# populationgenomics/cuKING

Measured on AMD Instinct MI355X. Metric: sample-pairs/s (all-pairs KING), higher is better.
Workload: dtype fp4 products, f32 accumulate (exact integers)

## Files before the change

### cuking_amd/csrc/king_abi.hip

```cpp
#include <hip/hip_runtime.h>

#include <algorithm>
#include <cstdio>
#include <cstdlib>
#include <cstring>
#include <vector>

#include "king_common.h"
#include "king_host.h"

using namespace cuking;

namespace {

#define HIP_TRY(expr)                                                      \
  do {                                                                     \
    const hipError_t _e = (expr);                                          \
    if (_e != hipSuccess) {                                                \
      (void)hipGetLastError();  \
      return cuking_fail(_e == hipErrorOutOfMemory ? CUKING_ERR_OUT_OF_MEMORY     \
                                            : CUKING_ERR_DEVICE,           \
                  "%s failed: %s", #expr, hipGetErrorString(_e));          \
    }                                                                      \
  } while (0)

uint32_t ceil_div(uint32_t a, uint32_t b) {
  return (uint32_t)(((uint64_t)a + b - 1) / b);
}
uint32_t round_up(uint32_t a, uint32_t b) { return ceil_div(a, b) * b; }

struct EventPair {
  hipEvent_t start = nullptr, stop = nullptr;
};

struct Timer {
  std::vector<EventPair> pool;
  size_t used = 0;

  hipError_t begin(hipStream_t s, EventPair **out) {
    if (used == pool.size()) {
      EventPair p;
      hipError_t e = hipEventCreate(&p.start);
      if (e != hipSuccess) return e;
      e = hipEventCreate(&p.stop);
      if (e != hipSuccess) return e;
      pool.push_back(p);
    }
    *out = &pool[used++];
    return hipEventRecord((*out)->start, s);
  }
  hipError_t collect(double *ms, uint64_t *n) {
    *ms = 0;
    *n = used;
    for (size_t k = 0; k < used; ++k) {
      hipError_t e = hipEventSynchronize(pool[k].stop);
      if (e != hipSuccess) return e;
      float t = 0;
      e = hipEventElapsedTime(&t, pool[k].start, pool[k].stop);
      if (e != hipSuccess) return e;
      *ms += t;
    }
    return hipSuccess;
  }
  void destroy() {
    for (auto &p : pool) {
      if (p.start) (void)hipEventDestroy(p.start);
      if (p.stop) (void)hipEventDestroy(p.stop);
    }
    pool.clear();
    used = 0;
  }
};

}

struct cuking_ctx {
  int device = 0;
  cuking_kernel kernel = CUKING_KERNEL_TILED;
  int variant = 0;
  uint32_t band_rows = 0;
  int counts_mode = -1;
  int xcd_swizzle = 2;
  uint32_t dyn_tail_tiles = 16384;

  uint4 *planes = nullptr;
  size_t planes_bytes = 0;
  uint64_t *band_prefix = nullptr;
  size_t band_prefix_bytes = 0;
  TileSpace prefix_for = {0, 0, 0, 0};

  uint32_t split_wgs = 0;
  struct StreamScratch {
    hipStream_t stream;
    uint32_t *split = nullptr;
    uint8_t *filter = nullptr;
    uint64_t filter_tiles = 0;
  };
  std::vector<StreamScratch> scratch;
  unsigned long long filter_totals_retired[kNumTotals] = {};
  uint32_t filter_quadrant_cap = kFilterQuadrantCap;
  uint32_t filter_cand_cap = kFilterCandCap;
  uint32_t filter_split_min_steps = 8;
  int filter_check0 = 1, filter_check1 = 1, filter_check_emit = (int)kCheckEmitCap;
  int filter_rotate = 1;
  uint32_t filter_rotate_min_steps = 128;
  uint32_t filter_rotate_min_tiles = 2048;
  int filter_sort = 1;
  bool filter_lazy_codes = true;
  void *sort_temp = nullptr;
  size_t sort_temp_bytes = 0;

  struct Prepared {
    bool valid = false;
    cuking_submatrix sm = {0, 0, 0, 0};
    uint32_t words_per_sample = 0;
    int variant = -1;
    uint32_t tile = 0;
    const uint64_t *bits = nullptr;
    bool codes = true;
    std::vector<uint8_t> tiles;
    hipStream_t ordered_on = nullptr;
    bool ordered_valid = false;
  } prepared;
  std::vector<std::pair<hipStream_t, hipEvent_t>> readers;

  bool reuse_prepared = false;
  uint64_t workspace_allocations = 0, host_syncs = 0, conversions_skipped = 0;

  bool timing = false;
  Timer king_timer, prepare_timer;
};

namespace {

int default_variant() {
  if (const char *v = getenv("CUKING_AMD_VARIANT")) {
    const int k = atoi(v);
    if (k >= 0 && k < kNumTiledVariants) return k;
  }
  return kMfmaFilterVariant;
}

int effective_variant(const cuking_ctx *ctx, uint32_t words_per_sample) {
  const uint64_t sites = (uint64_t)round_up(words_per_sample, 8) * 32;
  int v = ctx->variant;
  if ((v == kMfmaN4Variant || v == kMfmaFilterVariant) && sites > kMfmaN4MaxSites) v = kMfmaVariant;
  if (v == kMfmaVariant && sites > kMfmaMaxSites) v = 2;
  return v;
}

TiledVariant plan_variant(const cuking_ctx *ctx, uint32_t words_per_sample) {
  TiledVariant v = tiled_variant(effective_variant(ctx, words_per_sample));
  v.tile = tiled_variant(ctx->variant).tile;
  return v;
}

bool use_full_counts(const cuking_ctx *ctx, float kin_threshold, bool dense,
                     uint32_t words_per_sample) {
  if (dense || ctx->counts_mode == 1) return true;
  if (ctx->counts_mode == 0) return false;
  if (!(kin_threshold > 0.0f)) return true;
  const double sites = 32.0 * words_per_sample;
  const double c = is_mfma_variant(effective_variant(ctx, words_per_sample)) ? 2.05 : 1.6;
  return (double)kin_threshold * kin_threshold * sites < c * c;
}

cuking_status bind(cuking_ctx *ctx) {
  if (ctx == nullptr) return cuking_fail(CUKING_ERR_INVALID_ARGUMENT, "null context");
  HIP_TRY(hipSetDevice(ctx->device));
  return CUKING_OK;
}

PlaneGeometry make_geometry(const cuking_submatrix &sm,
                            uint32_t words_per_sample,
                            const TiledVariant &v) {
  PlaneGeometry g;
  g.num_rows = sm_num_rows(sm);
  g.num_cols = sm_num_cols(sm);
  g.diag = sm_is_diag(sm) ? 1u : 0u;
  g.rows_padded = round_up(g.num_rows, v.tile);
  g.cols_padded = round_up(g.num_cols, v.tile);
  g.col_base = g.diag ? 0u : g.rows_padded;
  g.s_stride = g.diag ? g.rows_padded : g.rows_padded + g.cols_padded;
  g.k_words = round_up(words_per_sample, v.k_chunk);
  return g;
}

uint32_t band_rows_for(uint32_t pinned, const PlaneGeometry &g, const TiledVariant &v) {
  if (pinned != 0) return pinned;
  if (v.layout == kLayoutWord) return 17;
  if (v.tile == kFilterTile) return 8;
  return g.rows_padded / v.tile >= 128 ? 5 : 17;
}

TileSpace make_tiles(const PlaneGeometry &g, const TiledVariant &v,
                     uint32_t band_rows) {
  band_rows = band_rows_for(band_rows, g, v);
  TileSpace t;
  t.tiles_r = g.rows_padded / v.tile;
  t.tiles_c = g.cols_padded / v.tile;
  t.band_rows = band_rows;
  t.diag = g.diag;
  return t;
}

uint64_t total_tiles(const TileSpace &t) {
  uint64_t n = 0;
  for (uint32_t b = 0; b < t.num_bands(); ++b) n += t.band_tiles(b);
  return n;
}

constexpr size_t kMaxStreams = 8;

void free_filter_scratch(cuking_ctx *ctx, cuking_ctx::StreamScratch &e) {
  if (e.filter == nullptr) return;
  unsigned long long v[kNumTotals] = {};
  if (hipMemcpy(v, e.filter + filter_scratch_layout(e.filter_tiles).totals, sizeof v,
                hipMemcpyDeviceToHost) == hipSuccess) {
    for (uint32_t k = 0; k < kNumTotals; ++k) ctx->filter_totals_retired[k] += v[k];
  }
  (void)hipGetLastError();
  (void)hipFree(e.filter);
  e.filter = nullptr;
}

void evict_scratch(cuking_ctx *ctx, size_t k) {
  cuking_ctx::StreamScratch &e = ctx->scratch[k];
  ++ctx->host_syncs;
  if (hipStreamSynchronize(e.stream) != hipSuccess) {
    (void)hipGetLastError();
    (void)hipDeviceSynchronize();
    (void)hipGetLastError();
  }
  free_filter_scratch(ctx, e);
  if (e.split != nullptr) (void)hipFree(e.split);
  ctx->scratch.erase(ctx->scratch.begin() + (ptrdiff_t)k);
}

bool uses_split_slab(const cuking_ctx *ctx) {
  return ctx->split_wgs != 0 && is_mfma_variant(ctx->variant);
}
bool uses_filter_scratch(const cuking_ctx *ctx) { return ctx->variant == kMfmaFilterVariant; }

cuking_status alloc_scratch(cuking_ctx *ctx, void **p, size_t bytes, size_t zero_at,
                            size_t zero_bytes, hipStream_t stream) {
  HIP_TRY(hipMalloc(p, bytes));
  ++ctx->workspace_allocations;
  const hipError_t e = hipMemsetAsync(static_cast<uint8_t *>(*p) + zero_at, 0, zero_bytes, stream);
  if (e != hipSuccess) {
    (void)hipFree(*p);
    *p = nullptr;
    HIP_TRY(e);
  }
  return CUKING_OK;
}

cuking_status scratch_for(cuking_ctx *ctx, hipStream_t stream, uint64_t tiles,
                          cuking_ctx::StreamScratch **out) {
  *out = nullptr;
  const bool split = uses_split_slab(ctx), filter = uses_filter_scratch(ctx);
  if (!split && !filter) return CUKING_OK;
  cuking_ctx::StreamScratch *e = nullptr;
  for (auto &x : ctx->scratch)
    if (x.stream == stream) e = &x;
  if (e == nullptr) {
    if (ctx->scratch.size() >= kMaxStreams) evict_scratch(ctx, 0);
    ctx->scratch.push_back({stream});
    e = &ctx->scratch.back();
  }
  cuking_status st;
  if (split && e->split == nullptr) {
    st = alloc_scratch(ctx, reinterpret_cast<void **>(&e->split),
                       mfma_split_scratch_bytes(ctx->split_wgs), 0,
                       mfma_split_counter_bytes(ctx->split_wgs), stream);
    if (st != CUKING_OK) return st;
  }
  const FilterScratchLayout want = filter_scratch_layout(tiles);
  if (filter && e->filter != nullptr && filter_scratch_layout(e->filter_tiles).bytes < want.bytes) {
    ++ctx->host_syncs;
    HIP_TRY(hipStreamSynchronize(stream));
    free_filter_scratch(ctx, *e);
  }
  if (filter && e->filter == nullptr) {
    st = alloc_scratch(ctx, reinterpret_cast<void **>(&e->filter), want.bytes, want.totals,
                       kFilterCtrlBytes + kFilterTicketBytes, stream);
    if (st != CUKING_OK) return st;
    e->filter_tiles = tiles;
  }
  *out = e;
  return CUKING_OK;
}

struct Outputs {
  uint32_t max_results;
  cuking_result *results;
  uint32_t *result_index, *result_overflow;
  cuking_counts *counts;
};
cuking_status launch_args(cuking_ctx *ctx, hipStream_t stream, const cuking_submatrix &sm,
                          uint32_t words_per_sample, const uint64_t *d_bit_sets,
                          const PlaneGeometry &geo, const TileSpace &tiles,
                          uint64_t block_tiles, float kin_threshold, const Outputs &out,
                          TiledArgs *args) {
  TiledArgs &a = *args;
  a = {};
  a.planes = ctx->planes;
  a.geo = geo;
  a.tiles = tiles;
  a.band_prefix = ctx->band_prefix;
  a.i_begin = sm.i_begin;
  a.j_begin = sm.j_begin;
  a.kin_threshold = kin_threshold;
  a.max_results = out.max_results;
  a.results = out.results;
  a.result_index = out.result_index;
  a.result_overflow = out.result_overflow;
  a.dense_counts = out.counts;
  a.rect_row_stride = 1;
  a.bits = d_bit_sets;
  a.words_per_sample = words_per_sample;
  a.split_wgs = ctx->split_wgs;
  a.xcd_chunk = (uint32_t)ctx->xcd_swizzle;
  a.dyn_tiles = ctx->dyn_tail_tiles;
  if (plan_variant(ctx, words_per_sample).layout == kLayoutNibbleStats) {
    a.perm = plane_perm(ctx->planes, geo);
    if (!ctx->prepared.codes) a.codes_ready = plane_flags(ctx->planes, geo);
  }
  cuking_ctx::StreamScratch *e;
  const cuking_status st = scratch_for(ctx, stream, block_tiles, &e);
  if (st != CUKING_OK || e == nullptr) return st;
  if (uses_split_slab(ctx)) {
    a.split_counters = e->split;
    a.split_scratch = e->split + mfma_split_counter_bytes(ctx->split_wgs) / sizeof(uint32_t);
  }
  if (!uses_filter_scratch(ctx)) return CUKING_OK;
  uint8_t *base = e->filter;
  const FilterScratchLayout l = filter_scratch_layout(e->filter_tiles);
  a.sample_stats = plane_stats(ctx->planes, geo);
  a.t2 = plane_t2(ctx->planes, geo);
  a.prefix_u = plane_prefix_u(ctx->planes, geo);
  a.cohort_sums = plane_cohort_sums(ctx->planes, geo);
  a.filter_ctrl = reinterpret_cast<uint32_t *>(base);
  a.filter_totals = reinterpret_cast<unsigned long long *>(base + l.totals);
  a.fsplit_tickets = reinterpret_cast<uint32_t *>(base + l.tickets);
  a.tile_done = base + l.tile_done;
  a.cand_list = reinterpret_cast<uint2 *>(base + l.cand);
  a.cand_cap = ctx->filter_cand_cap < l.cand_entries ? ctx->filter_cand_cap : l.cand_entries;
  a.quadrant_cap = ctx->filter_quadrant_cap;
  a.dense_list = reinterpret_cast<uint2 *>(base + l.dense);
  a.dense_cap = l.chunk_tiles * 4;
  a.fsplit_first = ctx->filter_split_min_steps;
  a.fsplit_slabs = ctx->split_wgs != 0 ? reinterpret_cast<float4 *>(base + l.slabs) : nullptr;
  a.check0 = (uint32_t)ctx->filter_check0;
  a.check1 = (uint32_t)ctx->filter_check1 | ((uint32_t)ctx->filter_check_emit << 8) |
             (ctx->filter_check0 != 0 ? 1u << 16 : 0u);
  a.rotate = (uint32_t)ctx->filter_rotate;
  a.rotate_min_steps = ctx->filter_rotate_min_steps;
  a.rotate_min_tiles = ctx->filter_rotate_min_tiles;
  a.check_steps = plane_check_steps(ctx->planes, geo);
  return CUKING_OK;
}

bool filter_runs(const cuking_ctx *ctx, uint32_t words_per_sample, bool full, float kin_threshold) {
  return effective_variant(ctx, words_per_sample) == kMfmaFilterVariant && !full &&
         kin_threshold > 0.f && kin_threshold < 0.5f;
}

hipError_t launch_planned(const cuking_ctx *ctx, uint32_t words_per_sample, bool full,
                          TiledArgs a, uint64_t num_tiles, hipStream_t stream) {
  const int kv = effective_variant(ctx, words_per_sample);
  a.quad = 0;
  a.tile_list = nullptr;
  a.tile_list_count = nullptr;
  a.tile_list_cap = 0;
  if (tiled_variant(kv).tile != tiled_variant(ctx->variant).tile) {
    if (tiled_variant(kv).tile * 2 != tiled_variant(ctx->variant).tile) return hipErrorInvalidValue;
    a.quad = 1;
    a.tile_begin *= 4;
    num_tiles *= 4;
  }
  return launch_tiled(kv, full, a, num_tiles, stream);
}

void note_reader(cuking_ctx *ctx, hipStream_t stream) {
  for (auto &r : ctx->readers)
    if (r.first == stream) return;
  ctx->readers.emplace_back(stream, nullptr);
}

cuking_status wait_for_readers(cuking_ctx *ctx, hipStream_t stream) {
  bool failed = false;
  for (auto &r : ctx->readers) {
    if (r.first == stream) continue;
    if (r.second == nullptr &&
        hipEventCreateWithFlags(&r.second, hipEventDisableTiming) != hipSuccess) {
      failed = true;
      break;
    }
    if (hipEventRecord(r.second, r.first) != hipSuccess ||
        hipStreamWaitEvent(stream, r.second, 0) != hipSuccess) {
      failed = true;
      break;
    }
  }
  if (failed) {
    (void)hipGetLastError();
    ++ctx->host_syncs;
    HIP_TRY(hipDeviceSynchronize());
  }
  for (auto &r : ctx->readers)
    if (r.second) (void)hipEventDestroy(r.second);
  ctx->readers.clear();
  ctx->readers.emplace_back(stream, nullptr);
  ctx->prepared.ordered_on = stream;
  ctx->prepared.ordered_valid = true;
  for (auto &t : ctx->prepared.tiles)
    if (t == 2) t = 1;
  return CUKING_OK;
}

void mark_read(cuking_ctx *ctx, uint32_t begin, uint32_t end) {
  std::vector<uint8_t> &t = ctx->prepared.tiles;
  if (end > t.size()) end = (uint32_t)t.size();
  for (uint32_t k = begin; k < end; ++k) t[k] = 2;
}

bool same_block(const cuking_ctx::Prepared &p, const cuking_submatrix &sm,
                uint32_t words_per_sample, int variant, uint32_t tile, const uint64_t *bits) {
  return p.valid && p.sm.i_begin == sm.i_begin && p.sm.i_end == sm.i_end &&
         p.sm.j_begin == sm.j_begin && p.sm.j_end == sm.j_end &&
         p.words_per_sample == words_per_sample && p.variant == variant &&
         p.tile == tile && p.bits == bits;
}

cuking_status grow(cuking_ctx *ctx, void **buf, size_t *bytes, size_t need) {
  if (need <= *bytes) return CUKING_OK;
  ++ctx->host_syncs;
  HIP_TRY(hipDeviceSynchronize());
  if (*buf) HIP_TRY(hipFree(*buf));
  *buf = nullptr;
  *bytes = 0;
  HIP_TRY(hipMalloc(buf, need));
  ++ctx->workspace_allocations;
  *bytes = need;
  return CUKING_OK;
}

cuking_status ensure_workspace(cuking_ctx *ctx, const PlaneGeometry &geo, const TiledVariant &v,
                               const TileSpace &tiles) {
  const size_t planes = plane_bytes(geo, v.layout);
  if (planes > ctx->planes_bytes) ctx->prepared.valid = false;
  cuking_status st = grow(ctx, reinterpret_cast<void **>(&ctx->planes), &ctx->planes_bytes, planes);
  if (st != CUKING_OK) return st;
  const size_t prefix = ((size_t)tiles.num_bands() + 1) * sizeof(uint64_t);
  if (prefix > ctx->band_prefix_bytes) ctx->prefix_for = TileSpace{0, 0, 0, 0};
  st = grow(ctx, reinterpret_cast<void **>(&ctx->band_prefix), &ctx->band_prefix_bytes, prefix);
  if (st != CUKING_OK || v.layout != kLayoutNibbleStats || ctx->filter_sort == 0) return st;
  return grow(ctx, &ctx->sort_temp, &ctx->sort_temp_bytes, sort_temp_bytes_for(geo.s_stride));
}

bool same_tile_space(const TileSpace &a, const TileSpace &b) {
  return a.tiles_r == b.tiles_r && a.tiles_c == b.tiles_c && a.band_rows == b.band_rows &&
         a.diag == b.diag;
}

cuking_status upload_prefix(cuking_ctx *ctx, const TileSpace &tiles, hipStream_t stream) {
  const uint32_t nb = tiles.num_bands();
  std::vector<uint64_t> prefix((size_t)nb + 1, 0);
  for (uint32_t b = 0; b < nb; ++b) prefix[b + 1] = prefix[b] + tiles.band_tiles(b);
  HIP_TRY(hipMemcpyAsync(ctx->band_prefix, prefix.data(), prefix.size() * sizeof(uint64_t),
                         hipMemcpyHostToDevice, stream));
  ++ctx->host_syncs;
  HIP_TRY(hipStreamSynchronize(stream));
  ctx->prefix_for = tiles;
  return CUKING_OK;
}

cuking_status convert_codes_now(cuking_ctx *ctx, const PlaneGeometry &geo,
                                uint32_t words_per_sample, const uint64_t *d_bit_sets,
                                hipStream_t stream) {
  cuking_ctx::Prepared &pr = ctx->prepared;
  const uint32_t all = (uint32_t)pr.tiles.size();
  for (uint32_t t = 0; t < all;) {
    if (pr.tiles[t] == 0) {
      ++t;
      continue;
    }
    uint32_t e = t;
    while (e < all && pr.tiles[e] != 0) ++e;
    HIP_TRY(launch_prepare_nibbles(true, false, d_bit_sets, words_per_sample, geo, ctx->planes,
                                   plane_perm(ctx->planes, geo), t, e, nullptr, nullptr, stream));
    t = e;
  }
  HIP_TRY(hipMemsetAsync(plane_flags(ctx->planes, geo), 1, sizeof(uint32_t), stream));
  pr.codes = true;
  return CUKING_OK;
}

cuking_status prepare(cuking_ctx *ctx, const cuking_submatrix &sm,
                      uint32_t words_per_sample, const uint64_t *d_bit_sets,
                      hipStream_t stream, PlaneGeometry *geo_out,
                      TileSpace *tiles_out, bool need_codes, uint32_t s_tile_begin = 0,
                      uint32_t s_tile_end = 0xFFFFFFFFu) {
  const int variant = effective_variant(ctx, words_per_sample);
  const TiledVariant v = plan_variant(ctx, words_per_sample);
  const PlaneGeometry geo = make_geometry(sm, words_per_sample, v);
  const TileSpace tiles = make_tiles(geo, v, ctx->band_rows);
  *geo_out = geo;
  *tiles_out = tiles;

  cuking_status st = ensure_workspace(ctx, geo, v, tiles);
  if (st != CUKING_OK) return st;
  const uint32_t all_tiles = (geo.s_stride + 63) / 64;
  const uint32_t t_end = s_tile_end < all_tiles ? s_tile_end : all_tiles;
  cuking_ctx::Prepared &pr = ctx->prepared;
  const bool new_prefix = !same_tile_space(ctx->prefix_for, tiles);
  const bool same = same_block(pr, sm, words_per_sample, variant, v.tile, d_bit_sets);
  if (ctx->reuse_prepared && same && !new_prefix) {
    bool all_there = true;
    for (uint32_t t = s_tile_begin; t < t_end && all_there; ++t) all_there = pr.tiles[t] != 0;
    if (all_there) {
      ++ctx->conversions_skipped;
      if (v.layout == kLayoutNibbleStats && need_codes && !pr.codes)
        return convert_codes_now(ctx, geo, words_per_sample, d_bit_sets, stream);
      return CUKING_OK;
    }
  }
  const bool other_stream = pr.ordered_valid && pr.ordered_on != stream;
  bool must_wait = new_prefix && !ctx->readers.empty();
  if (!same) {
    must_wait = must_wait || !ctx->readers.empty();
    pr.valid = true;
    pr.sm = sm;
    pr.words_per_sample = words_per_sample;
    pr.variant = variant;
    pr.tile = v.tile;
    pr.bits = d_bit_sets;
    pr.tiles.assign(all_tiles, 0);
    pr.codes = true;
  }
  for (uint32_t t = s_tile_begin; t < t_end; ++t)
    must_wait = must_wait || pr.tiles[t] == 2 || (pr.tiles[t] == 1 && other_stream);
  if (must_wait) {
    st = wait_for_readers(ctx, stream);
    if (st != CUKING_OK) return st;
  }
  for (uint32_t t = s_tile_begin; t < t_end; ++t) pr.tiles[t] = 1;
  if (new_prefix) {
    st = upload_prefix(ctx, tiles, stream);
    if (st != CUKING_OK) return st;
  }

  if (plane_bytes(geo, v.layout) == 0) return CUKING_OK;
  EventPair *ev = nullptr;
  if (ctx->timing) HIP_TRY(ctx->prepare_timer.begin(stream, &ev));
  if (v.layout == kLayoutNibbleStats) {
    const bool whole = s_tile_begin == 0 && t_end == all_tiles;
    const bool codes = need_codes || !ctx->filter_lazy_codes || !whole;
    const uint32_t sb = s_tile_begin * 64, se = t_end * 64;
    if (s_tile_begin == 0)
      HIP_TRY(hipMemsetAsync(const_cast<unsigned long long *>(plane_cohort_sums(ctx->planes, geo)),
                             0, 64, stream));
    HIP_TRY(hipMemsetAsync(plane_flags(ctx->planes, geo), 0, sizeof(uint32_t), stream));
    HIP_TRY(launch_sample_stats(d_bit_sets, words_per_sample, geo, ctx->planes, sb, se, stream));
    HIP_TRY(launch_sample_order(geo, words_per_sample, ctx->planes, sb, se,
                                ctx->filter_sort == 2 || (ctx->filter_sort == 1 && whole),
                                ctx->sort_temp, ctx->sort_temp_bytes, stream));
    HIP_TRY(launch_prepare_nibbles(codes, true, d_bit_sets, words_per_sample, geo, ctx->planes,
                                   plane_perm(ctx->planes, geo), s_tile_begin, t_end, nullptr,
                                   nullptr, stream));
    if (!codes) {
      pr.codes = false;
    } else if (!pr.codes) {
      st = convert_codes_now(ctx, geo, words_per_sample, d_bit_sets, stream);
      if (st != CUKING_OK) return st;
    } else {
      HIP_TRY(hipMemsetAsync(plane_flags(ctx->planes, geo), 1, sizeof(uint32_t), stream));
    }
  } else {
    HIP_TRY(launch_prepare_planes(v.layout, d_bit_sets, words_per_sample, geo, ctx->planes,
                                  s_tile_begin, s_tile_end, stream));
  }
  if (ev) HIP_TRY(hipEventRecord(ev->stop, stream));
  return CUKING_OK;
}

cuking_status run_tiled(cuking_ctx *ctx, const cuking_submatrix &sm,
                        uint32_t words_per_sample, const uint64_t *d_bit_sets,
                        uint64_t tile_begin, uint64_t tile_end, bool whole,
                        float kin_threshold, const Outputs &out, hipStream_t stream) {
  PlaneGeometry geo;
  TileSpace tiles;
  const bool full = use_full_counts(ctx, kin_threshold, out.counts != nullptr, words_per_sample);
  cuking_status st = prepare(ctx, sm, words_per_sample, d_bit_sets, stream, &geo, &tiles,
                             !filter_runs(ctx, words_per_sample, full, kin_threshold));
  if (st != CUKING_OK) return st;
  const uint64_t n_tiles = total_tiles(tiles);
  if (whole) {
    tile_begin = 0;
    tile_end = n_tiles;
  }
  if (tile_begin > tile_end || tile_end > n_tiles)
    return cuking_fail(CUKING_ERR_INVALID_ARGUMENT,
                "tile range [%llu, %llu) outside [0, %llu)",
                (unsigned long long)tile_begin, (unsigned long long)tile_end,
                (unsigned long long)n_tiles);
  if (tile_begin == tile_end) return CUKING_OK;

  TiledArgs a;
  st = launch_args(ctx, stream, sm, words_per_sample, d_bit_sets, geo, tiles, n_tiles,
                   kin_threshold, out, &a);
  if (st != CUKING_OK) return st;
  a.tile_begin = tile_begin;

  EventPair *ev = nullptr;
  if (ctx->timing) HIP_TRY(ctx->king_timer.begin(stream, &ev));
  HIP_TRY(launch_planned(ctx, words_per_sample, full, a, tile_end - tile_begin, stream));
  note_reader(ctx, stream);
  mark_read(ctx, 0, 0xFFFFFFFFu);
  if (ev) HIP_TRY(hipEventRecord(ev->stop, stream));
  return CUKING_OK;
}

cuking_status run_stream(cuking_ctx *ctx, const cuking_submatrix &sm,
                         uint32_t words_per_sample, const uint64_t *d_bit_sets,
                         float kin_threshold, uint32_t max_results,
                         cuking_result *d_results, uint32_t *d_result_index,
                         uint32_t *d_result_overflow, cuking_counts *d_counts,
                         hipStream_t stream) {
  EventPair *ev = nullptr;
  if (ctx->timing) HIP_TRY(ctx->king_timer.begin(stream, &ev));
  HIP_TRY(launch_stream(sm, words_per_sample, d_bit_sets, kin_threshold,
                        max_results, d_results, d_result_index,
                        d_result_overflow, d_counts, stream));
  if (ev) HIP_TRY(hipEventRecord(ev->stop, stream));
  return CUKING_OK;
}


enum : uint8_t {
  kInvalidatesLayout = 1,
  kResizesSlabs = 2,
};

struct Option {
  const char *key;
  int64_t lo, hi;
  const char *error;
  uint32_t error_arg;
  uint8_t effects;
  int64_t (*get)(const cuking_ctx *);
  void (*set)(cuking_ctx *, int64_t);
  int64_t hole = INT64_MIN;
};

#define CTX_FIELD(f)                                                     \
  [](const cuking_ctx *c) -> int64_t { return (int64_t)c->f; },          \
  [](cuking_ctx *c, int64_t v) { c->f = (decltype(c->f))v; }

const Option kOptions[] = {
    {"variant", 0, kNumTiledVariants - 1, "variant outside [0, %u)", kNumTiledVariants, 0,
     CTX_FIELD(variant)},
    {"band_rows", 0, 64, "band_rows outside [0, 64]", 0, 0, CTX_FIELD(band_rows)},
    {"counts_mode", -1, 1, "counts_mode outside [-1, 1]", 0, 0, CTX_FIELD(counts_mode)},
    {"split_wgs", 0, 4096, "split_wgs outside [0, 4096]", 0, kResizesSlabs, CTX_FIELD(split_wgs)},
    {"xcd_swizzle", 0, 2, "xcd_swizzle outside [0, 2]", 0, 0, CTX_FIELD(xcd_swizzle)},
    {"dyn_tail_tiles", 0, 0x7FFFFFFF, "dyn_tail_tiles outside [0, 2^31)", 0, 0,
     CTX_FIELD(dyn_tail_tiles)},
    {"reuse_prepared", 0, 1, "reuse_prepared outside [0, 1]", 0, 0, CTX_FIELD(reuse_prepared)},
    {"filter_sort", 0, 2, "filter_sort outside [0, 2]", 0, kInvalidatesLayout,
     CTX_FIELD(filter_sort)},
    {"filter_lazy_codes", 0, 1, "filter_lazy_codes outside [0, 1]", 0, kInvalidatesLayout,
     CTX_FIELD(filter_lazy_codes)},
    {"filter_check0", 0, 2, "filter_check0 outside [0, 2]", 0, 0, CTX_FIELD(filter_check0)},
    {"filter_check1", 0, 1 + kNumCheckShares, "filter_check1 outside {0, 1, 3 .. %u}",
     1 + kNumCheckShares, 0, CTX_FIELD(filter_check1), 2},
    {"filter_check_emit", 0, 255, "filter_check_emit outside [0, 255]", 0, 0,
     CTX_FIELD(filter_check_emit)},
    {"filter_rotate", 0, 2 + kNumPhases, "filter_rotate outside [0, %u]", 2 + kNumPhases, 0,
     CTX_FIELD(filter_rotate)},
    {"filter_rotate_min_steps", 1, 1 << 20, "filter_rotate_min_steps outside [1, 2^20]", 0, 0,
     CTX_FIELD(filter_rotate_min_steps)},
    {"filter_rotate_min_tiles", 0, 1 << 30, "filter_rotate_min_tiles outside [0, 2^30]", 0, 0,
     CTX_FIELD(filter_rotate_min_tiles)},
    {"filter_quadrant_cap", 0, 16384, "filter_quadrant_cap outside [0, 16384]", 0, 0,
     CTX_FIELD(filter_quadrant_cap)},
    {"filter_cand_cap", 0, kFilterCandCap, "filter_cand_cap outside [0, %u]", kFilterCandCap, 0,
     CTX_FIELD(filter_cand_cap)},
    {"filter_split_min_steps", 1, 4096, "filter_split_min_steps outside [1, 4096]", 0, 0,
     CTX_FIELD(filter_split_min_steps)},
    {"max_launch_blocks", 0, INT64_MAX, "negative block cap", 0, 0,
     [](const cuking_ctx *) -> int64_t { return (int64_t)max_blocks_override(); },
     [](cuking_ctx *, int64_t v) { set_max_blocks_per_launch((uint64_t)v); }},
    {"filter_check_min_steps", 4, 1 << 20, "filter_check_min_steps outside [4, 2^20]", 0,
     kInvalidatesLayout,
     [](const cuking_ctx *) -> int64_t { return filter_check_min_steps(); },
     [](cuking_ctx *, int64_t v) { set_filter_check_min_steps((uint32_t)v); }},
};
#undef CTX_FIELD

const Option *find_option(const char *key) {
  for (const Option &o : kOptions)
    if (strcmp(o.key, key) == 0) return &o;
  return nullptr;
}

cuking_status read_diagnostic(const cuking_ctx *ctx, const char *key, int64_t *value) {
  const std::pair<const char *, uint64_t> counters[] = {
      {"workspace_allocations", ctx->workspace_allocations},
      {"host_syncs", ctx->host_syncs},
      {"conversions_skipped", ctx->conversions_skipped}};
  for (const auto &c : counters)
    if (strcmp(c.first, key) == 0) {
      *value = (int64_t)c.second;
      return CUKING_OK;
    }
  const char *const totals[kNumTotals] = {"filter_candidates", "filter_dense_quadrants",
                                          "filter_early_exits", "filter_rotated_tiles"};
  static_assert(kTotalCand == 0 && kTotalDense == 1 && kTotalEarly == 2 && kTotalRotated == 3,
                "totals[] in the order of the running totals");
  uint32_t word = 0;
  while (word < kNumTotals && strcmp(totals[word], key) != 0) ++word;
  const bool ticks = strcmp(key, "filter_step_ticks16") == 0;
  if (word == kNumTotals && !ticks)
    return cuking_fail(CUKING_ERR_INVALID_ARGUMENT, "unknown option %s", key);
  if (hipSetDevice(ctx->device) != hipSuccess || hipDeviceSynchronize() != hipSuccess)
    return cuking_fail(CUKING_ERR_DEVICE, "device wait failed");
  unsigned long long sum = 0;
  uint64_t count = 0;
  for (const auto &e : ctx->scratch) {
    if (e.filter == nullptr) continue;
    if (ticks) {
      uint32_t w[8];
      if (hipMemcpy(w, e.filter + kCtrlStepTicks * 4, sizeof w, hipMemcpyDeviceToHost) != hipSuccess)
        return cuking_fail(CUKING_ERR_DEVICE, "reading the filter counters failed");
      for (uint32_t v : w)
        if (v != 0) {
          sum += v;
          ++count;
        }
    } else {
      unsigned long long v = 0;
      if (hipMemcpy(&v, e.filter + filter_scratch_layout(e.filter_tiles).totals + word * 8, 8,
                    hipMemcpyDeviceToHost) != hipSuccess)
        return cuking_fail(CUKING_ERR_DEVICE, "reading the filter counters failed");
      sum += v;
    }
  }
  if (ticks) *value = count != 0 ? (int64_t)(sum / count) : 0;
  else *value = (int64_t)(sum + ctx->filter_totals_retired[word]);
  return CUKING_OK;
}

}

extern "C" {


int cuking_device_count(void) {
  int n = 0;
  if (hipGetDeviceCount(&n) != hipSuccess) return 0;
  return n;
}

cuking_status cuking_ctx_create(int device, cuking_ctx **out) {
  if (out == nullptr) return cuking_fail(CUKING_ERR_INVALID_ARGUMENT, "null out pointer");
  *out = nullptr;
  int n = 0;
  hipError_t e = hipGetDeviceCount(&n);
  if (e != hipSuccess || n == 0)
    return cuking_fail(CUKING_ERR_DEVICE,
                "no HIP device available (%s); this library has no CPU path",
                e == hipSuccess ? "0 devices" : hipGetErrorString(e));
  if (device < 0 || device >= n)
    return cuking_fail(CUKING_ERR_INVALID_ARGUMENT, "device %d outside [0, %d)", device, n);
  hipDeviceProp_t prop;
  HIP_TRY(hipGetDeviceProperties(&prop, device));
  if (strncmp(prop.gcnArchName, "gfx950", 6) != 0)
    return cuking_fail(CUKING_ERR_DEVICE,
                "device %d is %s; this library only carries gfx950 code",
                device, prop.gcnArchName);
  HIP_TRY(hipSetDevice(device));
  cuking_ctx *ctx = new cuking_ctx();
  ctx->device = device;
  ctx->variant = default_variant();
  ctx->split_wgs = (uint32_t)prop.multiProcessorCount;
  *out = ctx;
  return CUKING_OK;
}

void cuking_ctx_destroy(cuking_ctx *ctx) {
  if (ctx == nullptr) return;
  (void)hipSetDevice(ctx->device);
  if (ctx->planes) (void)hipFree(ctx->planes);
  if (ctx->band_prefix) (void)hipFree(ctx->band_prefix);
  if (ctx->sort_temp) (void)hipFree(ctx->sort_temp);
  for (auto &e : ctx->scratch) {
    if (e.split) (void)hipFree(e.split);
    if (e.filter) (void)hipFree(e.filter);
  }
  for (auto &r : ctx->readers)
    if (r.second) (void)hipEventDestroy(r.second);
  ctx->king_timer.destroy();
  ctx->prepare_timer.destroy();
  delete ctx;
}

cuking_status cuking_ctx_set_kernel(cuking_ctx *ctx, cuking_kernel kernel) {
  if (ctx == nullptr) return cuking_fail(CUKING_ERR_INVALID_ARGUMENT, "null context");
  if (kernel != CUKING_KERNEL_TILED && kernel != CUKING_KERNEL_STREAM)
    return cuking_fail(CUKING_ERR_INVALID_ARGUMENT, "unknown kernel %d", (int)kernel);
  ctx->kernel = kernel;
  return CUKING_OK;
}

cuking_status cuking_ctx_set_option(cuking_ctx *ctx, const char *key,
                                    int64_t value) {
  if (ctx == nullptr || key == nullptr)
    return cuking_fail(CUKING_ERR_INVALID_ARGUMENT, "null argument");
  const Option *o = find_option(key);
  if (o == nullptr) return cuking_fail(CUKING_ERR_INVALID_ARGUMENT, "unknown option %s", key);
  if (value < o->lo || value > o->hi || value == o->hole)
    return cuking_fail(CUKING_ERR_INVALID_ARGUMENT, o->error, o->error_arg);
  if ((o->effects & kResizesSlabs) && value != o->get(ctx)) {
    HIP_TRY(hipDeviceSynchronize());
    for (auto &e : ctx->scratch) {
      if (e.split) (void)hipFree(e.split);
      e.split = nullptr;
    }
  }
  o->set(ctx, value);
  if (o->effects & kInvalidatesLayout) ctx->prepared.valid = false;
  return CUKING_OK;
}

cuking_status cuking_device_alloc(cuking_ctx *ctx, size_t bytes, void **d_ptr) {
  cuking_status st = bind(ctx);
  if (st != CUKING_OK) return st;
  if (d_ptr == nullptr) return cuking_fail(CUKING_ERR_INVALID_ARGUMENT, "null out pointer");
  *d_ptr = nullptr;
  if (bytes == 0) return CUKING_OK;
  HIP_TRY(hipMalloc(d_ptr, bytes));
  return CUKING_OK;
}

cuking_status cuking_device_free(cuking_ctx *ctx, void *d_ptr) {
  cuking_status st = bind(ctx);
  if (st != CUKING_OK) return st;
  if (d_ptr) HIP_TRY(hipFree(d_ptr));
  return CUKING_OK;
}

cuking_status cuking_memset_async(cuking_ctx *ctx, void *d_ptr, int byte_value,
                                  size_t bytes, void *stream) {
  cuking_status st = bind(ctx);
  if (st != CUKING_OK) return st;
  if (bytes) HIP_TRY(hipMemsetAsync(d_ptr, byte_value, bytes, (hipStream_t)stream));
  return CUKING_OK;
}

cuking_status cuking_copy_to_device(cuking_ctx *ctx, void *d_dst,
                                    const void *src, size_t bytes,
                                    void *stream) {
  cuking_status st = bind(ctx);
  if (st != CUKING_OK) return st;
  if (bytes)
    HIP_TRY(hipMemcpyAsync(d_dst, src, bytes, hipMemcpyHostToDevice,
                           (hipStream_t)stream));
  return CUKING_OK;
}

cuking_status cuking_copy_to_host(cuking_ctx *ctx, void *dst, const void *d_src,
                                  size_t bytes, void *stream) {
  cuking_status st = bind(ctx);
  if (st != CUKING_OK) return st;
  if (bytes)
    HIP_TRY(hipMemcpyAsync(dst, d_src, bytes, hipMemcpyDeviceToHost,
                           (hipStream_t)stream));
  return CUKING_OK;
}

cuking_status cuking_stream_synchronize(cuking_ctx *ctx, void *stream) {
  cuking_status st = bind(ctx);
  if (st != CUKING_OK) return st;
  HIP_TRY(hipStreamSynchronize((hipStream_t)stream));
  return CUKING_OK;
}

cuking_status cuking_stream_create(cuking_ctx *ctx, void **stream) {
  cuking_status st = bind(ctx);
  if (st != CUKING_OK) return st;
  if (stream == nullptr) return cuking_fail(CUKING_ERR_INVALID_ARGUMENT, "null out pointer");
  hipStream_t s = nullptr;
  HIP_TRY(hipStreamCreateWithFlags(&s, hipStreamNonBlocking));
  *stream = s;
  return CUKING_OK;
}

cuking_status cuking_stream_destroy(cuking_ctx *ctx, void *stream) {
  cuking_status st = bind(ctx);
  if (st != CUKING_OK) return st;
  if (stream) {
    auto &rs = ctx->readers;
    for (size_t k = 0; k < rs.size(); ++k)
      if (rs[k].first == (hipStream_t)stream) {
        HIP_TRY(hipStreamSynchronize((hipStream_t)stream));
        if (rs[k].second) (void)hipEventDestroy(rs[k].second);
        rs.erase(rs.begin() + k);
        break;
      }
    HIP_TRY(hipStreamDestroy((hipStream_t)stream));
  }
  return CUKING_OK;
}

cuking_status cuking_host_alloc(cuking_ctx *ctx, size_t bytes, void **ptr) {
  cuking_status st = bind(ctx);
  if (st != CUKING_OK) return st;
  if (ptr == nullptr) return cuking_fail(CUKING_ERR_INVALID_ARGUMENT, "null out pointer");
  *ptr = nullptr;
  if (bytes == 0) return CUKING_OK;
  HIP_TRY(hipHostMalloc(ptr, bytes, hipHostMallocDefault));
  return CUKING_OK;
}

cuking_status cuking_host_free(cuking_ctx *ctx, void *ptr) {
  cuking_status st = bind(ctx);
  if (st != CUKING_OK) return st;
  if (ptr) HIP_TRY(hipHostFree(ptr));
  return CUKING_OK;
}


cuking_status cuking_pack_device(cuking_ctx *ctx, const cuking_submatrix *sm,
                                 uint32_t words_per_sample, uint64_t *d_bit_set,
                                 const int64_t *d_row_idx,
                                 const int64_t *d_col_idx,
                                 const int32_t *d_n_alt_alleles,
                                 size_t num_triples, uint32_t *d_status,
                                 void *stream) {
  cuking_status st = bind(ctx);
  if (st != CUKING_OK) return st;
  st = cuking_check_block(sm, words_per_sample);
  if (st != CUKING_OK) return st;
  if (num_triples &&
      (!d_bit_set || !d_row_idx || !d_col_idx || !d_n_alt_alleles || !d_status))
    return cuking_fail(CUKING_ERR_INVALID_ARGUMENT, "null device pointer");
  HIP_TRY(launch_pack(*sm, words_per_sample, d_bit_set, d_row_idx, d_col_idx,
                      d_n_alt_alleles, num_triples, d_status,
                      (hipStream_t)stream));
  return CUKING_OK;
}

cuking_status cuking_pack_device_compact(cuking_ctx *ctx, const cuking_submatrix *sm,
                                         uint32_t words_per_sample, uint64_t *d_bit_set,
                                         const uint32_t *d_site,
                                         const uint32_t *d_sample_alt, size_t num_triples,
                                         uint32_t *d_status, void *stream) {
  cuking_status st = bind(ctx);
  if (st != CUKING_OK) return st;
  st = cuking_check_block(sm, words_per_sample);
  if (st != CUKING_OK) return st;
  if (num_triples && (!d_bit_set || !d_site || !d_sample_alt || !d_status))
    return cuking_fail(CUKING_ERR_INVALID_ARGUMENT, "null device pointer");
  HIP_TRY(launch_pack_compact(words_per_sample, sm_num_samples(*sm), d_bit_set, d_site,
                              d_sample_alt, num_triples, d_status, (hipStream_t)stream));
  return CUKING_OK;
}

cuking_status cuking_event_create(cuking_ctx *ctx, void **event) {
  cuking_status st = bind(ctx);
  if (st != CUKING_OK) return st;
  if (event == nullptr) return cuking_fail(CUKING_ERR_INVALID_ARGUMENT, "null out pointer");
  hipEvent_t e = nullptr;
  HIP_TRY(hipEventCreateWithFlags(&e, hipEventDisableTiming));
  *event = e;
  return CUKING_OK;
}

cuking_status cuking_event_record(cuking_ctx *ctx, void *event, void *stream) {
  cuking_status st = bind(ctx);
  if (st != CUKING_OK) return st;
  HIP_TRY(hipEventRecord((hipEvent_t)event, (hipStream_t)stream));
  return CUKING_OK;
}

cuking_status cuking_event_synchronize(cuking_ctx *ctx, void *event) {
  cuking_status st = bind(ctx);
  if (st != CUKING_OK) return st;
  HIP_TRY(hipEventSynchronize((hipEvent_t)event));
  return CUKING_OK;
}

cuking_status cuking_event_destroy(cuking_ctx *ctx, void *event) {
  cuking_status st = bind(ctx);
  if (st != CUKING_OK) return st;
  if (event) HIP_TRY(hipEventDestroy((hipEvent_t)event));
  return CUKING_OK;
}

uint32_t cuking_tile_samples(const cuking_ctx *ctx) {
  return tiled_variant(ctx ? ctx->variant : default_variant()).tile;
}

uint64_t cuking_num_tiles(const cuking_ctx *ctx, const cuking_submatrix *sm) {
  if (sm == nullptr) return 0;
  const TiledVariant &v = tiled_variant(ctx ? ctx->variant : default_variant());
  const PlaneGeometry g = make_geometry(*sm, 2, v);
  if (g.num_rows == 0 || g.num_cols == 0) return 0;
  return total_tiles(make_tiles(g, v, ctx ? ctx->band_rows : 0));
}

cuking_status cuking_tile_bounds(const cuking_ctx *ctx,
                                 const cuking_submatrix *sm, uint64_t tile,
                                 uint32_t *row_begin, uint32_t *row_end,
                                 uint32_t *col_begin, uint32_t *col_end) {
  cuking_status st = cuking_check_block(sm, 2);
  if (st != CUKING_OK) return st;
  const TiledVariant &v = tiled_variant(ctx ? ctx->variant : default_variant());
  const PlaneGeometry g = make_geometry(*sm, 2, v);
  const TileSpace ts = make_tiles(g, v, ctx ? ctx->band_rows : 0);
  if (g.num_rows == 0 || g.num_cols == 0 || tile >= total_tiles(ts))
    return cuking_fail(CUKING_ERR_INVALID_ARGUMENT, "tile index out of range");
  uint32_t b = 0;
  uint64_t first = 0;
  while (first + ts.band_tiles(b) <= tile) first += ts.band_tiles(b++);
  uint32_t tr, tc;
  ts.decode(b, tile - first, &tr, &tc);
  auto clampr = [&](uint64_t x) { return (uint32_t)std::min<uint64_t>(x, g.num_rows); };
  auto clampc = [&](uint64_t x) { return (uint32_t)std::min<uint64_t>(x, g.num_cols); };
  if (row_begin) *row_begin = sm->i_begin + clampr((uint64_t)tr * v.tile);
  if (row_end) *row_end = sm->i_begin + clampr((uint64_t)(tr + 1) * v.tile);
  if (col_begin) *col_begin = sm->j_begin + clampc((uint64_t)tc * v.tile);
  if (col_end) *col_end = sm->j_begin + clampc((uint64_t)(tc + 1) * v.tile);
  return CUKING_OK;
}

cuking_status cuking_ctx_get_option(const cuking_ctx *ctx, const char *key,
                                    int64_t *value) {
  if (ctx == nullptr || key == nullptr || value == nullptr)
    return cuking_fail(CUKING_ERR_INVALID_ARGUMENT, "null argument");
  if (const Option *o = find_option(key)) {
    *value = o->get(ctx);
    return CUKING_OK;
  }
  return read_diagnostic(ctx, key, value);
}

int cuking_num_variants(void) { return kNumTiledVariants; }
const char *cuking_variant_name(int variant) {
  if (variant < 0 || variant >= kNumTiledVariants) return "";
  return tiled_variant(variant).name;
}

static cuking_status check_compute_args(const cuking_submatrix *sm,
                                        uint32_t words_per_sample,
                                        const uint64_t *d_bit_sets) {
  cuking_status st = cuking_check_block(sm, words_per_sample);
  if (st != CUKING_OK) return st;
  if (sm_num_samples(*sm) != 0 && d_bit_sets == nullptr)
    return cuking_fail(CUKING_ERR_INVALID_ARGUMENT, "null bitset pointer");
  return CUKING_OK;
}

cuking_status cuking_compute_king(cuking_ctx *ctx, const cuking_submatrix *sm,
                                  uint32_t words_per_sample,
                                  const uint64_t *d_bit_sets,
                                  float kin_threshold, uint32_t max_results,
                                  cuking_result *d_results,
                                  uint32_t *d_result_index,
                                  uint32_t *d_result_overflow, void *stream) {
  cuking_status st = bind(ctx);
  if (st != CUKING_OK) return st;
  st = check_compute_args(sm, words_per_sample, d_bit_sets);
  if (st != CUKING_OK) return st;
  if (!d_result_index || !d_result_overflow || (max_results && !d_results))
    return cuking_fail(CUKING_ERR_INVALID_ARGUMENT, "null result pointer");
  if (sm_num_rows(*sm) == 0 || sm_num_cols(*sm) == 0) return CUKING_OK;
  if (ctx->kernel == CUKING_KERNEL_STREAM)
    return run_stream(ctx, *sm, words_per_sample, d_bit_sets, kin_threshold,
                      max_results, d_results, d_result_index, d_result_overflow,
                      nullptr, (hipStream_t)stream);
  return run_tiled(ctx, *sm, words_per_sample, d_bit_sets, 0, 0, true, kin_threshold,
                   {max_results, d_results, d_result_index, d_result_overflow, nullptr},
                   (hipStream_t)stream);
}

cuking_status cuking_compute_king_tiles(
    cuking_ctx *ctx, const cuking_submatrix *sm, uint32_t words_per_sample,
    const uint64_t *d_bit_sets, uint64_t tile_begin, uint64_t tile_end,
    float kin_threshold, uint32_t max_results, cuking_result *d_results,
    uint32_t *d_result_index, uint32_t *d_result_overflow, void *stream) {
  cuking_status st = bind(ctx);
  if (st != CUKING_OK) return st;
  st = check_compute_args(sm, words_per_sample, d_bit_sets);
  if (st != CUKING_OK) return st;
  if (!d_result_index || !d_result_overflow || (max_results && !d_results))
    return cuking_fail(CUKING_ERR_INVALID_ARGUMENT, "null result pointer");
  if (sm_num_rows(*sm) == 0 || sm_num_cols(*sm) == 0) {
    if (tile_begin != 0 || tile_end != 0)
      return cuking_fail(CUKING_ERR_INVALID_ARGUMENT, "empty block has no tiles");
    return CUKING_OK;
  }
  return run_tiled(ctx, *sm, words_per_sample, d_bit_sets, tile_begin, tile_end, false,
                   kin_threshold,
                   {max_results, d_results, d_result_index, d_result_overflow, nullptr},
                   (hipStream_t)stream);
}

static cuking_status tile_span(const cuking_submatrix &sm, uint32_t tile,
                               uint32_t begin, uint32_t end, const char *what,
                               uint32_t *t0, uint32_t *t1) {
  if (begin < sm.i_begin || end > sm.i_end || begin > end)
    return cuking_fail(CUKING_ERR_INVALID_ARGUMENT, "%s range [%u, %u) outside the block",
                what, begin, end);
  const uint32_t b = begin - sm.i_begin, e = end - sm.i_begin;
  if (b % tile != 0 || (e % tile != 0 && end != sm.i_end))
    return cuking_fail(CUKING_ERR_INVALID_ARGUMENT,
                "%s range [%u, %u) is not aligned to the %u-sample tile edge", what,
                begin, end, tile);
  *t0 = b / tile;
  *t1 = (e + tile - 1) / tile;
  return CUKING_OK;
}

cuking_status cuking_prepare_samples(cuking_ctx *ctx, const cuking_submatrix *sm,
                                     uint32_t words_per_sample,
                                     const uint64_t *d_bit_sets,
                                     uint32_t sample_begin, uint32_t sample_end,
                                     void *stream) {
  cuking_status st = bind(ctx);
  if (st != CUKING_OK) return st;
  st = check_compute_args(sm, words_per_sample, d_bit_sets);
  if (st != CUKING_OK) return st;
  if (!sm_is_diag(*sm))
    return cuking_fail(CUKING_ERR_INVALID_ARGUMENT,
                "staged preparation needs a diagonal block (rows == columns)");
  const uint32_t tile = plan_variant(ctx, words_per_sample).tile;
  uint32_t t0, t1;
  st = tile_span(*sm, tile, sample_begin, sample_end, "sample", &t0, &t1);
  if (st != CUKING_OK) return st;
  if (t0 == t1) return CUKING_OK;
  PlaneGeometry geo;
  TileSpace tiles;
  return prepare(ctx, *sm, words_per_sample, d_bit_sets, (hipStream_t)stream, &geo,
                 &tiles, true, t0 * (tile / 64), t1 * (tile / 64));
}

cuking_status cuking_compute_king_rect(
    cuking_ctx *ctx, const cuking_submatrix *sm, uint32_t words_per_sample,
    const uint64_t *d_bit_sets, uint32_t row_begin, uint32_t row_end,
    uint32_t row_step, uint32_t col_begin, uint32_t col_end, float kin_threshold,
    uint32_t max_results, cuking_result *d_results, uint32_t *d_result_index,
    uint32_t *d_result_overflow, void *stream) {
  cuking_status st = bind(ctx);
  if (st != CUKING_OK) return st;
  st = check_compute_args(sm, words_per_sample, d_bit_sets);
  if (st != CUKING_OK) return st;
  if (!sm_is_diag(*sm))
    return cuking_fail(CUKING_ERR_INVALID_ARGUMENT,
                "rectangle launches need a diagonal block (rows == columns)");
  if (!d_result_index || !d_result_overflow || (max_results && !d_results))
    return cuking_fail(CUKING_ERR_INVALID_ARGUMENT, "null result pointer");
  const TiledVariant v = plan_variant(ctx, words_per_sample);
  const PlaneGeometry geo = make_geometry(*sm, words_per_sample, v);
  const TileSpace tiles = make_tiles(geo, v, ctx->band_rows ? ctx->band_rows : 17);
  const size_t need = plane_bytes(geo, v.layout);
  const int variant = effective_variant(ctx, words_per_sample);
  if (ctx->planes == nullptr || ctx->planes_bytes < need ||
      !same_block(ctx->prepared, *sm, words_per_sample, variant, v.tile, d_bit_sets))
    return cuking_fail(CUKING_ERR_FAILED_PRECONDITION,
                "cuking_prepare_samples() has not been called for this block "
                "(or the workspace has been converted for another one since)");
  uint32_t r0, r1, c0, c1;
  st = tile_span(*sm, v.tile, row_begin, row_end, "row", &r0, &r1);
  if (st != CUKING_OK) return st;
  st = tile_span(*sm, v.tile, col_begin, col_end, "column", &c0, &c1);
  if (st != CUKING_OK) return st;
  if (r0 == r1 || c0 == c1) return CUKING_OK;
  if (row_step == 0) row_step = v.tile;
  if (row_step % v.tile != 0)
    return cuking_fail(CUKING_ERR_INVALID_ARGUMENT,
                "row_step %u is not a multiple of the %u-sample tile edge", row_step,
                v.tile);
  const uint32_t stride = row_step / v.tile;
  const uint32_t n_rows = (r1 - r0 + stride - 1) / stride;
  {
    const uint32_t per = v.tile / 64;
    const std::vector<uint8_t> &done = ctx->prepared.tiles;
    auto converted = [&](uint32_t tile) {
      for (uint32_t t = tile * per; t < (tile + 1) * per; ++t)
        if (t >= done.size() || !done[t]) return false;
      return true;
    };
    for (uint32_t r = r0; r < r1; r += stride)
      if (!converted(r))
        return cuking_fail(CUKING_ERR_FAILED_PRECONDITION,
                    "row samples from %u on have not been prepared",
                    sm->i_begin + r * v.tile);
    for (uint32_t c = c0; c < c1; ++c)
      if (!converted(c))
        return cuking_fail(CUKING_ERR_FAILED_PRECONDITION,
                    "column samples from %u on have not been prepared",
                    sm->i_begin + c * v.tile);
  }

  TiledArgs a;
  st = launch_args(ctx, (hipStream_t)stream, *sm, words_per_sample, d_bit_sets, geo, tiles,
                   total_tiles(make_tiles(geo, v, ctx->band_rows)), kin_threshold,
                   {max_results, d_results, d_result_index, d_result_overflow, nullptr}, &a);
  if (st != CUKING_OK) return st;
  a.rect_rows = n_rows;
  a.rect_cols = c1 - c0;
  a.rect_row0 = r0;
  a.rect_col0 = c0;
  a.rect_row_stride = stride;
  a.xcd_chunk = ctx->xcd_swizzle == 2 ? 2u : 0u;
  const bool full = use_full_counts(ctx, kin_threshold, false, words_per_sample);
  if (v.layout == kLayoutNibbleStats && !ctx->prepared.codes &&
      !filter_runs(ctx, words_per_sample, full, kin_threshold)) {
    st = convert_codes_now(ctx, geo, words_per_sample, d_bit_sets, (hipStream_t)stream);
    if (st != CUKING_OK) return st;
    a.codes_ready = nullptr;
  }
  EventPair *ev = nullptr;
  if (ctx->timing) HIP_TRY(ctx->king_timer.begin((hipStream_t)stream, &ev));
  HIP_TRY(launch_planned(ctx, words_per_sample, full, a, (uint64_t)n_rows * (c1 - c0),
                         (hipStream_t)stream));
  note_reader(ctx, (hipStream_t)stream);
  {
    const uint32_t per = v.tile / 64;
    for (uint32_t r = r0; r < r1; r += stride) mark_read(ctx, r * per, (r + 1) * per);
    mark_read(ctx, c0 * per, c1 * per);
  }
  if (ev) HIP_TRY(hipEventRecord(ev->stop, (hipStream_t)stream));
  return CUKING_OK;
}

cuking_status cuking_ctx_reserve(cuking_ctx *ctx, const cuking_submatrix *sm,
                                 uint32_t words_per_sample, void *const *streams,
                                 size_t num_streams) {
  cuking_status st = bind(ctx);
  if (st != CUKING_OK) return st;
  st = cuking_check_block(sm, words_per_sample);
  if (st != CUKING_OK) return st;
  if (num_streams != 0 && streams == nullptr)
    return cuking_fail(CUKING_ERR_INVALID_ARGUMENT, "null stream list");
  if (sm_num_rows(*sm) == 0 || sm_num_cols(*sm) == 0) return CUKING_OK;
  const TiledVariant v = plan_variant(ctx, words_per_sample);
  const PlaneGeometry geo = make_geometry(*sm, words_per_sample, v);
  const TileSpace tiles = make_tiles(geo, v, ctx->band_rows);
  st = ensure_workspace(ctx, geo, v, tiles);
  if (st != CUKING_OK) return st;
  if (!same_tile_space(ctx->prefix_for, tiles)) {
    if (!ctx->readers.empty()) {
      ++ctx->host_syncs;
      HIP_TRY(hipDeviceSynchronize());
    }
    st = upload_prefix(ctx, tiles, nullptr);
    if (st != CUKING_OK) return st;
  }
  if (num_streams > kMaxStreams)
    return cuking_fail(CUKING_ERR_INVALID_ARGUMENT,
                       "at most %zu streams per context can be reserved", kMaxStreams);
  auto named = [&](hipStream_t s) {
    for (size_t k = 0; k < num_streams; ++k)
      if ((hipStream_t)streams[k] == s) return true;
    return false;
  };
  if (uses_split_slab(ctx) || uses_filter_scratch(ctx)) {
    size_t missing = num_streams;
    for (const auto &e : ctx->scratch) missing -= named(e.stream) ? 1 : 0;
    for (size_t k = 0; ctx->scratch.size() + missing > kMaxStreams;) {
      if (named(ctx->scratch[k].stream))
        ++k;
      else
        evict_scratch(ctx, k);
    }
  }
  for (size_t k = 0; k < num_streams; ++k) {
    cuking_ctx::StreamScratch *e;
    st = scratch_for(ctx, (hipStream_t)streams[k], total_tiles(tiles), &e);
    if (st != CUKING_OK) return st;
  }
  return CUKING_OK;
}

cuking_status cuking_invalidate(cuking_ctx *ctx) {
  if (ctx == nullptr) return cuking_fail(CUKING_ERR_INVALID_ARGUMENT, "null context");
  ctx->prepared.valid = false;
  return CUKING_OK;
}

cuking_status cuking_compute_counts(cuking_ctx *ctx, const cuking_submatrix *sm,
                                    uint32_t words_per_sample,
                                    const uint64_t *d_bit_sets,
                                    cuking_counts *d_counts, void *stream) {
  cuking_status st = bind(ctx);
  if (st != CUKING_OK) return st;
  st = check_compute_args(sm, words_per_sample, d_bit_sets);
  if (st != CUKING_OK) return st;
  if (sm_num_rows(*sm) == 0 || sm_num_cols(*sm) == 0) return CUKING_OK;
  if (d_counts == nullptr)
    return cuking_fail(CUKING_ERR_INVALID_ARGUMENT, "null counts pointer");
  if (ctx->kernel == CUKING_KERNEL_STREAM)
    return run_stream(ctx, *sm, words_per_sample, d_bit_sets, 0.f, 0, nullptr,
                      nullptr, nullptr, d_counts, (hipStream_t)stream);
  return run_tiled(ctx, *sm, words_per_sample, d_bit_sets, 0, 0, true, 0.f,
                   {0, nullptr, nullptr, nullptr, d_counts}, (hipStream_t)stream);
}


cuking_status cuking_timing_enable(cuking_ctx *ctx, int enabled) {
  if (ctx == nullptr) return cuking_fail(CUKING_ERR_INVALID_ARGUMENT, "null context");
  ctx->timing = enabled != 0;
  return CUKING_OK;
}

cuking_status cuking_timing_reset(cuking_ctx *ctx) {
  if (ctx == nullptr) return cuking_fail(CUKING_ERR_INVALID_ARGUMENT, "null context");
  ctx->king_timer.used = 0;
  ctx->prepare_timer.used = 0;
  return CUKING_OK;
}

cuking_status cuking_timing_collect(cuking_ctx *ctx, double *king_ms,
                                    uint64_t *king_launches, double *prepare_ms,
                                    uint64_t *prepare_launches) {
  cuking_status st = bind(ctx);
  if (st != CUKING_OK) return st;
  double a = 0, b = 0;
  uint64_t na = 0, nb = 0;
  HIP_TRY(ctx->king_timer.collect(&a, &na));
  HIP_TRY(ctx->prepare_timer.collect(&b, &nb));
  if (king_ms) *king_ms = a;
  if (king_launches) *king_launches = na;
  if (prepare_ms) *prepare_ms = b;
  if (prepare_launches) *prepare_launches = nb;
  return CUKING_OK;
}

cuking_status cuking_clock_probe(cuking_ctx *ctx, uint64_t microseconds,
                                 uint64_t *d_ticks, void *stream) {
  cuking_status st = bind(ctx);
  if (st != CUKING_OK) return st;
  if (d_ticks == nullptr) return cuking_fail(CUKING_ERR_INVALID_ARGUMENT, "null out pointer");
  if (microseconds == 0 || microseconds > 60ull * 1000 * 1000)
    return cuking_fail(CUKING_ERR_INVALID_ARGUMENT, "probe time outside (0, 60 s]");
  HIP_TRY(launch_clock_probe(microseconds, d_ticks, (hipStream_t)stream));
  return CUKING_OK;
}


cuking_status cuking_synth_bitset(cuking_ctx *ctx, uint64_t seed,
                                  const uint32_t *d_kind, const uint32_t *d_pa,
                                  const uint32_t *d_pb, uint32_t sample_begin,
                                  uint32_t sample_end, uint32_t num_sites,
                                  uint32_t words_per_sample,
                                  uint64_t *d_bit_set, void *stream) {
  cuking_status st = bind(ctx);
  if (st != CUKING_OK) return st;
  if (sample_end < sample_begin)
    return cuking_fail(CUKING_ERR_INVALID_ARGUMENT, "sample range reversed");
  if (words_per_sample != cuking_words_per_sample(num_sites))
    return cuking_fail(CUKING_ERR_INVALID_ARGUMENT,
                "words_per_sample %u does not match %u sites", words_per_sample,
                num_sites);
  if (sample_end > sample_begin && (!d_kind || !d_pa || !d_pb || !d_bit_set))
    return cuking_fail(CUKING_ERR_INVALID_ARGUMENT, "null device pointer");
  HIP_TRY(launch_synth(seed, d_kind, d_pa, d_pb, sample_begin, sample_end,
                       num_sites, words_per_sample, d_bit_set,
                       (hipStream_t)stream));
  return CUKING_OK;
}

}
```

### cuking_amd/csrc/king_common.h

```cpp
#ifndef CUKING_AMD_KING_COMMON_H_
#define CUKING_AMD_KING_COMMON_H_

#include <hip/hip_runtime.h>
#include <stdint.h>

#include "cuking_amd.h"
#include "king_submatrix.h"

namespace cuking {

constexpr uint32_t kLayoutWord = 0;
constexpr uint32_t kLayoutQuad = 1;
constexpr uint32_t kLayoutNibble = 2;
constexpr uint32_t kLayoutNibbleStats = 3;

struct PlaneGeometry {
  uint32_t num_rows, num_cols;
  uint32_t rows_padded, cols_padded;
  uint32_t col_base;
  uint32_t s_stride;
  uint32_t k_words;
  uint32_t diag;
};

struct TileSpace {
  uint32_t tiles_r, tiles_c;
  uint32_t band_rows;
  uint32_t diag;

  __host__ __device__ uint32_t num_bands() const {
    return (tiles_r + band_rows - 1) / band_rows;
  }
  __host__ __device__ uint64_t band_tiles(uint32_t b) const {
    const uint32_t r0 = b * band_rows;
    const uint32_t h = (tiles_r - r0 < band_rows) ? tiles_r - r0 : band_rows;
    if (!diag) return (uint64_t)h * tiles_c;
    const uint32_t ncols = tiles_c - r0;
    return (uint64_t)h * (h + 1) / 2 + (uint64_t)(ncols - h) * h;
  }
  __host__ __device__ void decode(uint32_t b, uint64_t u, uint32_t *tr,
                                  uint32_t *tc) const {
    const uint32_t r0 = b * band_rows;
    const uint32_t h = (tiles_r - r0 < band_rows) ? tiles_r - r0 : band_rows;
    if (!diag) {
      *tc = (uint32_t)(u / h);
      *tr = r0 + (uint32_t)(u % h);
      return;
    }
    const uint64_t tri = (uint64_t)h * (h + 1) / 2;
    if (u < tri) {
      uint32_t c = 0;
      uint64_t before = 0;
      while (before + c + 1 <= u) {
        before += c + 1;
        ++c;
      }
      *tc = r0 + c;
      *tr = r0 + (uint32_t)(u - before);
    } else {
      const uint64_t v = u - tri;
      *tc = r0 + h + (uint32_t)(v / h);
      *tr = r0 + (uint32_t)(v % h);
    }
  }
};

struct TiledArgs {
  const uint4 *planes;
  PlaneGeometry geo;
  TileSpace tiles;
  const uint64_t *band_prefix;
  uint64_t tile_begin;
  uint32_t rect_rows, rect_cols, rect_row0, rect_col0, rect_row_stride;
  uint32_t i_begin, j_begin;
  float kin_threshold;
  uint32_t max_results;
  cuking_result *results;
  uint32_t *result_index;
  uint32_t *result_overflow;
  cuking_counts *dense_counts;
  const uint64_t *bits;
  uint32_t words_per_sample;
  uint32_t split_tiles, split_wgs;
  uint32_t split_whole;
  uint32_t *split_scratch, *split_counters;
  uint32_t xcd_chunk, launch_tiles;
  uint32_t dyn_tiles, dyn_wgs;
  uint32_t quad;
  const uint2 *tile_list;
  const uint32_t *tile_list_count;
  uint32_t tile_list_cap;
  const float2 *sample_stats;
  const uint4 *t2;
  uint32_t *filter_ctrl;
  unsigned long long *filter_totals;
  uint2 *cand_list;
  uint32_t cand_cap;
  uint32_t quadrant_cap;
  uint2 *dense_list;
  uint32_t dense_cap;
  uint32_t fsplit_parts, fsplit_first, fsplit_tile0;
  float4 *fsplit_slabs;
  uint32_t *fsplit_tickets;
  const uint32_t *check_steps;
  const float *prefix_u;
  const unsigned long long *cohort_sums;
  uint32_t check0, check1;
  uint32_t rotate, rotate_min_steps;
  uint32_t rotate_min_tiles;
  uint8_t *tile_done;
  const uint32_t *gate;
  uint32_t gate_count;
  const uint8_t *skip_tiles;
  uint64_t skip_base;
  const uint32_t *perm;
  uint32_t *codes_ready;
};

constexpr uint32_t kCheckEmitCap = 64;
constexpr uint32_t kNumCheckShares = 8;
constexpr uint32_t kCheckShares64[kNumCheckShares] = {8, 50, 53, 56, 58, 60, 61, 62};
constexpr uint32_t kNumPhases = 128;
constexpr uint32_t kPhasesPerShare = kNumPhases / 64;
constexpr uint32_t kNumCum = kNumPhases - 1;
__host__ __device__ inline uint32_t phase_step(uint32_t all_steps, uint32_t x) {
  return (uint32_t)((uint64_t)all_steps * x / kNumPhases);
}
__host__ __device__ inline uint32_t check_step_of(uint32_t all_steps, uint32_t k,
                                                  uint32_t min_steps = 64) {
  if (all_steps < min_steps) return 0;
  return phase_step(all_steps, kCheckShares64[k] * kPhasesPerShare);
}
constexpr uint32_t kFilterSplitSlabs = 256;
constexpr size_t kFilterSlabBytes = 256 * 256 * sizeof(float);
constexpr size_t kFilterTicketBytes = kFilterSplitSlabs * sizeof(uint32_t);
__host__ __device__ inline size_t plane_bytes(const PlaneGeometry &g,
                                              uint32_t layout) {
  const size_t base = (size_t)g.k_words * g.s_stride * (layout == kLayoutQuad ? 8 : 16);
  if (layout == kLayoutNibble) return base + base / 4;
  if (layout == kLayoutNibbleStats)
    return base + base / 4 + base / 2 + (size_t)g.s_stride * sizeof(float2) +
           (size_t)g.s_stride * kNumCum * sizeof(float) + 64 + 64 +
           64 + (size_t)g.s_stride * (4 + 8 + 4 * kNumCum + 16);
  return base;
}
__host__ __device__ inline const uint4 *plane_t2(const uint4 *planes, const PlaneGeometry &g) {
  return planes + (size_t)g.k_words * g.s_stride * 5 / 4;
}
__host__ __device__ inline const float2 *plane_stats(const uint4 *planes, const PlaneGeometry &g) {
  return reinterpret_cast<const float2 *>(planes + (size_t)g.k_words * g.s_stride * 7 / 4);
}
__host__ __device__ inline const float *plane_prefix_u(const uint4 *planes, const PlaneGeometry &g) {
  return reinterpret_cast<const float *>(plane_stats(planes, g) + g.s_stride);
}
__host__ __device__ inline const unsigned long long *plane_cohort_sums(const uint4 *planes,
                                                                       const PlaneGeometry &g) {
  return reinterpret_cast<const unsigned long long *>(plane_prefix_u(planes, g) +
                                                      (size_t)g.s_stride * kNumCum);
}

struct TiledVariant {
  const char *name;
  uint32_t tile;
  uint32_t k_chunk;
  uint32_t threads;
  uint32_t lds_bytes;
  uint32_t layout;
};

constexpr uint32_t kMfmaMaxSites = 1u << 24;

constexpr int kNumTiledVariants = 8;
constexpr int kMfmaVariant = 5;
constexpr int kMfmaN4Variant = 6;
constexpr uint32_t kMfmaN4MaxSites = 1u << 22;
constexpr int kMfmaN4Stages = 5;
constexpr uint32_t kMfmaN4LdsBytes = kMfmaN4Stages * 2 * 2 * 4 * 128 * 16;
static_assert(kMfmaN4LdsBytes <= 160 * 1024, "LDS of one CU");
constexpr int kMfmaFilterVariant = 7;
constexpr uint32_t kFilterTile = 256;
constexpr uint32_t kFilterLdsBytes = 5 * 2 * 2 * 2 * 256 * 16;
static_assert(kFilterLdsBytes <= 160 * 1024, "LDS of one CU");
constexpr uint32_t kFilterChunkTiles = 1u << 17;
constexpr uint32_t kFilterCandCap = 1u << 25;
constexpr uint32_t kFilterQuadrantCap = 384;
constexpr size_t kFilterCtrlBytes = 256;
constexpr uint32_t kCtrlCand = 0, kCtrlDense = 1, kCtrlDyn = 2, kCtrlFinished = 3,
                   kCtrlLeft = 4, kCtrlAllLeave = 5, kCtrlGate = 6;
constexpr uint32_t kCtrlStepTicks = 8, kCtrlPos = 16, kPosSlots = 16;
constexpr size_t kCtrlChunkBytes = (kCtrlPos + 8 * kPosSlots * 2) * 4;
constexpr uint32_t kTotalCand = 0, kTotalDense = 1, kTotalEarly = 2, kTotalRotated = 3;
constexpr uint32_t kNumTotals = 4;
__host__ __device__ inline const uint32_t *plane_check_steps(const uint4 *planes,
                                                             const PlaneGeometry &g) {
  return reinterpret_cast<const uint32_t *>(plane_cohort_sums(planes, g) + 8);
}
__host__ __device__ inline uint32_t *plane_flags(const uint4 *planes, const PlaneGeometry &g) {
  return const_cast<uint32_t *>(plane_check_steps(planes, g)) + 16;
}
__host__ __device__ inline uint32_t *plane_perm(const uint4 *planes, const PlaneGeometry &g) {
  return plane_flags(planes, g) + 16;
}
__host__ __device__ inline float2 *plane_tmp_stats(const uint4 *planes, const PlaneGeometry &g) {
  return reinterpret_cast<float2 *>(plane_perm(planes, g) + g.s_stride);
}
__host__ __device__ inline float *plane_tmp_prefix(const uint4 *planes, const PlaneGeometry &g) {
  return reinterpret_cast<float *>(plane_tmp_stats(planes, g) + g.s_stride);
}
__host__ __device__ inline uint32_t *plane_sort_words(const uint4 *planes, const PlaneGeometry &g) {
  return reinterpret_cast<uint32_t *>(plane_tmp_prefix(planes, g) +
                                      (size_t)g.s_stride * kNumCum);
}
constexpr uint32_t kNoSample = 0xFFFFFFFFu;

struct FilterScratchLayout {
  size_t tile_done, totals, tickets, cand, dense, slabs, bytes;
  uint32_t chunk_tiles, cand_entries;
};
inline FilterScratchLayout filter_scratch_layout(uint64_t tiles) {
  FilterScratchLayout l;
  l.chunk_tiles = (uint32_t)(tiles < kFilterChunkTiles ? (tiles ? tiles : 1) : kFilterChunkTiles);
  const uint64_t cand = (uint64_t)l.chunk_tiles * 4 * 64;
  l.cand_entries = (uint32_t)(cand < kFilterCandCap ? cand : kFilterCandCap);
  auto up = [](size_t x) { return (x + 255) / 256 * 256; };
  l.tile_done = kCtrlChunkBytes;
  l.totals = up(l.tile_done + l.chunk_tiles);
  l.tickets = l.totals + kFilterCtrlBytes;
  l.cand = l.tickets + kFilterTicketBytes;
  l.dense = l.cand + up((size_t)l.cand_entries * sizeof(uint2));
  l.slabs = l.dense + up((size_t)l.chunk_tiles * 4 * sizeof(uint2));
  l.bytes = l.slabs + kFilterSplitSlabs * kFilterSlabBytes;
  return l;
}
inline bool is_mfma_variant(int v) {
  return v == kMfmaVariant || v == kMfmaN4Variant || v == kMfmaFilterVariant;
}
constexpr int kMfmaStages = 6;
constexpr uint32_t kMfmaLdsBytes = kMfmaStages * 2 * 2 * 2 * 128 * 16;
constexpr uint32_t kMfmaParkBytes = 4 * 64 * 64 * 4;
static_assert(kMfmaLdsBytes + kMfmaParkBytes <= 160 * 1024, "LDS of one CU");
const TiledVariant &tiled_variant(int v);
hipError_t launch_tiled(int variant, bool full, const TiledArgs &args,
                        uint64_t num_tiles, hipStream_t stream);
hipError_t launch_mfma(bool full, bool nibble, const TiledArgs &args, uint64_t num_tiles,
                       uint32_t lds_bytes, hipStream_t stream);
hipError_t launch_mfma_list(const TiledArgs &args, uint32_t grid, hipStream_t stream);
hipError_t launch_mfma_gated(const TiledArgs &args, uint64_t num_units, uint32_t grid,
                             hipStream_t stream);
hipError_t launch_filter(const TiledArgs &args, uint64_t num_tiles, hipStream_t stream);
hipError_t launch_sample_stats(const uint64_t *d_bit_sets, uint32_t words_per_sample,
                               const PlaneGeometry &geo, uint4 *d_planes, uint32_t s_begin,
                               uint32_t s_end, hipStream_t stream);
void set_filter_check_min_steps(uint32_t steps);
uint32_t filter_check_min_steps();
size_t sort_temp_bytes_for(uint32_t n);
hipError_t launch_sample_order(const PlaneGeometry &geo, uint32_t words_per_sample,
                               uint4 *d_planes, uint32_t s_begin, uint32_t s_end, bool sort,
                               void *sort_temp, size_t sort_temp_bytes, hipStream_t stream);
hipError_t launch_prepare_nibbles(bool codes, bool t2, const uint64_t *d_bit_sets,
                                  uint32_t words_per_sample, const PlaneGeometry &geo,
                                  uint4 *d_planes, const uint32_t *perm, uint32_t s_tile_begin,
                                  uint32_t s_tile_end, const uint32_t *gate,
                                  const uint32_t *ready, hipStream_t stream);
hipError_t launch_mark_codes_ready(const uint32_t *gate, uint32_t *ready, hipStream_t stream);
size_t mfma_split_scratch_bytes(uint32_t wgs);
size_t mfma_split_counter_bytes(uint32_t wgs);

void set_max_blocks_per_launch(uint64_t blocks);
uint64_t max_blocks_override();

hipError_t launch_prepare_planes(uint32_t layout, const uint64_t *d_bit_sets,
                                 uint32_t words_per_sample,
                                 const PlaneGeometry &geo, uint4 *d_planes,
                                 uint32_t s_tile_begin, uint32_t s_tile_end,
                                 hipStream_t stream);

hipError_t launch_stream(const cuking_submatrix &sm, uint32_t words_per_sample,
                         const uint64_t *d_bit_sets, float kin_threshold,
                         uint32_t max_results, cuking_result *d_results,
                         uint32_t *d_result_index, uint32_t *d_result_overflow,
                         cuking_counts *d_dense_counts, hipStream_t stream);

hipError_t launch_pack(const cuking_submatrix &sm, uint32_t words_per_sample,
                       uint64_t *d_bit_set, const int64_t *d_row_idx,
                       const int64_t *d_col_idx, const int32_t *d_n_alt,
                       size_t num_triples, uint32_t *d_status,
                       hipStream_t stream);

hipError_t launch_pack_compact(uint32_t words_per_sample, uint32_t num_samples,
                               uint64_t *d_bit_set, const uint32_t *d_site,
                               const uint32_t *d_sample_alt, size_t num_triples,
                               uint32_t *d_status, hipStream_t stream);

hipError_t launch_synth(uint64_t seed, const uint32_t *d_kind,
                        const uint32_t *d_pa, const uint32_t *d_pb,
                        uint32_t sample_begin, uint32_t sample_end,
                        uint32_t num_sites, uint32_t words_per_sample,
                        uint64_t *d_bit_set, hipStream_t stream);

hipError_t launch_clock_probe(uint64_t microseconds, uint64_t *d_out,
                              hipStream_t stream);

}

#endif
```

### cuking_amd/csrc/king_filter.hip

```cpp
#include <hip/hip_runtime.h>
#include <stdio.h>

#include <atomic>
#include <stdlib.h>

#include "king_common.h"
#include "king_device.h"

#pragma clang diagnostic ignored "-Winline-asm"

namespace cuking {

namespace {

typedef int v8i __attribute__((ext_vector_type(8)));
typedef float v16f __attribute__((ext_vector_type(16)));

constexpr int kT = (int)kFilterTile;
constexpr int kUnits = 2;
constexpr int kStages = 5;
constexpr int kSliceU4 = kT;
constexpr int kStageU4 = 2 * 2 * kUnits * kSliceU4;
constexpr int kStageReqs = 4 * kUnits;
constexpr int kSyncVm = (kStages - 3) * kStageReqs + (kStageReqs - 2);
static_assert(kSyncVm < 64, "vmcnt is a 6-bit counter");
static_assert(kStages * kStageU4 * 16 == (int)kFilterLdsBytes, "LDS size");
constexpr int vmcnt_imm(int n) { return 0x0F70 | (n & 15) | ((n >> 4) << 14); }
constexpr uint32_t kNoPair = 0xFFFFFFFFu;

__device__ __forceinline__ uint32_t source_sample(const PlaneGeometry &geo, uint32_t ps) {
  if (geo.diag || ps < geo.rows_padded) return ps < geo.num_rows ? ps : kNoPair;
  const uint32_t c = ps - geo.col_base;
  return c < geo.num_cols ? geo.num_rows + c : kNoPair;
}

struct CheckWords {
  uint32_t w[kNumCheckShares];
};
constexpr uint32_t kStatsMaxSteps = kMfmaN4MaxSites / 256;
__global__ __launch_bounds__(256) void sample_stats_kernel(
    const uint64_t *__restrict__ bits, uint32_t words_per_sample, PlaneGeometry geo,
    float2 *__restrict__ stats, float *__restrict__ cum, unsigned long long *__restrict__ sums,
    uint32_t *__restrict__ steps_out, CheckWords cw, uint32_t s_begin, uint32_t s_end) {
  __shared__ uint8_t phase_of[kStatsMaxSteps];
  __shared__ int32_t phase_sum[4][kNumPhases];
  const uint32_t lane = threadIdx.x & 63, wave = threadIdx.x >> 6;
  if (blockIdx.x == 0 && threadIdx.x < kNumCheckShares) steps_out[threadIdx.x] = cw.w[threadIdx.x];
  const uint32_t all_steps = geo.k_words / 8;
  for (uint32_t st = threadIdx.x; st < all_steps; st += 256) {
    const uint32_t x = (kNumPhases * (st + 1) - 1) / all_steps;
    phase_of[st] = (uint8_t)(x < kNumPhases ? x : kNumPhases - 1);
  }
#pragma unroll
  for (uint32_t k = 0; k < kNumPhases / 64; ++k) phase_sum[wave][lane + 64 * k] = 0;
  __syncthreads();
  const uint32_t ps = s_begin + blockIdx.x * 4 + wave;
  if (ps >= s_end) return;
  const uint32_t src = source_sample(geo, ps);
  int32_t yc = 0, mc = 0, hc = 0;
  if (src != kNoPair) {
    const uint32_t n = words_per_sample / 2;
    const uint64_t *het = bits + (uint64_t)src * words_per_sample;
    const uint64_t *hom = het + n;
    constexpr uint32_t kAhead = 4;
    for (uint32_t w0 = 0; w0 < n; w0 += 64 * kAhead) {
      uint64_t h[kAhead], v[kAhead];
#pragma unroll
      for (uint32_t k = 0; k < kAhead; ++k) {
        const uint32_t w = w0 + 64 * k + lane;
        const bool in = w < n;
        h[k] = in ? het[w] : 0ull;
        v[k] = in ? hom[w] : 0ull;
      }
#pragma unroll
      for (uint32_t k = 0; k < kAhead; ++k) {
        const uint32_t w = w0 + 64 * k + lane;
        const bool in = w < n;
        const int32_t y = in ? __popcll(~h[k]) : 0;
        const int32_t m = __popcll(h[k] & v[k]);
        yc += y;
        mc += m;
        hc += __popcll(h[k] & ~v[k]);
        int32_t d = y - m;
        d += __shfl_xor(d, 1);
        d += __shfl_xor(d, 2);
        if ((lane & 3) == 0 && in) atomicAdd(&phase_sum[wave][phase_of[w >> 2]], d);
      }
    }
#pragma unroll
    for (int off = 32; off > 0; off >>= 1) {
      yc += __shfl_xor(yc, off);
      mc += __shfl_xor(mc, off);
      hc += __shfl_xor(hc, off);
    }
  }
  static_assert(kNumPhases == 128, "two phases per lane");
  const int32_t p0 = phase_sum[wave][2 * lane], p1 = phase_sum[wave][2 * lane + 1];
  int32_t run = p0 + p1;
#pragma unroll
  for (int off = 1; off < 64; off <<= 1) {
    const int32_t up = __shfl_up(run, off);
    if ((int)lane >= off) run += up;
  }
  cum[(size_t)(2 * lane) * geo.s_stride + ps] = (float)(run - p1);
  if (2 * lane + 1 < kNumCum) cum[(size_t)(2 * lane + 1) * geo.s_stride + ps] = (float)run;
  if (lane == 0) {
    stats[ps] = make_float2((float)(yc - mc), (float)hc);
    if (src != kNoPair && ((blockIdx.x & 15) == 0 || gridDim.x < 64)) {
      __hip_atomic_fetch_add(sums, 1ull, __ATOMIC_RELAXED, __HIP_MEMORY_SCOPE_AGENT);
      __hip_atomic_fetch_add(sums + 1, (unsigned long long)mc, __ATOMIC_RELAXED,
                             __HIP_MEMORY_SCOPE_AGENT);
      __hip_atomic_fetch_add(sums + 2, (unsigned long long)hc, __ATOMIC_RELAXED,
                             __HIP_MEMORY_SCOPE_AGENT);
    }
  }
}

__device__ __forceinline__ v16f mma(const v8i a, const v8i b, const v16f c) {
  return __builtin_amdgcn_mfma_scale_f32_32x32x64_f8f6f4(a, b, c, 4 , 4, 0, 0, 0, 0);
}

__device__ __forceinline__ v8i tfrag(const uint4 w, uint32_t mask) {
  v8i r = {0, 0, 0, 0, 0, 0, 0, 0};
  r[0] = (int)(w.x & mask);
  r[1] = (int)(w.y & mask);
  r[2] = (int)(w.z & mask);
  r[3] = (int)(w.w & mask);
  return r;
}

__device__ __forceinline__ uint4 shl2(const uint4 w) {
  return make_uint4(w.x << 2, w.y << 2, w.z << 2, w.w << 2);
}

#define F_ISSUE(SRC, DST, OFF)                                                 \
  asm volatile("s_mov_b32 m0, %0\n\t"                                          \
               "s_nop 0\n\t"                                                   \
               "global_load_lds_dwordx4 %1, %2 offset:" #OFF                   \
               :                                                               \
               : "s"(DST), "v"(lane16), "s"(SRC)                               \
               : "memory", "m0")

__device__ __forceinline__ int filter_tile(const TiledArgs &a, const uint32_t wg, uint4 *const lds) {
  uint32_t bid = wg;
  const bool split = a.fsplit_parts != 0 && wg >= a.fsplit_first;
  uint32_t part = 0, piece = 0;
  if (split) {
    piece = wg - a.fsplit_first;
    part = __builtin_amdgcn_readfirstlane(piece % a.fsplit_parts);
    bid = a.fsplit_tile0 + piece / a.fsplit_parts;
  } else
  if (a.dyn_tiles != 0 && wg >= a.launch_tiles) {
    uint32_t *slot = reinterpret_cast<uint32_t *>(lds);
    if (threadIdx.x == 0)
      *slot = __hip_atomic_fetch_add(a.filter_ctrl + kCtrlDyn, 1u, __ATOMIC_RELAXED,
                                     __HIP_MEMORY_SCOPE_AGENT);
    __syncthreads();
    const uint32_t t = __builtin_amdgcn_readfirstlane(*slot);
    __syncthreads();
    if (t >= a.dyn_tiles) return 1;
    bid = a.launch_tiles + t;
  } else if (a.xcd_chunk == 1) {
    const uint32_t x = bid & 7, j = bid >> 3;
    bid = (((j >> 5) * 8 + x) << 5) + (j & 31);
    if (bid >= a.launch_tiles) return 0;
  }
  bid = __builtin_amdgcn_readfirstlane(bid);
  uint32_t tr, tc;
  if (!decode_tile_space(a, a.tile_begin + bid, &tr, &tc)) return 0;
  tr = __builtin_amdgcn_readfirstlane(tr);
  tc = __builtin_amdgcn_readfirstlane(tc);

  const uint32_t lane = threadIdx.x & 63;
  const uint32_t wave = __builtin_amdgcn_readfirstlane(threadIdx.x >> 6);
  const uint32_t wy = wave >> 1, wx = wave & 1;
  uint32_t xcd_pos = 0;
  if (!split && a.tile_done != nullptr) {
    uint32_t *verdict = reinterpret_cast<uint32_t *>(lds);
    if (threadIdx.x == 0) {
      uint32_t leave = __hip_atomic_load(a.filter_ctrl + kCtrlAllLeave, __ATOMIC_RELAXED,
                                         __HIP_MEMORY_SCOPE_AGENT);
      if (leave == 0 && a.cohort_sums != nullptr && a.check_steps != nullptr) {
        const float ns = (float)a.cohort_sums[0], nm = (float)a.cohort_sums[1],
                    nh = (float)a.cohort_sums[2];
        if (ns > 0.f && nh > 0.f) {
          const float sites = 32.f * (float)a.geo.k_words;
          const float m = nm / (ns * sites), h = nh / (ns * sites);
          if (m * (1.f + m / (2.f * h * (1.f - m))) - 4.f * rsqrtf(sites) > a.kin_threshold &&
              (a.check1 >> 16) != 0) {
            leave = 1;
            __hip_atomic_store(a.filter_ctrl + kCtrlAllLeave, 1u, __ATOMIC_RELAXED,
                               __HIP_MEMORY_SCOPE_AGENT);
            __hip_atomic_store(a.filter_ctrl + kCtrlGate, 1u, __ATOMIC_RELAXED,
                               __HIP_MEMORY_SCOPE_AGENT);
          }
        }
      }
      if (leave == 0) {
        const uint32_t dense_so_far =
            __hip_atomic_load(a.filter_ctrl + kCtrlDense, __ATOMIC_RELAXED, __HIP_MEMORY_SCOPE_AGENT) +
            __hip_atomic_load(a.filter_ctrl + kCtrlLeft, __ATOMIC_RELAXED, __HIP_MEMORY_SCOPE_AGENT);
        const uint32_t finished = __hip_atomic_load(a.filter_ctrl + kCtrlFinished, __ATOMIC_RELAXED,
                                                    __HIP_MEMORY_SCOPE_AGENT);
        if (finished >= 512 && 2 * dense_so_far > finished) {
          leave = 1;
          __hip_atomic_store(a.filter_ctrl + kCtrlAllLeave, 1u, __ATOMIC_RELAXED,
                             __HIP_MEMORY_SCOPE_AGENT);
          __hip_atomic_store(a.filter_ctrl + kCtrlGate, 1u, __ATOMIC_RELAXED,
                             __HIP_MEMORY_SCOPE_AGENT);
        }
      }
      verdict[0] = leave;
    }
    if (a.rotate == 1 && threadIdx.x < kPosSlots) {
      const uint32_t x = wg & 7;
      const unsigned long long said = __hip_atomic_load(
          reinterpret_cast<const unsigned long long *>(a.filter_ctrl + kCtrlPos) + x * kPosSlots +
              threadIdx.x,
          __ATOMIC_RELAXED, __HIP_MEMORY_SCOPE_AGENT);
      const uint32_t ticks16 = __hip_atomic_load(a.filter_ctrl + kCtrlStepTicks + x,
                                                 __ATOMIC_RELAXED, __HIP_MEMORY_SCOPE_AGENT);
      uint32_t pos = (uint32_t)(said >> 32);
      const uint32_t ago = (uint32_t)__builtin_amdgcn_s_memrealtime() - (uint32_t)said;
      if (said != 0 && ticks16 != 0 && ago < 16384u)
        pos += ago * 16u / ticks16;
      verdict[1 + threadIdx.x] = pos;
    }
    __syncthreads();
    const bool give_up = verdict[0] != 0;
    if (a.rotate == 1) {
#pragma unroll
      for (uint32_t k = 0; k < kPosSlots; ++k) xcd_pos = max(xcd_pos, verdict[1 + k]);
    }
    __syncthreads();
    if (give_up) {
      if (threadIdx.x == 0)
        __hip_atomic_fetch_add(a.filter_totals + kTotalDense, 4ull, __ATOMIC_RELAXED,
                               __HIP_MEMORY_SCOPE_AGENT);
      return 0;
    }
  }
  xcd_pos = __builtin_amdgcn_readfirstlane(xcd_pos);
  const uint32_t g = lane >> 5;
  const uint32_t lr = lane & 31;
  uint32_t lane16 = lane * 16;
  const uint32_t s_stride = a.geo.s_stride;
  const uint32_t all_steps = a.geo.k_words / (4 * kUnits);
  const uint32_t k_first = __builtin_amdgcn_readfirstlane(
      split ? part * all_steps / a.fsplit_parts : 0u);
  const uint32_t num_steps = __builtin_amdgcn_readfirstlane(
      split ? (part + 1) * all_steps / a.fsplit_parts - k_first : all_steps);
  const uint4 *g_rows = a.t2 + (uint64_t)tr * kT;
  const uint4 *g_cols = a.t2 + a.geo.col_base + (uint64_t)tc * kT;

  uint32_t mT;
  asm volatile("s_mov_b32 %0, 0xcccccccc" : "=s"(mT));

  const uint32_t dma_side = wave >> 1, dma_h = wave & 1;
  const uint32_t row_bytes = s_stride * 16;
  const char *const g_wave = reinterpret_cast<const char *>(
      (dma_side ? g_cols : g_rows) + ((uint64_t)2 * kUnits * k_first + kUnits * dma_h) * s_stride);
  const uint32_t l_wave = (uint32_t)(uintptr_t)(lds_void_ptr)(
      lds + ((dma_side * 2 + dma_h) * kUnits) * kSliceU4);
  struct Addr { const char *src; uint32_t dst; };
  const uint32_t kstep_bytes = 2 * kUnits * row_bytes;
  const char *seg_src = g_wave;
  uint32_t seg_steps = num_steps;
  uint32_t seg_wrap = 0xFFFFFFFFu;
  auto addr_of = [&](uint32_t step, uint32_t buf) {
    Addr pa;
    if (step >= seg_steps) step = seg_steps - 1;
    const int32_t rel = (int32_t)step - (int32_t)(step >= seg_wrap ? all_steps : 0u);
    pa.src = seg_src + (int64_t)rel * (int64_t)kstep_bytes;
    pa.dst = l_wave + buf * (kStageU4 * 16);
    asm volatile("" : "+s"(pa.src), "+s"(pa.dst));
    return pa;
  };
  auto addr_next = [&](const Addr &cur, uint32_t step, uint32_t buf) {
    Addr pa;
    const int32_t adv = (int32_t)(step < seg_steps ? 1u : 0u) -
                        (int32_t)(step == seg_wrap ? all_steps : 0u);
    pa.src = cur.src + (int64_t)adv * (int64_t)kstep_bytes;
    pa.dst = l_wave + buf * (kStageU4 * 16);
    asm volatile("" : "+s"(pa.src), "+s"(pa.dst));
    return pa;
  };
#define F_ISSUE4(PA, C)                                                        \
  {                                                                            \
    const char *src_ = (PA).src + (C) * row_bytes;                             \
    const uint32_t dst_ = (PA).dst + (C) * (kSliceU4 * 16);                    \
    F_ISSUE(src_, dst_, 0);                                                    \
    F_ISSUE(src_, dst_, 1024);                                                 \
    F_ISSUE(src_, dst_, 2048);                                                 \
    F_ISSUE(src_, dst_, 3072);                                                 \
  }

  v16f acc[4][4];
#pragma unroll
  for (int bi = 0; bi < 4; ++bi)
#pragma unroll
    for (int bj = 0; bj < 4; ++bj)
#pragma unroll
      for (int r = 0; r < 16; ++r) acc[bi][bj][r] = 0.f;

  uint32_t row_off = ((0 * 2 + g) * kUnits) * kSliceU4 + wy * 128 + lr;
  uint32_t col_off = ((1 * 2 + g) * kUnits) * kSliceU4 + wx * 128 + lr;
  asm volatile("" : "+v"(row_off), "+v"(col_off), "+v"(lane16));
  v8i FA[2][4], FB[2][4];
  uint4 RAW[8];
#define F_READ(K, BUF, C)                                                      \
  RAW[K] = lds[(BUF) * kStageU4 + ((K) < 4 ? row_off : col_off) + (C) * kSliceU4 + ((K) & 3) * 32];
#define F_PIN4(W) asm volatile("" : "+v"((W).x), "+v"((W).y), "+v"((W).z), "+v"((W).w));
#define F_PINF(F) asm volatile("" : "+v"((F)[0]), "+v"((F)[1]), "+v"((F)[2]), "+v"((F)[3]));
#define F_BUILD_B(NXT, K)                                                      \
  F_PIN4(RAW[K])                                                               \
  if ((K) < 4) {                                                               \
    FA[NXT][(K) & 3] = tfrag(RAW[K], mT);                                      \
    F_PINF(FA[NXT][(K) & 3])                                                   \
  } else {                                                                     \
    FB[NXT][(K) & 3] = tfrag(RAW[K], mT);                                      \
    F_PINF(FB[NXT][(K) & 3])                                                   \
  }
#define F_BUILD_A(NXT, K)                                                      \
  F_PIN4(RAW[K])                                                               \
  if ((K) < 4) {                                                               \
    FA[NXT][(K) & 3] = tfrag(shl2(RAW[K]), mT);                                \
    F_PINF(FA[NXT][(K) & 3])                                                   \
  } else {                                                                     \
    FB[NXT][(K) & 3] = tfrag(shl2(RAW[K]), mT);                                \
    F_PINF(FB[NXT][(K) & 3])                                                   \
  }
#define F_MMA(CUR, BI, BJ) acc[BI][BJ] = mma(FA[CUR][BI], FB[CUR][BJ], acc[BI][BJ]);
#define F_BAR __builtin_amdgcn_sched_barrier(0);
#define F_SLICE_B(CUR, NXT, PA, DC, OFF0, OFF1)                                \
  {                                                                            \
    const char *src_ = (PA).src + (DC) * row_bytes;                            \
    const uint32_t dst_ = (PA).dst + (DC) * (kSliceU4 * 16);                   \
    F_ISSUE(src_, dst_, OFF0);                                                 \
    F_MMA(CUR, 0, 0) F_BAR                                                     \
    F_BUILD_A(NXT, 0) F_MMA(CUR, 0, 1) F_BAR                                   \
    F_MMA(CUR, 0, 2) F_BAR                                                     \
    F_BUILD_A(NXT, 1) F_MMA(CUR, 0, 3) F_BAR                                   \
    F_MMA(CUR, 1, 0) F_BAR                                                     \
    F_BUILD_A(NXT, 2) F_MMA(CUR, 1, 1) F_BAR                                   \
    F_MMA(CUR, 1, 2) F_BAR                                                     \
    F_BUILD_A(NXT, 3) F_MMA(CUR, 1, 3) F_BAR                                   \
    F_ISSUE(src_, dst_, OFF1);                                                 \
    F_MMA(CUR, 2, 0) F_BAR                                                     \
    F_BUILD_A(NXT, 4) F_MMA(CUR, 2, 1) F_BAR                                   \
    F_MMA(CUR, 2, 2) F_BAR                                                     \
    F_BUILD_A(NXT, 5) F_MMA(CUR, 2, 3) F_BAR                                   \
    F_MMA(CUR, 3, 0) F_BAR                                                     \
    F_BUILD_A(NXT, 6) F_MMA(CUR, 3, 1) F_BAR                                   \
    F_MMA(CUR, 3, 2) F_BAR                                                     \
    F_BUILD_A(NXT, 7) F_MMA(CUR, 3, 3) F_BAR                                   \
  }
#define F_SLICE_A(CUR, NXT, RBUF, RC, SYNC, PA, DC, OFF0, OFF1)                \
  {                                                                            \
    if (SYNC) {                                                                \
      __builtin_amdgcn_s_waitcnt(vmcnt_imm(kSyncVm));                          \
      __syncthreads();                                                         \
    }                                                                          \
    const char *src_ = (PA).src + (DC) * row_bytes;                            \
    const uint32_t dst_ = (PA).dst + (DC) * (kSliceU4 * 16);                   \
    F_READ(0, RBUF, RC) F_READ(1, RBUF, RC)                                    \
    F_ISSUE(src_, dst_, OFF0);                                                 \
    F_MMA(CUR, 0, 0) F_MMA(CUR, 0, 1) F_BAR                                    \
    F_READ(2, RBUF, RC) F_READ(3, RBUF, RC)                                    \
    F_MMA(CUR, 0, 2) F_MMA(CUR, 0, 3) F_BAR                                    \
    F_READ(4, RBUF, RC) F_READ(5, RBUF, RC)                                    \
    F_ISSUE(src_, dst_, OFF1);                                                 \
    F_MMA(CUR, 1, 0) F_MMA(CUR, 1, 1) F_BAR                                    \
    F_READ(6, RBUF, RC) F_READ(7, RBUF, RC)                                    \
    F_MMA(CUR, 1, 2) F_MMA(CUR, 1, 3) F_BAR                                    \
    F_BUILD_B(NXT, 0) F_MMA(CUR, 2, 0) F_BAR                                   \
    F_BUILD_B(NXT, 1) F_MMA(CUR, 2, 1) F_BAR                                   \
    F_BUILD_B(NXT, 2) F_MMA(CUR, 2, 2) F_BAR                                   \
    F_BUILD_B(NXT, 3) F_MMA(CUR, 2, 3) F_BAR                                   \
    F_BUILD_B(NXT, 4) F_MMA(CUR, 3, 0) F_BAR                                   \
    F_BUILD_B(NXT, 5) F_MMA(CUR, 3, 1) F_BAR                                   \
    F_BUILD_B(NXT, 6) F_MMA(CUR, 3, 2) F_BAR                                   \
    F_BUILD_B(NXT, 7) F_MMA(CUR, 3, 3) F_BAR                                   \
  }
#define F_KSTEP                                                                \
  {                                                                            \
    const uint32_t nbuf = buf == kStages - 1 ? 0 : buf + 1;                    \
    F_SLICE_B(0, 1, pa, 0, 0, 1024)                                            \
    F_SLICE_A(1, 0, buf, 1, false, pa, 0, 2048, 3072)                          \
    F_SLICE_B(0, 1, pa, 1, 0, 1024)                                            \
    F_SLICE_A(1, 0, nbuf, 0, true, pa, 1, 2048, 3072)                          \
    pa = addr_next(pa, step + kStages, buf);                                   \
    buf = nbuf;                                                                \
    ++step;                                                                    \
  }

  uint32_t chk0 = 0, chk1 = 0, entry1 = 0, share1 = 0;
  uint32_t phase = 0, k0 = 0, wrap = 0, start_abs = 0;
  if (!split && a.check_steps != nullptr && a.tile_done != nullptr) {
    if (a.rotate != 0 && all_steps >= a.rotate_min_steps) {
      uint32_t base = 0;
      if (a.rotate == 1) {
        const uint32_t r = xcd_pos % all_steps;
        base = xcd_pos - r;
        phase = (r * kNumPhases + all_steps / 2) / all_steps;
        if (phase >= kNumPhases) {
          phase = 0;
          base += all_steps;
        }
      } else if (a.rotate == 2) {
        phase = (bid * 37u + 11u) & (kNumPhases - 1);
      } else {
        phase = (a.rotate - 3u) & (kNumPhases - 1);
      }
      k0 = phase_step(all_steps, phase);
      start_abs = base + k0;
      wrap = k0 != 0 ? all_steps - k0 : 0u;
    }
    float kappa = -1.f;
    {
      const float ns = (float)a.cohort_sums[0], nm = (float)a.cohort_sums[1],
                  nh = (float)a.cohort_sums[2];
      if (ns > 0.f && nh > 0.f) {
        const float sites = 256.f * (float)all_steps;
        const float m = nm / (ns * sites), h = nh / (ns * sites);
        kappa = m * (1.f + m / (2.f * h * (1.f - m))) + 4.6f * rsqrtf(sites) + 0.003f;
      }
    }
    auto steps_of = [&](uint32_t share) {
      const uint32_t hi = phase + share * kPhasesPerShare;
      return hi <= kNumPhases ? phase_step(all_steps, hi) - k0
                              : (all_steps - k0) + phase_step(all_steps, hi - kNumPhases);
    };
    if ((a.check0 == 2 || (a.check0 == 1 && kappa > 0.7f * a.kin_threshold)) &&
        a.check_steps[0] != 0)
      chk0 = steps_of(kCheckShares64[0]);
    const uint32_t sw1 = a.check1 & 0xFFu;
    if (sw1 >= 2) {
      entry1 = sw1 - 2;
    } else if (sw1 == 1 && kappa >= 0.f) {
      const float f64 = 64.f * (1.f - 2.f * a.kin_threshold) / (1.f - 2.f * kappa);
      if (f64 <= 62.f) {
        share1 = (uint32_t)ceilf(f64);
        if (share1 < 32) share1 = 32;
        entry1 = 1;
      }
    }
#pragma unroll
    for (uint32_t k = 1; k < kNumCheckShares; ++k)
      if (sw1 >= 2 && k == entry1) share1 = kCheckShares64[k];
    if (share1 != 0 && a.check_steps[entry1] != 0) chk1 = steps_of(share1);
    if (chk0 >= num_steps) chk0 = 0;
    if (chk1 >= num_steps || chk1 <= chk0) chk1 = 0;
  }
  chk0 = __builtin_amdgcn_readfirstlane(chk0);
  chk1 = __builtin_amdgcn_readfirstlane(chk1);
  share1 = __builtin_amdgcn_readfirstlane(share1);
  phase = __builtin_amdgcn_readfirstlane(phase);
  k0 = __builtin_amdgcn_readfirstlane(k0);
  wrap = __builtin_amdgcn_readfirstlane(wrap);
  start_abs = __builtin_amdgcn_readfirstlane(start_abs);
  auto prefix_u_of = [&](uint32_t share, size_t idx, float total) {
    const uint32_t hi = phase + share * kPhasesPerShare;
    const uint32_t xb = hi > kNumPhases ? hi - kNumPhases : hi;
    float u = hi > kNumPhases ? total : 0.f;
    if (xb == kNumPhases)
      u += total;
    else if (xb != 0)
      u += a.prefix_u[(size_t)(xb - 1) * s_stride + idx];
    if (phase != 0) u -= a.prefix_u[(size_t)(phase - 1) * s_stride + idx];
    return u;
  };
  unsigned long long *const pos_word =
      reinterpret_cast<unsigned long long *>(a.filter_ctrl + kCtrlPos) +
      (wg & 7) * kPosSlots + ((wg >> 3) & (kPosSlots - 1));
  uint32_t *const ticks_word = a.filter_ctrl + kCtrlStepTicks + (wg & 7);
  const uint32_t t_start = a.rotate == 1 ? (uint32_t)__builtin_amdgcn_s_memrealtime() : 0u;
#define F_PUBLISH(STEPS)                                                       \
  if (a.rotate == 1 && wave == 0) {                                            \
    const uint32_t now_ = (uint32_t)__builtin_amdgcn_s_memrealtime();          \
    const unsigned long long val_ =                                            \
        ((unsigned long long)(start_abs + (STEPS)) << 32) | now_;              \
     \
    const uint32_t t16_ = (STEPS) >= 32 ? (now_ - t_start) * 16u / (STEPS) : 0u; \
    const uint32_t zero_ = 0;                                                  \
    unsigned long long save_;                                                  \
    asm volatile("s_mov_b64 %0, exec\n\t"                                      \
                 "s_mov_b64 exec, 1\n\t"                                       \
                 "global_store_dwordx2 %1, %2, %3\n\t"                         \
                 "s_mov_b64 exec, %0"                                          \
                 : "=&s"(save_)                                                \
                 : "v"(zero_), "v"(val_), "s"(pos_word)                        \
                 : "memory");                                                  \
    if (t16_ != 0)                                                             \
      asm volatile("s_mov_b64 %0, exec\n\t"                                    \
                   "s_mov_b64 exec, 1\n\t"                                     \
                   "global_store_dword %1, %2, %3\n\t"                         \
                   "s_mov_b64 exec, %0"                                        \
                   : "=&s"(save_)                                              \
                   : "v"(zero_), "v"(t16_), "s"(ticks_word)                    \
                   : "memory");                                                \
  }

  uint32_t seg_first = 0;
  bool left = false, left_forecast = false, left_emit = false;
#pragma nounroll
  while (true) {
    uint32_t seg_end = num_steps;
    if (chk1 > seg_first) seg_end = chk1;
    if (chk0 > seg_first) seg_end = chk0;
    seg_end = __builtin_amdgcn_readfirstlane(seg_end);
    seg_steps = seg_end - seg_first;
    const uint32_t seg_k = seg_first >= wrap && wrap != 0 ? seg_first - wrap : k0 + seg_first;
    seg_src = g_wave + (uint64_t)seg_k * kstep_bytes;
    seg_wrap = __builtin_amdgcn_readfirstlane(
        wrap > seg_first && wrap < seg_end ? wrap - seg_first : 0xFFFFFFFFu);
    asm volatile("" : "+s"(seg_src), "+s"(seg_steps), "+s"(seg_wrap));

#pragma unroll
    for (int st = 0; st < kStages - 1; ++st) {
      const Addr p0 = addr_of(st, st);
      F_ISSUE4(p0, 0)
      F_ISSUE4(p0, 1)
    }
    __builtin_amdgcn_s_waitcnt(vmcnt_imm((kStages - 2) * kStageReqs));
    __syncthreads();
#pragma unroll
    for (int k = 0; k < 8; ++k) {
      F_READ(k, 0, 0)
    }
#pragma unroll
    for (int k = 0; k < 8; ++k) {
      F_BUILD_B(0, k)
    }
    uint32_t buf = 0;
    Addr pa = addr_of(kStages - 1, kStages - 1);
    uint32_t step = 0;
    while (step + 1 < seg_steps) {
      F_KSTEP
      F_KSTEP
    }
    if (step < seg_steps) F_KSTEP
    __builtin_amdgcn_s_waitcnt(0x0F70);
    __syncthreads();
    F_PUBLISH(seg_end)
    if (seg_end == num_steps) break;

    const bool forecast = seg_end == chk0;
    const float scale = forecast ? (float)kCheckShares64[0] * (1.f / 64.f) : 1.f;
    float2 *const ck_rows = reinterpret_cast<float2 *>(lds);
    float2 *const ck_cols = ck_rows + kT;
    uint32_t *const ck_words = reinterpret_cast<uint32_t *>(ck_cols + kT);
    {
      const uint32_t share = forecast ? kCheckShares64[0] : share1;
      const float thr_f = forecast ? a.kin_threshold + 3.66f * rsqrtf(256.f * (float)all_steps)
                                   : a.kin_threshold;
      const float t = 2.f - 4.f * thr_f;
      const size_t ir = (size_t)tr * kT + threadIdx.x;
      const size_t ic = (size_t)a.geo.col_base + (size_t)tc * kT + threadIdx.x;
      const float2 sr = a.sample_stats[ir], sc = a.sample_stats[ic];
      ck_rows[threadIdx.x] = make_float2(prefix_u_of(share, ir, sr.x), scale * fmaf(t, sr.y, 8.f));
      ck_cols[threadIdx.x] = make_float2(prefix_u_of(share, ic, sc.x), scale * fmaf(t, sc.y, 8.f));
    }
    __syncthreads();
    const uint32_t emit_cap = (a.check1 >> 8) & 0xFFu;
    uint32_t cnt = 0;
    {
      float2 cc[4];
#pragma unroll
      for (int bj = 0; bj < 4; ++bj) cc[bj] = ck_cols[wx * 128 + bj * 32 + lr];
#pragma unroll
      for (int bi = 0; bi < 4; ++bi)
#pragma unroll
        for (int r = 0; r < 16; ++r) {
          const float2 cr = ck_rows[wy * 128 + bi * 32 + (r & 3) + 8 * (r >> 2) + 4 * g];
#pragma unroll
          for (int bj = 0; bj < 4; ++bj)
            cnt += fmaf(-0.5f, acc[bi][bj][r], cr.x + cc[bj].x) < fminf(cr.y, cc[bj].y) ? 1u : 0u;
        }
    }
#pragma unroll
    for (int off = 32; off > 0; off >>= 1) cnt += __shfl_xor(cnt, off);
    if (lane == 0)
      ck_words[wave] = forecast ? (cnt > 2 * a.quadrant_cap ? 1u : 0u)
                                : (cnt > emit_cap ? emit_cap + 1 : cnt);
    __syncthreads();
    uint32_t found = forecast ? ck_words[0] + ck_words[1] + ck_words[2] + ck_words[3]
                              : max(max(ck_words[0], ck_words[1]), max(ck_words[2], ck_words[3]));
    found = __builtin_amdgcn_readfirstlane(found);
    __syncthreads();
    if (forecast ? found >= 3 : found <= emit_cap) {
      left = true;
      left_forecast = forecast;
      left_emit = !forecast && found != 0;
      break;
    }
    seg_first = seg_end;
  }
#undef F_KSTEP
#undef F_SLICE_A
#undef F_SLICE_B
#undef F_BAR
#undef F_MMA
#undef F_BUILD_A
#undef F_BUILD_B
#undef F_PIN4
#undef F_PINF
#undef F_READ
#undef F_ISSUE4
#undef F_PUBLISH
  if (left && left_emit && threadIdx.x == 0)
    __hip_atomic_fetch_add(a.filter_totals + kTotalEarly, 1ull, __ATOMIC_RELAXED,
                           __HIP_MEMORY_SCOPE_AGENT);
  if (phase != 0 && threadIdx.x == 0)
    __hip_atomic_fetch_add(a.filter_totals + kTotalRotated, 1ull, __ATOMIC_RELAXED,
                           __HIP_MEMORY_SCOPE_AGENT);
  if (left && !left_emit) {
    if (threadIdx.x == 0) {
      __hip_atomic_fetch_add(a.filter_ctrl + kCtrlFinished, 4u, __ATOMIC_RELAXED,
                             __HIP_MEMORY_SCOPE_AGENT);
      if (left_forecast) {
        __hip_atomic_fetch_add(a.filter_ctrl + kCtrlLeft, 4u, __ATOMIC_RELAXED,
                               __HIP_MEMORY_SCOPE_AGENT);
        __hip_atomic_store(a.filter_ctrl + kCtrlGate, 1u, __ATOMIC_RELAXED,
                           __HIP_MEMORY_SCOPE_AGENT);
        __hip_atomic_fetch_add(
            a.filter_totals + kTotalDense, 4ull,
            __ATOMIC_RELAXED, __HIP_MEMORY_SCOPE_AGENT);
      } else {
        a.tile_done[bid] = 1;
        __hip_atomic_fetch_add(
            a.filter_totals + kTotalEarly, 1ull,
            __ATOMIC_RELAXED, __HIP_MEMORY_SCOPE_AGENT);
      }
    }
    return 0;
  }

  if (!split && a.tile_done != nullptr && threadIdx.x == 0) a.tile_done[bid] = 1;

  if (split) {
    typedef uint32_t v4u __attribute__((ext_vector_type(4)));
    constexpr uint32_t kSlabU4 = 64 * 256;
    {
      const __amdgpu_buffer_rsrc_t rsrc = __builtin_amdgcn_make_buffer_rsrc(
          a.fsplit_slabs + (size_t)piece * kSlabU4, 0, (int)(kSlabU4 * 16), 0x00020000);
#pragma unroll
      for (int bi = 0; bi < 4; ++bi)
#pragma unroll
        for (int bj = 0; bj < 4; ++bj)
#pragma unroll
          for (int r4 = 0; r4 < 4; ++r4) {
            v4u v;
            v[0] = __float_as_uint(acc[bi][bj][4 * r4]);
            v[1] = __float_as_uint(acc[bi][bj][4 * r4 + 1]);
            v[2] = __float_as_uint(acc[bi][bj][4 * r4 + 2]);
            v[3] = __float_as_uint(acc[bi][bj][4 * r4 + 3]);
            __builtin_amdgcn_raw_buffer_store_b128(
                v, rsrc, (int)((((bi * 4 + bj) * 4 + r4) * 256 + threadIdx.x) * 16), 0,
                16 );
          }
    }
    asm volatile("s_waitcnt vmcnt(0)" ::: "memory");
    __syncthreads();
    uint32_t *flag = reinterpret_cast<uint32_t *>(lds);
    if (threadIdx.x == 0) {
      uint32_t *counter = a.fsplit_tickets + piece / a.fsplit_parts;
      const uint32_t ticket = __hip_atomic_fetch_add(counter, 1u, __ATOMIC_RELAXED,
                                                     __HIP_MEMORY_SCOPE_AGENT);
      const bool last = ticket == a.fsplit_parts - 1;
      if (last) {
        __builtin_amdgcn_fence(__ATOMIC_ACQUIRE, "agent");
        asm volatile("s_waitcnt vmcnt(0)" ::: "memory");
        *counter = 0;
      }
      *flag = last ? 1u : 0u;
    }
    __syncthreads();
    const bool last = *flag != 0;
    __syncthreads();
    if (!last) return 0;
    const uint32_t first_piece = piece - part;
    for (uint32_t p = 0; p < a.fsplit_parts; ++p) {
      if (p == part) continue;
      const float4 *src = a.fsplit_slabs + (size_t)(first_piece + p) * kSlabU4 + threadIdx.x;
#pragma unroll
      for (int bi = 0; bi < 4; ++bi)
#pragma unroll
        for (int bj = 0; bj < 4; ++bj)
#pragma unroll
          for (int r4 = 0; r4 < 4; ++r4) {
            const float4 v = src[((bi * 4 + bj) * 4 + r4) * 256];
            acc[bi][bj][4 * r4] += v.x;
            acc[bi][bj][4 * r4 + 1] += v.y;
            acc[bi][bj][4 * r4 + 2] += v.z;
            acc[bi][bj][4 * r4 + 3] += v.w;
          }
    }
  }

  float2 *const st_rows = reinterpret_cast<float2 *>(lds);
  float2 *const st_cols = st_rows + kT;
  {
    const float t = 2.f - 4.f * a.kin_threshold;
    const size_t ir = (size_t)tr * kT + threadIdx.x;
    const size_t ic = (size_t)a.geo.col_base + (size_t)tc * kT + threadIdx.x;
    float2 r = a.sample_stats[ir];
    float2 c = a.sample_stats[ic];
    if (left_emit) {
      r.x = prefix_u_of(share1, ir, r.x);
      c.x = prefix_u_of(share1, ic, c.x);
    }
    r.y = fmaf(t, r.y, 8.f);
    c.y = fmaf(t, c.y, 8.f);
    st_rows[threadIdx.x] = r;
    st_cols[threadIdx.x] = c;
  }
  __syncthreads();
  float2 sc[4];
#pragma unroll
  for (int bj = 0; bj < 4; ++bj) sc[bj] = st_cols[wx * 128 + bj * 32 + lr];

  {
    float best = -1.f;
#pragma unroll
    for (int bi = 0; bi < 4; ++bi)
#pragma unroll
      for (int r = 0; r < 16; ++r) {
        const float2 sr = st_rows[wy * 128 + bi * 32 + (r & 3) + 8 * (r >> 2) + 4 * g];
#pragma unroll
        for (int bj = 0; bj < 4; ++bj)
          best = fmaxf(best, fminf(sr.y, sc[bj].y) -
                                 fmaf(-0.5f, acc[bi][bj][r], sr.x + sc[bj].x));
      }
    if (__ballot(best > 0.f) == 0) {
      if (lane == 0)
        __hip_atomic_fetch_add(a.filter_ctrl + kCtrlFinished, 1u, __ATOMIC_RELAXED, __HIP_MEMORY_SCOPE_AGENT);
      return 0;
    }
  }
  if (lane == 0)
    __hip_atomic_fetch_add(a.filter_ctrl + kCtrlFinished, 1u, __ATOMIC_RELAXED, __HIP_MEMORY_SCOPE_AGENT);

  uint32_t total = 0, base = 0, run = 0;
#pragma nounroll
  for (int pass = 0; pass < 2; ++pass) {
    uint32_t tr_p = tr, tc_p = tc;
    asm volatile("" : "+s"(tr_p), "+s"(tc_p));
#pragma unroll
    for (int bi = 0; bi < 4; ++bi) {
#pragma unroll
      for (int r = 0; r < 16; ++r) {
        const uint32_t row = wy * 128 + bi * 32 + (r & 3) + 8 * (r >> 2) + 4 * g;
        const float2 sr = st_rows[row];
        const uint32_t li = tr_p * kT + row;
#pragma unroll
        for (int bj = 0; bj < 4; ++bj) {
          const uint32_t lj = tc_p * kT + wx * 128 + bj * 32 + lr;
          const bool valid = li < a.geo.num_rows && lj < a.geo.num_cols &&
                             a.i_begin + li < a.j_begin + lj;
          const float x_lb = fmaf(-0.5f, acc[bi][bj][r], sr.x + sc[bj].x);
          const bool cand = valid && x_lb < fminf(sr.y, sc[bj].y);
          const unsigned long long b = __ballot(cand);
          if (b != 0) {
            if (pass == 0) {
              total += (uint32_t)__popcll(b);
            } else {
              const uint32_t before = __builtin_amdgcn_mbcnt_hi(
                  (uint32_t)(b >> 32), __builtin_amdgcn_mbcnt_lo((uint32_t)b, 0u));
              if (cand) a.cand_list[base + run + before] = make_uint2(li, lj);
              run += (uint32_t)__popcll(b);
            }
          }
        }
      }
    }
    if (pass == 0) {
      if (total == 0) break;
      bool dense = total > a.quadrant_cap;
      if (!dense) {
        uint32_t got = 0;
        if (lane == 0) {
          got = __hip_atomic_fetch_add(a.filter_ctrl, total, __ATOMIC_RELAXED,
                                       __HIP_MEMORY_SCOPE_AGENT);
          __hip_atomic_fetch_add(a.filter_totals + kTotalCand,
                                 (unsigned long long)total, __ATOMIC_RELAXED,
                                 __HIP_MEMORY_SCOPE_AGENT);
        }
        base = (uint32_t)__builtin_amdgcn_readfirstlane(got);
        if (base >= a.cand_cap || total > a.cand_cap - base) {
          for (uint32_t k = base + lane; k < a.cand_cap; k += 64)
            a.cand_list[k] = make_uint2(kNoPair, kNoPair);
          dense = true;
        }
      }
      if (dense) {
        if (lane == 0) {
          const uint32_t slot = __hip_atomic_fetch_add(a.filter_ctrl + kCtrlDense, 1u, __ATOMIC_RELAXED,
                                                       __HIP_MEMORY_SCOPE_AGENT);
          if (slot < a.dense_cap) a.dense_list[slot] = make_uint2(2 * tr + wy, 2 * tc + wx);
          __hip_atomic_fetch_add(a.filter_totals + kTotalDense, 1ull,
                                 __ATOMIC_RELAXED, __HIP_MEMORY_SCOPE_AGENT);
        }
        break;
      }
    }
  }
  return 0;
}

__global__ __launch_bounds__(256, 1) void king_filter_kernel(const TiledArgs a) {
  extern __shared__ uint4 lds[];
  (void)filter_tile(a, blockIdx.x, lds);
}

__global__ __launch_bounds__(256) void king_refine_kernel(const TiledArgs a) {
  const uint32_t lane = threadIdx.x & 63;
  uint32_t count = *a.filter_ctrl;
  if (count > a.cand_cap) count = a.cand_cap;
  const uint32_t n = a.words_per_sample / 2;
  const uint32_t stride = gridDim.x * 4;
  for (uint32_t p = blockIdx.x * 4 + (threadIdx.x >> 6); p < count; p += stride) {
    const uint2 e = a.cand_list[p];
    if (e.x == kNoPair) continue;
    const uint32_t off_i = a.perm != nullptr ? a.perm[e.x] : e.x;
    const uint32_t off_j = a.perm != nullptr ? a.perm[a.geo.col_base + e.y]
                                             : (a.geo.diag ? e.y : a.geo.num_rows + e.y);
    const uint64_t *het_i_w = a.bits + (uint64_t)off_i * a.words_per_sample;
    const uint64_t *alt_i_w = het_i_w + n;
    const uint64_t *het_j_w = a.bits + (uint64_t)off_j * a.words_per_sample;
    const uint64_t *alt_j_w = het_j_w + n;
    uint32_t s_het_i = 0, s_het_j = 0, s_both = 0, s_opp = 0, s_conc = 0, s_shared = 0;
    constexpr uint32_t kAhead = 8;
    for (uint32_t w0 = 0; w0 < n; w0 += 64 * kAhead) {
      uint64_t hi[kAhead], ai[kAhead], hj[kAhead], aj[kAhead];
#pragma unroll
      for (uint32_t k = 0; k < kAhead; ++k) {
        const uint32_t w = w0 + 64 * k + lane;
        const bool in = w < n;
        hi[k] = in ? het_i_w[w] : ~0ull;
        ai[k] = in ? alt_i_w[w] : ~0ull;
        hj[k] = in ? het_j_w[w] : ~0ull;
        aj[k] = in ? alt_j_w[w] : ~0ull;
      }
#pragma unroll
      for (uint32_t k = 0; k < kAhead; ++k) {
        const uint64_t ri = ~(hi[k] | ai[k]), rj = ~(hj[k] | aj[k]);
        const uint64_t defined = ~((hi[k] & ai[k]) | (hj[k] & aj[k]));
        s_het_i += __popcll(hi[k] & defined);
        s_het_j += __popcll(hj[k] & defined);
        s_both += __popcll(hi[k] & hj[k] & defined);
        s_opp += __popcll(((ri & aj[k]) | (ai[k] & rj)) & defined);
        s_conc += __popcll(((ri & rj) | (ai[k] & aj[k])) & defined);
        s_shared += __popcll(defined);
      }
    }
#pragma unroll
    for (int off = 32; off > 0; off >>= 1) {
      s_het_i += __shfl_xor(s_het_i, off);
      s_het_j += __shfl_xor(s_het_j, off);
      s_both += __shfl_xor(s_both, off);
      s_opp += __shfl_xor(s_opp, off);
      s_conc += __shfl_xor(s_conc, off);
      s_shared += __shfl_xor(s_shared, off);
    }
    if (lane == 0) {
      const float kin = king_kinship(s_het_i, s_het_j, s_both, s_opp);
      if (kin > a.kin_threshold) {
        const uint32_t ibs0 = s_opp, ibs2 = s_conc + s_both;
        const uint32_t gi = a.i_begin + off_i;
        const uint32_t gj = a.geo.diag ? a.j_begin + off_j : a.j_begin + (off_j - a.geo.num_rows);
        emit_result(gi < gj ? gi : gj, gi < gj ? gj : gi, kin, ibs0, s_shared - ibs0 - ibs2, ibs2,
                    a.max_results, a.results, a.result_index, a.result_overflow);
      }
    }
  }
}

}

static std::atomic<uint32_t> g_check_min_steps{64};
void set_filter_check_min_steps(uint32_t steps) { g_check_min_steps.store(steps); }
uint32_t filter_check_min_steps() { return g_check_min_steps.load(); }

hipError_t launch_sample_stats(const uint64_t *d_bit_sets, uint32_t words_per_sample,
                               const PlaneGeometry &geo, uint4 *d_planes, uint32_t s_begin,
                               uint32_t s_end, hipStream_t stream) {
  if (s_end > geo.s_stride) s_end = geo.s_stride;
  if (s_begin >= s_end) return hipSuccess;
  float2 *stats = plane_tmp_stats(d_planes, geo);
  float *prefix = plane_tmp_prefix(d_planes, geo);
  unsigned long long *sums = const_cast<unsigned long long *>(plane_cohort_sums(d_planes, geo));
  uint32_t *steps = const_cast<uint32_t *>(plane_check_steps(d_planes, geo));
  CheckWords cw;
  const uint32_t all_steps = geo.k_words / 8;
  if (all_steps > kStatsMaxSteps) return hipErrorInvalidValue;
  for (uint32_t k = 0; k < kNumCheckShares; ++k)
    cw.w[k] = check_step_of(all_steps, k, g_check_min_steps.load());
  sample_stats_kernel<<<dim3((s_end - s_begin + 3) / 4), dim3(256), 0, stream>>>(
      d_bit_sets, words_per_sample, geo, stats, prefix, sums, steps, cw, s_begin, s_end);
  return hipGetLastError();
}

hipError_t launch_filter(const TiledArgs &args, uint64_t num_tiles, hipStream_t stream) {
  if ((uint64_t)args.geo.k_words * 32 > kMfmaN4MaxSites || args.filter_ctrl == nullptr ||
      args.cand_list == nullptr || args.dense_list == nullptr || args.sample_stats == nullptr)
    return hipErrorInvalidValue;
  static DeviceOnce attr_set;
  if (!attr_set.done()) {
    hipError_t e = hipFuncSetAttribute(reinterpret_cast<const void *>(king_filter_kernel),
                                       hipFuncAttributeMaxDynamicSharedMemorySize,
                                       (int)kFilterLdsBytes);
    if (e != hipSuccess) return e;
    attr_set.mark();
  }
  uint64_t cap = max_blocks_per_launch(256);
  if (cap > kFilterChunkTiles) cap = kFilterChunkTiles;
  if (cap > args.dense_cap / 4) cap = args.dense_cap / 4;
  if (cap == 0) return hipErrorInvalidValue;
  const uint32_t wgs = args.split_wgs != 0 ? args.split_wgs : 256;
  uint64_t done = 0;
  while (done < num_tiles) {
    const uint64_t n = num_tiles - done < cap ? num_tiles - done : cap;
    const bool checks = args.tile_done != nullptr;
    hipError_t e = hipMemsetAsync(args.filter_ctrl, 0, kCtrlChunkBytes + (checks ? n : 0), stream);
    if (e != hipSuccess) return e;
    TiledArgs a = args;
    a.tile_begin = args.tile_begin + done;
    a.quad = 0;
    a.tile_list = nullptr;
    a.gate = nullptr;
    a.skip_tiles = nullptr;
    a.check0 = !checks ? 0u : args.check0 == 2 ? 2u : (args.check0 == 1 && n < 16ull * wgs) ? 1u : 0u;
    a.check1 = checks ? args.check1 : 0u;
    a.rotate = checks && (n >= args.rotate_min_tiles || args.rotate >= 2) ? args.rotate : 0u;
    uint32_t rest = 0, parts = 0;
    if (args.fsplit_slabs != nullptr && args.fsplit_tickets != nullptr && n < 16ull * wgs) {
      rest = (uint32_t)(n % wgs);
      if (rest != 0 && 2 * rest <= wgs && rest <= kFilterSplitSlabs / 2) {
        parts = wgs / rest;
        if (parts > 8) parts = 8;
        if (parts * rest > kFilterSplitSlabs) parts = kFilterSplitSlabs / rest;
        const uint32_t min_steps = args.fsplit_first != 0 ? args.fsplit_first : 8;
        while (parts > 1 && args.geo.k_words / 8 / parts < min_steps) --parts;
      }
      if (parts < 2) rest = parts = 0;
    }
    const uint64_t n_whole = n - rest;
    uint64_t grid = n_whole;
    a.dyn_tiles = a.dyn_wgs = 0;
    if (args.xcd_chunk == 2 && args.dyn_tiles != 0 && n_whole >= args.dyn_tiles / 4 &&
        n_whole >= 288) {
      const uint64_t fixed = (n_whole - n_whole / 16) / 256 * 256;
      a.launch_tiles = (uint32_t)fixed;
      a.xcd_chunk = 1;
      a.dyn_tiles = (uint32_t)(n_whole - fixed);
      a.dyn_wgs = a.dyn_tiles + a.dyn_tiles / 2;
      grid = fixed + a.dyn_wgs;
    } else if (args.xcd_chunk == 2 && n_whole >= 64) {
      a.launch_tiles = (uint32_t)n_whole;
      a.xcd_chunk = 1;
      grid = 8ull * 32 * ((((n_whole + 31) / 32) + 7) / 8);
    } else {
      a.xcd_chunk = 0;
      a.launch_tiles = (uint32_t)n_whole;
    }
    a.fsplit_parts = parts;
    a.fsplit_tile0 = (uint32_t)n_whole;
    a.fsplit_first = (uint32_t)grid;
    grid += (uint64_t)rest * parts;
    if (checks && rest != 0) {
      e = hipMemsetAsync(args.tile_done + n_whole, 1, rest, stream);
      if (e != hipSuccess) return e;
    }
    king_filter_kernel<<<dim3((uint32_t)grid), dim3(256), kFilterLdsBytes, stream>>>(a);
    e = hipGetLastError();
    if (e != hipSuccess) return e;
    king_refine_kernel<<<dim3(wgs * 4), dim3(256), 0, stream>>>(a);
    e = hipGetLastError();
    if (e != hipSuccess) return e;
    if (a.codes_ready != nullptr) {
      e = launch_prepare_nibbles(true, false, a.bits, a.words_per_sample, a.geo,
                                 const_cast<uint4 *>(a.planes), a.perm, 0, 0xFFFFFFFFu,
                                 a.filter_ctrl, a.codes_ready, stream);
      if (e != hipSuccess) return e;
      e = launch_mark_codes_ready(a.filter_ctrl, a.codes_ready, stream);
      if (e != hipSuccess) return e;
    }
    TiledArgs d = a;
    d.tile_list = a.dense_list;
    d.tile_list_count = a.filter_ctrl + kCtrlDense;
    d.tile_list_cap = a.dense_cap;
    e = launch_mfma_list(d, wgs, stream);
    if (e != hipSuccess) return e;
    if (checks) {
      TiledArgs f = a;
      f.quad = 1;
      f.tile_begin = a.tile_begin * 4;
      f.gate = a.filter_ctrl + kCtrlGate;
      f.skip_tiles = a.tile_done;
      f.skip_base = a.tile_begin;
      e = launch_mfma_gated(f, n * 4, wgs, stream);
      if (e != hipSuccess) return e;
    }
    done += n;
  }
  return hipSuccess;
}

}
```

### cuking_amd/csrc/king_kernels.hip

```cpp
#include <hip/hip_runtime.h>

#include "king_common.h"
#include "king_device.h"

#pragma clang diagnostic ignored "-Winline-asm"

namespace cuking {

namespace {

constexpr int kPrepSamples = 64;
constexpr int kPrepWords = 16;

__global__ __launch_bounds__(256) void prepare_planes_kernel(
    const uint64_t *__restrict__ bits, uint32_t words_per_sample,
    PlaneGeometry geo, uint4 *__restrict__ planes, uint32_t s_tile_begin) {
  __shared__ uint64_t het_lds[kPrepSamples][kPrepWords + 1];
  __shared__ uint64_t hom_lds[kPrepSamples][kPrepWords + 1];

  const uint32_t plane_words = words_per_sample / 2;
  const uint32_t s0 = (s_tile_begin + blockIdx.x) * kPrepSamples;
  const uint32_t w0 = blockIdx.y * kPrepWords;

#pragma unroll
  for (int it = 0; it < kPrepSamples * kPrepWords / 256; ++it) {
    const uint32_t idx = it * 256 + threadIdx.x;
    const uint32_t s = idx / kPrepWords, w = idx % kPrepWords;
    const uint32_t ps = s0 + s;
    uint32_t src = 0xFFFFFFFFu;
    if (geo.diag || ps < geo.rows_padded) {
      if (ps < geo.num_rows) src = ps;
    } else {
      const uint32_t c = ps - geo.col_base;
      if (c < geo.num_cols) src = geo.num_rows + c;
    }
    uint64_t het = ~0ull, hom = ~0ull;
    if (src != 0xFFFFFFFFu && w0 + w < plane_words) {
      const uint64_t *p = bits + (uint64_t)src * words_per_sample + (w0 + w);
      het = p[0];
      hom = p[plane_words];
    }
    het_lds[s][w] = het;
    hom_lds[s][w] = hom;
  }
  __syncthreads();

#pragma unroll
  for (int it = 0; it < kPrepSamples * kPrepWords * 2 / 256; ++it) {
    const uint32_t idx = it * 256 + threadIdx.x;
    const uint32_t krow = idx / kPrepSamples, s = idx % kPrepSamples;
    const uint32_t k = w0 * 2 + krow;
    if (k >= geo.k_words || s0 + s >= geo.s_stride) continue;
    const uint32_t shift = (krow & 1) * 32;
    const uint32_t het = (uint32_t)(het_lds[s][krow >> 1] >> shift);
    const uint32_t hom = (uint32_t)(hom_lds[s][krow >> 1] >> shift);
    uint4 v;
    v.x = het & ~hom;
    v.y = hom & ~het;
    v.z = ~het;
    v.w = ~(het & hom);
    planes[(uint64_t)k * geo.s_stride + s0 + s] = v;
  }
}

__global__ __launch_bounds__(256) void prepare_quads_kernel(
    const uint64_t *__restrict__ bits, uint32_t words_per_sample,
    PlaneGeometry geo, uint4 *__restrict__ planes, uint32_t s_tile_begin) {
  __shared__ uint64_t het_lds[kPrepSamples][kPrepWords + 1];
  __shared__ uint64_t hom_lds[kPrepSamples][kPrepWords + 1];

  const uint32_t plane_words = words_per_sample / 2;
  const uint32_t s0 = (s_tile_begin + blockIdx.x) * kPrepSamples;
  const uint32_t w0 = blockIdx.y * kPrepWords;

#pragma unroll
  for (int it = 0; it < kPrepSamples * kPrepWords / 256; ++it) {
    const uint32_t idx = it * 256 + threadIdx.x;
    const uint32_t s = idx / kPrepWords, w = idx % kPrepWords;
    const uint32_t ps = s0 + s;
    uint32_t src = 0xFFFFFFFFu;
    if (geo.diag || ps < geo.rows_padded) {
      if (ps < geo.num_rows) src = ps;
    } else {
      const uint32_t c = ps - geo.col_base;
      if (c < geo.num_cols) src = geo.num_rows + c;
    }
    uint64_t het = ~0ull, hom = ~0ull;
    if (src != 0xFFFFFFFFu && w0 + w < plane_words) {
      const uint64_t *p = bits + (uint64_t)src * words_per_sample + (w0 + w);
      het = p[0];
      hom = p[plane_words];
    }
    het_lds[s][w] = het;
    hom_lds[s][w] = hom;
  }
  __syncthreads();

  constexpr int kQuads = kPrepWords / 2;
#pragma unroll
  for (int it = 0; it < kQuads * 2 * kPrepSamples / 256; ++it) {
    const uint32_t idx = it * 256 + threadIdx.x;
    const uint32_t s = idx % kPrepSamples;
    const uint32_t p = (idx / kPrepSamples) % 2;
    const uint32_t ql = idx / (kPrepSamples * 2);
    const uint32_t q = w0 / 2 + ql;
    if (q * 4 >= geo.k_words || s0 + s >= geo.s_stride) continue;
    const uint64_t lo = p ? hom_lds[s][2 * ql] : het_lds[s][2 * ql];
    const uint64_t hi = p ? hom_lds[s][2 * ql + 1] : het_lds[s][2 * ql + 1];
    uint4 v;
    v.x = (uint32_t)lo;
    v.y = (uint32_t)(lo >> 32);
    v.z = (uint32_t)hi;
    v.w = (uint32_t)(hi >> 32);
    planes[((uint64_t)q * 2 + p) * geo.s_stride + s0 + s] = v;
  }
}

__device__ __forceinline__ uint32_t spread8(uint32_t b) {
  uint32_t x = b & 0xFFu;
  x = (x | (x << 12)) & 0x000F000Fu;
  x = (x | (x << 6)) & 0x03030303u;
  x = (x | (x << 3)) & 0x11111111u;
  return x;
}

constexpr int kNibWords = 32;

template <bool CODES, bool T2>
__global__ __launch_bounds__(256) void prepare_nibbles_kernel(
    const uint64_t *__restrict__ bits, uint32_t words_per_sample,
    PlaneGeometry geo, uint4 *__restrict__ planes, uint32_t s_tile_begin,
    const uint32_t *__restrict__ perm, const uint32_t *__restrict__ gate,
    const uint32_t *__restrict__ ready) {
  __shared__ uint64_t het_lds[kPrepSamples][kNibWords + 1];
  __shared__ uint64_t hom_lds[kPrepSamples][kNibWords + 1];
  if (gate != nullptr && ((gate[kCtrlGate] | gate[kCtrlDense]) == 0 || *ready != 0)) return;

  const uint32_t plane_words = words_per_sample / 2;
  const uint32_t s0 = (s_tile_begin + blockIdx.x) * kPrepSamples;
  const uint32_t w0 = blockIdx.y * kNibWords;
  const bool wide = (plane_words & 1) == 0 && (words_per_sample & 1) == 0 &&
                    (reinterpret_cast<uintptr_t>(bits) & 15) == 0;

#pragma unroll
  for (int it = 0; it < kPrepSamples * kNibWords / 2 / 256; ++it) {
    const uint32_t idx = it * 256 + threadIdx.x;
    const uint32_t s = idx / (kNibWords / 2), w = (idx % (kNibWords / 2)) * 2;
    const uint32_t ps = s0 + s;
    uint32_t src = 0xFFFFFFFFu;
    if (perm != nullptr) {
      if (ps < geo.s_stride) src = perm[ps];
    } else if (geo.diag || ps < geo.rows_padded) {
      if (ps < geo.num_rows) src = ps;
    } else {
      const uint32_t c = ps - geo.col_base;
      if (c < geo.num_cols) src = geo.num_rows + c;
    }
    uint64_t het[2] = {~0ull, ~0ull}, hom[2] = {~0ull, ~0ull};
    if (src != 0xFFFFFFFFu && w0 + w < plane_words) {
      const uint64_t *p = bits + (uint64_t)src * words_per_sample + (w0 + w);
      if (wide && w0 + w + 1 < plane_words) {
        const ulonglong2 a = *reinterpret_cast<const ulonglong2 *>(p);
        const ulonglong2 b = *reinterpret_cast<const ulonglong2 *>(p + plane_words);
        het[0] = a.x; het[1] = a.y;
        hom[0] = b.x; hom[1] = b.y;
      } else {
        het[0] = p[0];
        hom[0] = p[plane_words];
        if (w0 + w + 1 < plane_words) {
          het[1] = p[1];
          hom[1] = p[plane_words + 1];
        }
      }
    }
    het_lds[s][w] = het[0];
    het_lds[s][w + 1] = het[1];
    hom_lds[s][w] = hom[0];
    hom_lds[s][w + 1] = hom[1];
  }
  __syncthreads();

  if constexpr (CODES) {
#pragma unroll
  for (int it = 0; it < kPrepSamples * kNibWords * 2 / 256; ++it) {
    const uint32_t idx = it * 256 + threadIdx.x;
    const uint32_t krow = idx / kPrepSamples, s = idx % kPrepSamples;
    const uint32_t k = w0 * 2 + krow;
    if (k >= geo.k_words || s0 + s >= geo.s_stride) continue;
    const uint32_t shift = (krow & 1) * 32;
    const uint32_t het = (uint32_t)(het_lds[s][krow >> 1] >> shift);
    const uint32_t hom = (uint32_t)(hom_lds[s][krow >> 1] >> shift);
    uint32_t out[4];
#pragma unroll
    for (int d = 0; d < 4; ++d) {
      const uint32_t hs = spread8(het >> (8 * d)), ms = spread8(hom >> (8 * d));
      const uint32_t H = hs & ~ms;
      const uint32_t D = 0x11111111u ^ (hs & ms);
      const uint32_t Y = 0x11111111u ^ hs;
      const uint32_t A = ms & ~hs;
      out[d] = H | (D << 1) | (Y << 2) | (A << 3);
    }
    planes[(uint64_t)k * geo.s_stride + s0 + s] = make_uint4(out[0], out[1], out[2], out[3]);
  }
  uint4 *hetq = planes + (uint64_t)geo.k_words * geo.s_stride;
  constexpr int kQuads = kNibWords / 2;
#pragma unroll
  for (int it = 0; it < kQuads * kPrepSamples / 256; ++it) {
    const uint32_t idx = it * 256 + threadIdx.x;
    const uint32_t s = idx % kPrepSamples, ql = idx / kPrepSamples;
    const uint32_t q = w0 / 2 + ql;
    if (q * 4 >= geo.k_words || s0 + s >= geo.s_stride) continue;
    const uint64_t lo = het_lds[s][2 * ql], hi = het_lds[s][2 * ql + 1];
    hetq[(uint64_t)q * geo.s_stride + s0 + s] =
        make_uint4((uint32_t)lo, (uint32_t)(lo >> 32), (uint32_t)hi, (uint32_t)(hi >> 32));
  }
  }
  if constexpr (T2) {
    uint4 *t2 = const_cast<uint4 *>(plane_t2(planes, geo));
#pragma unroll
    for (int it = 0; it < kNibWords * kPrepSamples / 256; ++it) {
      const uint32_t idx = it * 256 + threadIdx.x;
      const uint32_t s = idx % kPrepSamples, ul = idx / kPrepSamples;
      const uint32_t u = w0 + ul;
      if (u * 2 >= geo.k_words || s0 + s >= geo.s_stride) continue;
      const uint64_t het = het_lds[s][ul], hom = hom_lds[s][ul];
      uint32_t out[4];
#pragma unroll
      for (int d = 0; d < 4; ++d) {
        const uint32_t h_lo = (uint32_t)(het >> (8 * d)), m_lo = (uint32_t)(hom >> (8 * d));
        const uint32_t h_hi = (uint32_t)(het >> (32 + 8 * d)), m_hi = (uint32_t)(hom >> (32 + 8 * d));
        const uint32_t y_lo = spread8(~h_lo), a_lo = spread8(m_lo & ~h_lo);
        const uint32_t y_hi = spread8(~h_hi), a_hi = spread8(m_hi & ~h_hi);
        out[d] = (a_lo << 3) | (y_lo << 2) | (a_hi << 1) | y_hi;
      }
      t2[(uint64_t)u * geo.s_stride + s0 + s] = make_uint4(out[0], out[1], out[2], out[3]);
    }
  }
}

template <int TIT, int TJT, int RI, int RJ, int KC, int KU, int MINW, bool FULL,
          bool PHASED = false>
__global__ __launch_bounds__(TIT *TJT, MINW) void king_tiled_kernel(
    const TiledArgs a) {
  constexpr int TILE = TIT * RI;
  static_assert(TILE == TJT * RJ, "square tiles only");
  constexpr int NT = TIT * TJT;
  constexpr int NW = NT / 64;
  constexpr int SEG = TILE / 64;
  constexpr int WAVE_ROWS = 2 * KC * SEG;
  static_assert(WAVE_ROWS % NW == 0, "rows must split evenly over waves");
  constexpr int PER_WAVE = WAVE_ROWS / NW;

  extern __shared__ uint4 lds[];

  const uint64_t t = a.tile_begin + blockIdx.x;
  uint32_t tr, tc;
  if (!decode_tile(a, t, &tr, &tc)) return;

  const uint32_t lane = threadIdx.x & 63;
  const uint32_t wave = __builtin_amdgcn_readfirstlane(threadIdx.x >> 6);
  const uint32_t ti = threadIdx.x % TIT;
  const uint32_t tj = threadIdx.x / TIT;

  const uint4 *g_rows = a.planes + (uint64_t)tr * TILE;
  const uint4 *g_cols = a.planes + a.geo.col_base + (uint64_t)tc * TILE;
  const uint32_t s_stride = a.geo.s_stride;
  const uint32_t num_chunks = a.geo.k_words / KC;

  auto issue_chunk = [&](uint32_t chunk, uint32_t buf) {
#pragma unroll
    for (int r = 0; r < PER_WAVE; ++r) {
      const uint32_t wr = wave * PER_WAVE + r;
      const uint32_t side = wr / (KC * SEG);
      const uint32_t rem = wr % (KC * SEG);
      const uint32_t kc = rem / SEG, seg = rem % SEG;
      const uint4 *src = (side ? g_cols : g_rows) +
                         (uint64_t)(chunk * KC + kc) * s_stride + seg * 64 +
                         lane;
      uint4 *dst = lds + ((buf * 2 + side) * KC + kc) * TILE + seg * 64;
      if (PHASED) {
        const uint32_t lds_addr = (uint32_t)(uintptr_t)(lds_void_ptr)dst;
        asm volatile(
            "s_mov_b32 m0, %0\n\t"
            "s_nop 0\n\t"
            "global_load_lds_dwordx4 %1, off"
            :
            : "s"(lds_addr), "v"(src)
            : "memory", "m0");
      } else {
        __builtin_amdgcn_global_load_lds((global_void_ptr)src, (lds_void_ptr)dst,
                                         16, 0, 0);
      }
    }
  };

  uint32_t c_hh[RI][RJ], c_opp[RI][RJ], c_bh[RI][RJ], c_hi[RI][RJ],
      c_hj[RI][RJ];
#pragma unroll
  for (int x = 0; x < RI; ++x)
#pragma unroll
    for (int y = 0; y < RJ; ++y)
      c_hh[x][y] = c_opp[x][y] = c_bh[x][y] = c_hi[x][y] = c_hj[x][y] = 0;

  issue_chunk(0, 0);
  for (uint32_t chunk = 0; chunk < num_chunks; ++chunk) {
    const uint32_t buf = chunk & 1;
    __builtin_amdgcn_s_waitcnt(0x0F70);
    __syncthreads();
    if (chunk + 1 < num_chunks) issue_chunk(chunk + 1, buf ^ 1);

    const uint4 *l_rows = lds + (buf * 2 + 0) * KC * TILE;
    const uint4 *l_cols = lds + (buf * 2 + 1) * KC * TILE;
    if (PHASED) {
      uint4 ri[RI], cj[RJ];
#pragma unroll
      for (int x = 0; x < RI; ++x) ri[x] = l_rows[x * TIT + ti];
#pragma unroll
      for (int y = 0; y < RJ; ++y) cj[y] = l_cols[y * TJT + tj];
#pragma unroll KU
      for (int kc = 0; kc < KC; ++kc) {
        uint32_t v_opp[RI][RJ], v_bh[RI][RJ], v_hi[RI][RJ], v_hj[RI][RJ],
            v_hh[RI][RJ];
#pragma unroll
        for (int x = 0; x < RI; ++x) {
#pragma unroll
          for (int y = 0; y < RJ; ++y) {
            const uint32_t hom_both = ri[x].z & cj[y].z;
            v_hh[x][y] = hom_both;
            v_opp[x][y] =
                __builtin_amdgcn_bitop3_b32(ri[x].y, cj[y].y, hom_both, 0x28);
            v_bh[x][y] = ri[x].x & cj[y].x;
            v_hi[x][y] = ri[x].x & cj[y].w;
            v_hj[x][y] = ri[x].w & cj[y].x;
          }
        }
        if (kc + 1 < KC) {
#pragma unroll
          for (int x = 0; x < RI; ++x) ri[x] = l_rows[(kc + 1) * TILE + x * TIT + ti];
#pragma unroll
          for (int y = 0; y < RJ; ++y) cj[y] = l_cols[(kc + 1) * TILE + y * TJT + tj];
        }
        __builtin_amdgcn_sched_barrier(0);
        __builtin_amdgcn_sched_barrier(0);
#pragma unroll
        for (int x = 0; x < RI; ++x) {
#pragma unroll
          for (int y = 0; y < RJ; ++y) {
            if (FULL)
              asm("v_bcnt_u32_b32 %0, %1, %0" : "+v"(c_hh[x][y]) : "v"(v_hh[x][y]));
            asm("v_bcnt_u32_b32 %0, %1, %0" : "+v"(c_opp[x][y]) : "v"(v_opp[x][y]));
            asm("v_bcnt_u32_b32 %0, %1, %0" : "+v"(c_bh[x][y]) : "v"(v_bh[x][y]));
            asm("v_bcnt_u32_b32 %0, %1, %0" : "+v"(c_hi[x][y]) : "v"(v_hi[x][y]));
            asm("v_bcnt_u32_b32 %0, %1, %0" : "+v"(c_hj[x][y]) : "v"(v_hj[x][y]));
          }
        }
        __builtin_amdgcn_sched_barrier(0);
        __builtin_amdgcn_s_barrier();
        __builtin_amdgcn_sched_barrier(0);
      }
      continue;
    }
#pragma unroll KU
    for (int kc = 0; kc < KC; ++kc) {
      uint4 ri[RI], cj[RJ];
#pragma unroll
      for (int x = 0; x < RI; ++x) ri[x] = l_rows[kc * TILE + x * TIT + ti];
#pragma unroll
      for (int y = 0; y < RJ; ++y) cj[y] = l_cols[kc * TILE + y * TJT + tj];
#pragma unroll
      for (int x = 0; x < RI; ++x) {
#pragma unroll
        for (int y = 0; y < RJ; ++y) {
          const uint32_t hom_both = ri[x].z & cj[y].z;
          if (FULL) c_hh[x][y] += __builtin_popcount(hom_both);
          c_opp[x][y] += __builtin_popcount(
              __builtin_amdgcn_bitop3_b32(ri[x].y, cj[y].y, hom_both, 0x28));
          c_bh[x][y] += __builtin_popcount(ri[x].x & cj[y].x);
          c_hi[x][y] += __builtin_popcount(ri[x].x & cj[y].w);
          c_hj[x][y] += __builtin_popcount(ri[x].w & cj[y].x);
        }
      }
    }
  }

  const EmitCtx emit_ctx = make_emit_ctx(a);
#pragma unroll
  for (int x = 0; x < RI; ++x) {
    const uint32_t li = tr * TILE + x * TIT + ti;
#pragma unroll
    for (int y = 0; y < RJ; ++y) {
      const uint32_t lj = tc * TILE + y * TJT + tj;
      const bool valid = li < a.geo.num_rows && lj < a.geo.num_cols &&
                         a.i_begin + li < a.j_begin + lj;
      if (FULL)
        full_epilogue_pair(a, valid, li, lj, c_hi[x][y], c_hj[x][y], c_bh[x][y],
                           c_opp[x][y], c_hh[x][y]);
      else
        lean_epilogue_pair(emit_ctx, valid, li, lj, c_hi[x][y], c_hj[x][y],
                           c_bh[x][y], c_opp[x][y], lane);
    }
  }
}

__global__ __launch_bounds__(256) void king_stream_kernel(
    const cuking_submatrix sm, const uint32_t words_per_sample,
    const uint64_t *__restrict__ bits, const float kin_threshold,
    const uint32_t max_results, cuking_result *results, uint32_t *result_index,
    uint32_t *result_overflow, cuking_counts *dense_counts,
    const uint64_t block_offset) {
  const uint32_t lane = threadIdx.x & 63;
  const uint32_t wave = threadIdx.x >> 6;
  const uint32_t num_cols = sm_num_cols(sm);
  const uint32_t col_groups = (num_cols + 3) / 4;
  const uint64_t b = block_offset + blockIdx.x;
  const uint32_t li = (uint32_t)(b / col_groups);
  const uint32_t lj = (uint32_t)(b % col_groups) * 4 + wave;
  const uint32_t i = sm.i_begin + li, j = sm.j_begin + lj;
  if (lj >= num_cols || i >= j) return;

  const uint32_t n = words_per_sample / 2;
  const uint64_t *het_i_w =
      bits + (uint64_t)sm_sample_offset(sm, i) * words_per_sample;
  const uint64_t *alt_i_w = het_i_w + n;
  const uint64_t *het_j_w =
      bits + (uint64_t)sm_sample_offset(sm, j) * words_per_sample;
  const uint64_t *alt_j_w = het_j_w + n;

  uint32_t s_het_i = 0, s_het_j = 0, s_both = 0, s_opp = 0, s_conc = 0,
           s_shared = 0;
  for (uint32_t k = lane; k < n; k += 64) {
    const uint64_t hi = het_i_w[k], ai = alt_i_w[k];
    const uint64_t hj = het_j_w[k], aj = alt_j_w[k];
    const uint64_t ri = ~(hi | ai), rj = ~(hj | aj);
    const uint64_t defined = ~((hi & ai) | (hj & aj));
    s_het_i += __popcll(hi & defined);
    s_het_j += __popcll(hj & defined);
    s_both += __popcll(hi & hj & defined);
    s_opp += __popcll(((ri & aj) | (ai & rj)) & defined);
    s_conc += __popcll(((ri & rj) | (ai & aj)) & defined);
    s_shared += __popcll(defined);
  }
#pragma unroll
  for (int off = 32; off > 0; off >>= 1) {
    s_het_i += __shfl_xor(s_het_i, off);
    s_het_j += __shfl_xor(s_het_j, off);
    s_both += __shfl_xor(s_both, off);
    s_opp += __shfl_xor(s_opp, off);
    s_conc += __shfl_xor(s_conc, off);
    s_shared += __shfl_xor(s_shared, off);
  }
  if (lane != 0) return;
  if (dense_counts != nullptr) {
    cuking_counts c;
    c.het_i = s_het_i;
    c.het_j = s_het_j;
    c.both_het = s_both;
    c.opposing_hom = s_opp;
    c.concordant_hom = s_conc;
    c.shared = s_shared;
    dense_counts[(uint64_t)li * num_cols + lj] = c;
    return;
  }
  const float kin = king_kinship(s_het_i, s_het_j, s_both, s_opp);
  if (kin > kin_threshold) {
    const uint32_t ibs0 = s_opp, ibs2 = s_conc + s_both;
    emit_result(i, j, kin, ibs0, s_shared - ibs0 - ibs2, ibs2, max_results,
                results, result_index, result_overflow);
  }
}

__global__ __launch_bounds__(256) void pack_kernel(
    const cuking_submatrix sm, const uint32_t words_per_sample,
    uint64_t *bit_set, const int64_t *__restrict__ row_idx,
    const int64_t *__restrict__ col_idx, const int32_t *__restrict__ n_alt,
    const uint64_t num_triples, uint32_t *status) {
  const uint32_t plane_words = words_per_sample / 2;
  const uint64_t plane_bits = (uint64_t)plane_words * 64;
  uint32_t bad = 0;
  for (uint64_t t = (uint64_t)blockIdx.x * blockDim.x + threadIdx.x;
       t < num_triples; t += (uint64_t)gridDim.x * blockDim.x) {
    const int64_t col = col_idx[t];
    if (col < 0 || col > 0xFFFFFFFFll || !sm_contains(sm, (uint32_t)col))
      continue;
    const int64_t row = row_idx[t];
    if (row < 0 || (uint64_t)row >= plane_bits) {
      bad |= 2u;
      continue;
    }
    unsigned long long *het = reinterpret_cast<unsigned long long *>(
        bit_set + (uint64_t)sm_sample_offset(sm, (uint32_t)col) *
                      words_per_sample);
    unsigned long long *hom = het + plane_words;
    const unsigned long long clear = ~(1ull << (row & 63));
    const uint64_t word = (uint64_t)row >> 6;
    const int32_t g = n_alt[t];
    if (g == 0) {
      atomicAnd(het + word, clear);
      atomicAnd(hom + word, clear);
    } else if (g == 1) {
      atomicAnd(hom + word, clear);
    } else if (g == 2) {
      atomicAnd(het + word, clear);
    } else {
      bad |= 1u;
    }
  }
  if (bad) atomicOr(status, bad);
}

__global__ __launch_bounds__(256) void pack_compact_kernel(
    const uint32_t words_per_sample, const uint32_t num_samples, uint64_t *bit_set,
    const uint32_t *__restrict__ site, const uint32_t *__restrict__ sample_alt,
    const uint64_t num_triples, uint32_t *status) {
  const uint32_t plane_words = words_per_sample / 2;
  const uint64_t plane_bits = (uint64_t)plane_words * 64;
  uint32_t bad = 0;
  for (uint64_t t = (uint64_t)blockIdx.x * blockDim.x + threadIdx.x;
       t < num_triples; t += (uint64_t)gridDim.x * blockDim.x) {
    const uint32_t sa = sample_alt[t], row = site[t];
    const uint32_t sample = sa & 0x3FFFFFFFu, g = sa >> 30;
    if (row >= plane_bits || sample >= num_samples) {
      bad |= 2u;
      continue;
    }
    unsigned long long *het = reinterpret_cast<unsigned long long *>(
        bit_set + (uint64_t)sample * words_per_sample);
    unsigned long long *hom = het + plane_words;
    const unsigned long long clear = ~(1ull << (row & 63));
    const uint32_t word = row >> 6;
    if (g == 0) {
      atomicAnd(het + word, clear);
      atomicAnd(hom + word, clear);
    } else if (g == 1) {
      atomicAnd(hom + word, clear);
    } else if (g == 2) {
      atomicAnd(het + word, clear);
    } else {
      bad |= 1u;
    }
  }
  if (bad) atomicOr(status, bad);
}

uint64_t g_max_blocks_override = 0;

template <int TIT, int TJT, int RI, int RJ, int KC, int KU, int MINW, bool FULL,
          bool PHASED = false>
hipError_t launch_variant(const TiledArgs &args, uint64_t num_tiles,
                          uint32_t lds_bytes, hipStream_t stream) {
  auto kernel = king_tiled_kernel<TIT, TJT, RI, RJ, KC, KU, MINW, FULL, PHASED>;
  static DeviceOnce attr_set;
  if (!attr_set.done()) {
    hipError_t e = hipFuncSetAttribute(
        reinterpret_cast<const void *>(kernel),
        hipFuncAttributeMaxDynamicSharedMemorySize, (int)lds_bytes);
    if (e != hipSuccess) return e;
    attr_set.mark();
  }
  const uint64_t cap = max_blocks_per_launch(TIT * TJT);
  uint64_t done = 0;
  while (done < num_tiles) {
    const uint64_t n = (num_tiles - done < cap) ? num_tiles - done : cap;
    TiledArgs a = args;
    a.tile_begin = args.tile_begin + done;
    kernel<<<dim3((uint32_t)n), dim3(TIT * TJT), lds_bytes, stream>>>(a);
    hipError_t e = hipGetLastError();
    if (e != hipSuccess) return e;
    done += n;
  }
  return hipSuccess;
}

const TiledVariant kVariants[kNumTiledVariants] = {
    {"t64_r4x2_k16_phased", 64, 16, 512, 2 * 2 * 16 * 64 * 16, kLayoutWord},
    {"t64_r4x4_k8_w4", 64, 8, 256, 2 * 2 * 8 * 64 * 16, kLayoutWord},
    {"t128_r8x4_k8_w2", 128, 8, 512, 2 * 2 * 8 * 128 * 16, kLayoutWord},
    {"t128_r4x4_k8_w4", 128, 8, 1024, 2 * 2 * 8 * 128 * 16, kLayoutWord},
    {"t64_r4x4_k16_w4", 64, 16, 256, 2 * 2 * 16 * 64 * 16, kLayoutWord},
    {"t128_mfma_fp4", 128, 8, 256, kMfmaLdsBytes, kLayoutQuad},
    {"t128_mfma_fp4_n4", 128, 8, 256, kMfmaN4LdsBytes, kLayoutNibble},
    {"t256_mfma_fp4_filter", kFilterTile, 8, 256, kFilterLdsBytes, kLayoutNibbleStats},
};


}

void set_max_blocks_per_launch(uint64_t blocks) { g_max_blocks_override = blocks; }
uint64_t max_blocks_override() { return g_max_blocks_override; }

uint64_t max_blocks_per_launch(uint32_t threads) {
  const uint64_t hw = 0xFFFFFFFFull / threads;
  return (g_max_blocks_override && g_max_blocks_override < hw) ? g_max_blocks_override : hw;
}

const TiledVariant &tiled_variant(int v) { return kVariants[v]; }

hipError_t launch_tiled(int variant, bool full, const TiledArgs &args,
                        uint64_t num_tiles, hipStream_t stream) {
  if (num_tiles == 0) return hipSuccess;
  const uint32_t lds = kVariants[variant].lds_bytes;
#define CUKING_SHAPE(...)                                                      \
  (full ? launch_variant<__VA_ARGS__, true>(args, num_tiles, lds, stream)      \
        : launch_variant<__VA_ARGS__, false>(args, num_tiles, lds, stream))
  switch (variant) {
    case 0:
      return full ? launch_variant<16, 32, 4, 2, 16, 16, 4, true, true>(args, num_tiles, lds, stream)
                  : launch_variant<16, 32, 4, 2, 16, 16, 4, false, true>(args, num_tiles, lds, stream);
    case 1: return CUKING_SHAPE(16, 16, 4, 4, 8, 2, 4);
    case 2: return CUKING_SHAPE(16, 32, 8, 4, 8, 2, 2);
    case 3: return CUKING_SHAPE(32, 32, 4, 4, 8, 2, 4);
    case 4: return CUKING_SHAPE(16, 16, 4, 4, 16, 2, 4);
    case kMfmaVariant: return launch_mfma(full, false, args, num_tiles, lds, stream);
    case kMfmaN4Variant: return launch_mfma(full, true, args, num_tiles, lds, stream);
    case kMfmaFilterVariant: {
      const bool filter = !full && args.dense_counts == nullptr && args.quad == 0 &&
                          args.kin_threshold > 0.f && args.kin_threshold < 0.5f &&
                          args.filter_ctrl != nullptr;
      if (filter) return launch_filter(args, num_tiles, stream);
      TiledArgs a = args;
      if (a.quad == 0) {
        a.quad = 1;
        a.tile_begin = args.tile_begin * 4;
        num_tiles *= 4;
      }
      return launch_mfma(full, true, a, num_tiles, kMfmaN4LdsBytes, stream);
    }
    default: return hipErrorInvalidValue;
  }
#undef CUKING_SHAPE
}

hipError_t launch_prepare_planes(uint32_t layout, const uint64_t *d_bit_sets,
                                 uint32_t words_per_sample,
                                 const PlaneGeometry &geo, uint4 *d_planes,
                                 uint32_t s_tile_begin, uint32_t s_tile_end,
                                 hipStream_t stream) {
  const uint32_t all = (geo.s_stride + kPrepSamples - 1) / kPrepSamples;
  if (s_tile_end > all) s_tile_end = all;
  if (s_tile_begin >= s_tile_end) return hipSuccess;
  const bool nibble = layout == kLayoutNibble || layout == kLayoutNibbleStats;
  const uint32_t block_words = nibble ? kNibWords : kPrepWords;
  const dim3 grid(s_tile_end - s_tile_begin,
                  (geo.k_words + 2 * block_words - 1) / (2 * block_words));
  if (grid.y == 0) return hipSuccess;
  if (layout == kLayoutQuad)
    prepare_quads_kernel<<<grid, dim3(256), 0, stream>>>(
        d_bit_sets, words_per_sample, geo, d_planes, s_tile_begin);
  else if (layout == kLayoutNibbleStats)
    return hipErrorInvalidValue;
  else if (nibble)
    prepare_nibbles_kernel<true, false><<<grid, dim3(256), 0, stream>>>(
        d_bit_sets, words_per_sample, geo, d_planes, s_tile_begin, nullptr, nullptr, nullptr);
  else
    prepare_planes_kernel<<<grid, dim3(256), 0, stream>>>(
        d_bit_sets, words_per_sample, geo, d_planes, s_tile_begin);
  return hipGetLastError();
}

hipError_t launch_prepare_nibbles(bool codes, bool t2, const uint64_t *d_bit_sets,
                                  uint32_t words_per_sample, const PlaneGeometry &geo,
                                  uint4 *d_planes, const uint32_t *perm, uint32_t s_tile_begin,
                                  uint32_t s_tile_end, const uint32_t *gate,
                                  const uint32_t *ready, hipStream_t stream) {
  const uint32_t all = (geo.s_stride + kPrepSamples - 1) / kPrepSamples;
  if (s_tile_end > all) s_tile_end = all;
  if (s_tile_begin >= s_tile_end || (!codes && !t2)) return hipSuccess;
  const dim3 grid(s_tile_end - s_tile_begin, (geo.k_words + 2 * kNibWords - 1) / (2 * kNibWords));
  if (grid.y == 0) return hipSuccess;
  if (codes && t2)
    prepare_nibbles_kernel<true, true><<<grid, dim3(256), 0, stream>>>(
        d_bit_sets, words_per_sample, geo, d_planes, s_tile_begin, perm, gate, ready);
  else if (codes)
    prepare_nibbles_kernel<true, false><<<grid, dim3(256), 0, stream>>>(
        d_bit_sets, words_per_sample, geo, d_planes, s_tile_begin, perm, gate, ready);
  else
    prepare_nibbles_kernel<false, true><<<grid, dim3(256), 0, stream>>>(
        d_bit_sets, words_per_sample, geo, d_planes, s_tile_begin, perm, gate, ready);
  return hipGetLastError();
}

namespace {
__global__ void mark_codes_ready_kernel(const uint32_t *gate, uint32_t *ready) {
  if ((gate[kCtrlGate] | gate[kCtrlDense]) != 0) *ready = 1;
}
}

hipError_t launch_mark_codes_ready(const uint32_t *gate, uint32_t *ready, hipStream_t stream) {
  mark_codes_ready_kernel<<<dim3(1), dim3(1), 0, stream>>>(gate, ready);
  return hipGetLastError();
}

hipError_t launch_stream(const cuking_submatrix &sm, uint32_t words_per_sample,
                         const uint64_t *d_bit_sets, float kin_threshold,
                         uint32_t max_results, cuking_result *d_results,
                         uint32_t *d_result_index, uint32_t *d_result_overflow,
                         cuking_counts *d_dense_counts, hipStream_t stream) {
  const uint64_t rows = sm_num_rows(sm);
  const uint64_t col_groups = ((uint64_t)sm_num_cols(sm) + 3) / 4;
  const uint64_t blocks = rows * col_groups;
  const uint64_t cap = max_blocks_per_launch(256);
  for (uint64_t done = 0; done < blocks; done += cap) {
    const uint64_t n = blocks - done < cap ? blocks - done : cap;
    king_stream_kernel<<<dim3((uint32_t)n), dim3(256), 0, stream>>>(
        sm, words_per_sample, d_bit_sets, kin_threshold, max_results, d_results,
        d_result_index, d_result_overflow, d_dense_counts, done);
    const hipError_t e = hipGetLastError();
    if (e != hipSuccess) return e;
  }
  return hipSuccess;
}

hipError_t launch_pack(const cuking_submatrix &sm, uint32_t words_per_sample,
                       uint64_t *d_bit_set, const int64_t *d_row_idx,
                       const int64_t *d_col_idx, const int32_t *d_n_alt,
                       size_t num_triples, uint32_t *d_status,
                       hipStream_t stream) {
  if (num_triples == 0) return hipSuccess;
  uint64_t blocks = (num_triples + 255) / 256;
  if (blocks > 256 * 32) blocks = 256 * 32;
  pack_kernel<<<dim3((uint32_t)blocks), dim3(256), 0, stream>>>(
      sm, words_per_sample, d_bit_set, d_row_idx, d_col_idx, d_n_alt,
      num_triples, d_status);
  return hipGetLastError();
}

hipError_t launch_pack_compact(uint32_t words_per_sample, uint32_t num_samples,
                               uint64_t *d_bit_set, const uint32_t *d_site,
                               const uint32_t *d_sample_alt, size_t num_triples,
                               uint32_t *d_status, hipStream_t stream) {
  if (num_triples == 0) return hipSuccess;
  uint64_t blocks = (num_triples + 255) / 256;
  if (blocks > 256 * 32) blocks = 256 * 32;
  pack_compact_kernel<<<dim3((uint32_t)blocks), dim3(256), 0, stream>>>(
      words_per_sample, num_samples, d_bit_set, d_site, d_sample_alt, num_triples, d_status);
  return hipGetLastError();
}

}
```

### cuking_amd/csrc/king_sort.hip

```cpp
#include <hip/hip_runtime.h>

#include <hipcub/hipcub.hpp>

#include "king_common.h"

namespace cuking {

namespace {

__global__ void sort_keys_kernel(const float2 *__restrict__ tmp_stats, uint32_t begin, uint32_t n,
                                 float stored_sites, uint32_t *__restrict__ keys,
                                 uint32_t *__restrict__ vals) {
  const uint32_t p = blockIdx.x * blockDim.x + threadIdx.x;
  if (p >= n) return;
  const float2 st = tmp_stats[begin + p];
  const float missing = 0.5f * (stored_sites - st.y - st.x);
  uint32_t key = (uint32_t)(missing * 64.f / stored_sites);
  keys[p] = key > 255u ? 255u : key;
  vals[p] = begin + p;
}

__global__ void identity_order_kernel(uint32_t begin, uint32_t n, uint32_t *__restrict__ vals) {
  const uint32_t p = blockIdx.x * blockDim.x + threadIdx.x;
  if (p < n) vals[p] = begin + p;
}

__global__ void apply_order_kernel(PlaneGeometry geo, uint32_t begin, uint32_t end, uint32_t n,
                                   const uint32_t *__restrict__ order,
                                   const float2 *__restrict__ tmp_stats,
                                   const float *__restrict__ tmp_prefix,
                                   uint32_t *__restrict__ perm, float2 *__restrict__ stats,
                                   float *__restrict__ prefix) {
  const uint32_t p = begin + blockIdx.x * blockDim.x + threadIdx.x;
  if (p >= end) return;
  if (p - begin >= n) {
    perm[p] = kNoSample;
    stats[p] = make_float2(0.f, 0.f);
#pragma unroll
    for (uint32_t c = 0; c < kNumCum; ++c) prefix[(size_t)c * geo.s_stride + p] = 0.f;
    return;
  }
  const uint32_t src = order[p - begin];
  perm[p] = (geo.diag || src < geo.rows_padded) ? src : geo.num_rows + (src - geo.col_base);
  stats[p] = tmp_stats[src];
#pragma unroll 7
  for (uint32_t c = 0; c < kNumCum; ++c)
    prefix[(size_t)c * geo.s_stride + p] = tmp_prefix[(size_t)c * geo.s_stride + src];
}

}

size_t sort_temp_bytes_for(uint32_t n) {
  size_t bytes = 0;
  uint32_t *nil = nullptr;
  if (n == 0) return 0;
  (void)hipcub::DeviceRadixSort::SortPairs(nullptr, bytes, nil, nil, nil, nil, (int)n, 0, 8);
  return (bytes + 255) / 256 * 256;
}

hipError_t launch_sample_order(const PlaneGeometry &geo, uint32_t words_per_sample,
                               uint4 *d_planes, uint32_t s_begin, uint32_t s_end, bool sort,
                               void *sort_temp, size_t sort_temp_bytes, hipStream_t stream) {
  if (s_end > geo.s_stride) s_end = geo.s_stride;
  if (s_begin >= s_end) return hipSuccess;
  const float2 *tmp_stats = plane_tmp_stats(d_planes, geo);
  const float *tmp_prefix = plane_tmp_prefix(d_planes, geo);
  uint32_t *perm = plane_perm(d_planes, geo);
  float2 *stats = const_cast<float2 *>(plane_stats(d_planes, geo));
  float *prefix = const_cast<float *>(plane_prefix_u(d_planes, geo));
  uint32_t *words = plane_sort_words(d_planes, geo);
  const float stored_sites = 32.f * (float)words_per_sample;
  struct Side { uint32_t begin, end, real_end; };
  Side sides[2];
  int num_sides = 0;
  if (geo.diag) {
    sides[num_sides++] = {0, geo.rows_padded, geo.num_rows};
  } else {
    sides[num_sides++] = {0, geo.rows_padded, geo.num_rows};
    sides[num_sides++] = {geo.col_base, geo.col_base + geo.cols_padded, geo.col_base + geo.num_cols};
  }
  for (int k = 0; k < num_sides; ++k) {
    const uint32_t b = s_begin > sides[k].begin ? s_begin : sides[k].begin;
    const uint32_t e = s_end < sides[k].end ? s_end : sides[k].end;
    if (b >= e) continue;
    const uint32_t real_e = e < sides[k].real_end ? e : sides[k].real_end;
    const uint32_t n = real_e > b ? real_e - b : 0;
    uint32_t *keys_in = words + b, *keys_out = words + geo.s_stride + b;
    uint32_t *vals_in = words + 2 * (size_t)geo.s_stride + b;
    uint32_t *vals_out = words + 3 * (size_t)geo.s_stride + b;
    const uint32_t *order = vals_in;
    if (n != 0) {
      if (sort) {
        sort_keys_kernel<<<dim3((n + 255) / 256), dim3(256), 0, stream>>>(
            tmp_stats, b, n, stored_sites, keys_in, vals_in);
        hipError_t e0 = hipGetLastError();
        if (e0 != hipSuccess) return e0;
        size_t bytes = sort_temp_bytes;
        e0 = hipcub::DeviceRadixSort::SortPairs(sort_temp, bytes, keys_in, keys_out, vals_in,
                                                vals_out, (int)n, 0, 8, stream);
        if (e0 != hipSuccess) return e0;
        order = vals_out;
      } else {
        identity_order_kernel<<<dim3((n + 255) / 256), dim3(256), 0, stream>>>(b, n, vals_in);
        hipError_t e0 = hipGetLastError();
        if (e0 != hipSuccess) return e0;
      }
    }
    apply_order_kernel<<<dim3((e - b + 255) / 256), dim3(256), 0, stream>>>(
        geo, b, e, n, order, tmp_stats, tmp_prefix, perm, stats, prefix);
    hipError_t e1 = hipGetLastError();
    if (e1 != hipSuccess) return e1;
  }
  return hipSuccess;
}

}
```

Before: 37.19 billion.

## Reorder genotype sites by informativeness so the kinship filter can check early

Counts per site how many samples carry the relevant genotype, radix-sorts sites in descending order, and rebuilds the t2 planes in that site order. Per-phase cumulative mass is recorded so the filter kernel can cap its rotation span to a 'core' prefix of sites holding enough mass to decide the threshold early. The aim is to let more tile pairs be rejected after fewer k-steps. In exchange it adds prepare-time sort and permutation kernels, extra workspace, and more complex rotation and wrap logic in the filter kernel.

```diff
diff --git a/cuking_amd/csrc/king_abi.hip b/cuking_amd/csrc/king_abi.hip
--- a/cuking_amd/csrc/king_abi.hip
+++ b/cuking_amd/csrc/king_abi.hip
@@ -106,6 +106,8 @@
   uint32_t filter_rotate_min_steps = 128;
   uint32_t filter_rotate_min_tiles = 2048;
   int filter_sort = 1;
+  int filter_site_order = 1;
+  uint32_t filter_site_order_min_tiles = 2048;
   bool filter_lazy_codes = true;
   void *sort_temp = nullptr;
   size_t sort_temp_bytes = 0;
@@ -118,6 +120,7 @@
     uint32_t tile = 0;
     const uint64_t *bits = nullptr;
     bool codes = true;
+    bool site_ordered = false;
     std::vector<uint8_t> tiles;
     hipStream_t ordered_on = nullptr;
     bool ordered_valid = false;
@@ -358,6 +361,7 @@
   a.rotate_min_steps = ctx->filter_rotate_min_steps;
   a.rotate_min_tiles = ctx->filter_rotate_min_tiles;
   a.check_steps = plane_check_steps(ctx->planes, geo);
+  a.site_ctrl = plane_site_ctrl(ctx->planes, geo);
   return CUKING_OK;
 }
 
@@ -455,8 +459,13 @@
   const size_t prefix = ((size_t)tiles.num_bands() + 1) * sizeof(uint64_t);
   if (prefix > ctx->band_prefix_bytes) ctx->prefix_for = TileSpace{0, 0, 0, 0};
   st = grow(ctx, reinterpret_cast<void **>(&ctx->band_prefix), &ctx->band_prefix_bytes, prefix);
-  if (st != CUKING_OK || v.layout != kLayoutNibbleStats || ctx->filter_sort == 0) return st;
-  return grow(ctx, &ctx->sort_temp, &ctx->sort_temp_bytes, sort_temp_bytes_for(geo.s_stride));
+  if (st != CUKING_OK || v.layout != kLayoutNibbleStats) return st;
+  size_t temp = ctx->filter_sort != 0 ? sort_temp_bytes_for(geo.s_stride) : 0;
+  if (ctx->filter_site_order != 0 && site_order_fits(geo)) {
+    const size_t site_temp = site_sort_temp_bytes_for(geo.k_words * 32);
+    if (site_temp > temp) temp = site_temp;
+  }
+  return grow(ctx, &ctx->sort_temp, &ctx->sort_temp_bytes, temp);
 }
 
 bool same_tile_space(const TileSpace &a, const TileSpace &b) {
@@ -515,7 +524,8 @@
   const uint32_t t_end = s_tile_end < all_tiles ? s_tile_end : all_tiles;
   cuking_ctx::Prepared &pr = ctx->prepared;
   const bool new_prefix = !same_tile_space(ctx->prefix_for, tiles);
-  const bool same = same_block(pr, sm, words_per_sample, variant, v.tile, d_bit_sets);
+  bool same = same_block(pr, sm, words_per_sample, variant, v.tile, d_bit_sets);
+  if (same && pr.site_ordered && !(s_tile_begin == 0 && t_end == all_tiles)) same = false;
   if (ctx->reuse_prepared && same && !new_prefix) {
     bool all_there = true;
     for (uint32_t t = s_tile_begin; t < t_end && all_there; ++t) all_there = pr.tiles[t] != 0;
@@ -538,6 +548,7 @@
     pr.bits = d_bit_sets;
     pr.tiles.assign(all_tiles, 0);
     pr.codes = true;
+    pr.site_ordered = false;
   }
   for (uint32_t t = s_tile_begin; t < t_end; ++t)
     must_wait = must_wait || pr.tiles[t] == 2 || (pr.tiles[t] == 1 && other_stream);
@@ -562,13 +573,26 @@
       HIP_TRY(hipMemsetAsync(const_cast<unsigned long long *>(plane_cohort_sums(ctx->planes, geo)),
                              0, 64, stream));
     HIP_TRY(hipMemsetAsync(plane_flags(ctx->planes, geo), 0, sizeof(uint32_t), stream));
+    if (whole)
+      pr.site_ordered = ctx->filter_site_order != 0 && site_order_fits(geo) &&
+                        geo.k_words / 8 >= filter_check_min_steps() &&
+                        total_tiles(tiles) >= ctx->filter_site_order_min_tiles;
+    if (whole && pr.site_ordered)
+      HIP_TRY(launch_site_order(d_bit_sets, words_per_sample, geo, ctx->planes, ctx->sort_temp,
+                                ctx->sort_temp_bytes, stream));
+    else if (!pr.site_ordered)
+      HIP_TRY(hipMemsetAsync(plane_site_ctrl(ctx->planes, geo) + kSiteOn, 0, sizeof(uint32_t),
+                             stream));
     HIP_TRY(launch_sample_stats(d_bit_sets, words_per_sample, geo, ctx->planes, sb, se, stream));
     HIP_TRY(launch_sample_order(geo, words_per_sample, ctx->planes, sb, se,
                                 ctx->filter_sort == 2 || (ctx->filter_sort == 1 && whole),
                                 ctx->sort_temp, ctx->sort_temp_bytes, stream));
-    HIP_TRY(launch_prepare_nibbles(codes, true, d_bit_sets, words_per_sample, geo, ctx->planes,
-                                   plane_perm(ctx->planes, geo), s_tile_begin, t_end, nullptr,
-                                   nullptr, stream));
+    HIP_TRY(launch_prepare_nibbles(codes, !pr.site_ordered, d_bit_sets, words_per_sample, geo,
+                                   ctx->planes, plane_perm(ctx->planes, geo), s_tile_begin, t_end,
+                                   nullptr, nullptr, stream));
+    if (pr.site_ordered)
+      HIP_TRY(launch_prepare_t2_ordered(d_bit_sets, words_per_sample, geo, ctx->planes,
+                                        plane_perm(ctx->planes, geo), s_tile_begin, t_end, stream));
     if (!codes) {
       pr.codes = false;
     } else if (!pr.codes) {
@@ -672,6 +696,10 @@
      CTX_FIELD(filter_sort)},
     {"filter_lazy_codes", 0, 1, "filter_lazy_codes outside [0, 1]", 0, kInvalidatesLayout,
      CTX_FIELD(filter_lazy_codes)},
+    {"filter_site_order", 0, 1, "filter_site_order outside [0, 1]", 0, kInvalidatesLayout,
+     CTX_FIELD(filter_site_order)},
+    {"filter_site_order_min_tiles", 0, 1 << 30, "filter_site_order_min_tiles outside [0, 2^30]", 0,
+     kInvalidatesLayout, CTX_FIELD(filter_site_order_min_tiles)},
     {"filter_check0", 0, 2, "filter_check0 outside [0, 2]", 0, 0, CTX_FIELD(filter_check0)},
     {"filter_check1", 0, 1 + kNumCheckShares, "filter_check1 outside {0, 1, 3 .. %u}",
      1 + kNumCheckShares, 0, CTX_FIELD(filter_check1), 2},
@@ -722,7 +750,9 @@
   uint32_t word = 0;
   while (word < kNumTotals && strcmp(totals[word], key) != 0) ++word;
   const bool ticks = strcmp(key, "filter_step_ticks16") == 0;
-  if (word == kNumTotals && !ticks)
+  const bool core_share = strcmp(key, "filter_core_share") == 0;
+  if (core_share) word = kTotalCoreShare;
+  if (word == kNumTotals && !ticks && !core_share)
     return cuking_fail(CUKING_ERR_INVALID_ARGUMENT, "unknown option %s", key);
   if (hipSetDevice(ctx->device) != hipSuccess || hipDeviceSynchronize() != hipSuccess)
     return cuking_fail(CUKING_ERR_DEVICE, "device wait failed");
@@ -744,10 +774,12 @@
       if (hipMemcpy(&v, e.filter + filter_scratch_layout(e.filter_tiles).totals + word * 8, 8,
                     hipMemcpyDeviceToHost) != hipSuccess)
         return cuking_fail(CUKING_ERR_DEVICE, "reading the filter counters failed");
-      sum += v;
+      if (!core_share) sum += v;
+      else if (v > sum) sum = v;
     }
   }
-  if (ticks) *value = count != 0 ? (int64_t)(sum / count) : 0;
+  if (core_share) *value = (int64_t)sum;
+  else if (ticks) *value = count != 0 ? (int64_t)(sum / count) : 0;
   else *value = (int64_t)(sum + ctx->filter_totals_retired[word]);
   return CUKING_OK;
 }
diff --git a/cuking_amd/csrc/king_common.h b/cuking_amd/csrc/king_common.h
--- a/cuking_amd/csrc/king_common.h
+++ b/cuking_amd/csrc/king_common.h
@@ -105,6 +105,7 @@
   const uint32_t *check_steps;
   const float *prefix_u;
   const unsigned long long *cohort_sums;
+  const uint32_t *site_ctrl;
   uint32_t check0, check1;
   uint32_t rotate, rotate_min_steps;
   uint32_t rotate_min_tiles;
@@ -131,6 +132,8 @@
   if (all_steps < min_steps) return 0;
   return phase_step(all_steps, kCheckShares64[k] * kPhasesPerShare);
 }
+constexpr uint32_t kSiteOn = 0, kSiteMass = 16;
+constexpr size_t kSiteCtrlBytes = (kSiteMass + kNumPhases) * sizeof(uint32_t);
 constexpr uint32_t kFilterSplitSlabs = 256;
 constexpr size_t kFilterSlabBytes = 256 * 256 * sizeof(float);
 constexpr size_t kFilterTicketBytes = kFilterSplitSlabs * sizeof(uint32_t);
@@ -141,7 +144,8 @@
   if (layout == kLayoutNibbleStats)
     return base + base / 4 + base / 2 + (size_t)g.s_stride * sizeof(float2) +
            (size_t)g.s_stride * kNumCum * sizeof(float) + 64 + 64 +
-           64 + (size_t)g.s_stride * (4 + 8 + 4 * kNumCum + 16);
+           64 + (size_t)g.s_stride * (4 + 8 + 4 * kNumCum + 16) +
+           kSiteCtrlBytes + (size_t)g.k_words * 32 * 5 * sizeof(uint32_t);
   return base;
 }
 __host__ __device__ inline const uint4 *plane_t2(const uint4 *planes, const PlaneGeometry &g) {
@@ -191,6 +195,8 @@
 constexpr size_t kCtrlChunkBytes = (kCtrlPos + 8 * kPosSlots * 2) * 4;
 constexpr uint32_t kTotalCand = 0, kTotalDense = 1, kTotalEarly = 2, kTotalRotated = 3;
 constexpr uint32_t kNumTotals = 4;
+constexpr uint32_t kTotalCoreShare = kNumTotals;
+static_assert((kTotalCoreShare + 1) * 8 <= 256, "inside the totals block (kFilterCtrlBytes)");
 __host__ __device__ inline const uint32_t *plane_check_steps(const uint4 *planes,
                                                              const PlaneGeometry &g) {
   return reinterpret_cast<const uint32_t *>(plane_cohort_sums(planes, g) + 8);
@@ -210,6 +216,12 @@
 __host__ __device__ inline uint32_t *plane_sort_words(const uint4 *planes, const PlaneGeometry &g) {
   return reinterpret_cast<uint32_t *>(plane_tmp_prefix(planes, g) +
                                       (size_t)g.s_stride * kNumCum);
+}
+__host__ __device__ inline uint32_t *plane_site_ctrl(const uint4 *planes, const PlaneGeometry &g) {
+  return plane_sort_words(planes, g) + 4 * (size_t)g.s_stride;
+}
+__host__ __device__ inline uint32_t *plane_site_words(const uint4 *planes, const PlaneGeometry &g) {
+  return plane_site_ctrl(planes, g) + kSiteCtrlBytes / sizeof(uint32_t);
 }
 constexpr uint32_t kNoSample = 0xFFFFFFFFu;
 
@@ -257,6 +269,15 @@
 hipError_t launch_sample_order(const PlaneGeometry &geo, uint32_t words_per_sample,
                                uint4 *d_planes, uint32_t s_begin, uint32_t s_end, bool sort,
                                void *sort_temp, size_t sort_temp_bytes, hipStream_t stream);
+size_t site_sort_temp_bytes_for(uint32_t sites);
+hipError_t launch_site_order(const uint64_t *d_bit_sets, uint32_t words_per_sample,
+                             const PlaneGeometry &geo, uint4 *d_planes, void *sort_temp,
+                             size_t sort_temp_bytes, hipStream_t stream);
+bool site_order_fits(const PlaneGeometry &geo);
+hipError_t launch_prepare_t2_ordered(const uint64_t *d_bit_sets, uint32_t words_per_sample,
+                                     const PlaneGeometry &geo, uint4 *d_planes,
+                                     const uint32_t *perm, uint32_t s_tile_begin,
+                                     uint32_t s_tile_end, hipStream_t stream);
 hipError_t launch_prepare_nibbles(bool codes, bool t2, const uint64_t *d_bit_sets,
                                   uint32_t words_per_sample, const PlaneGeometry &geo,
                                   uint4 *d_planes, const uint32_t *perm, uint32_t s_tile_begin,
diff --git a/cuking_amd/csrc/king_filter.hip b/cuking_amd/csrc/king_filter.hip
--- a/cuking_amd/csrc/king_filter.hip
+++ b/cuking_amd/csrc/king_filter.hip
@@ -141,6 +141,23 @@
                : "s"(DST), "v"(lane16), "s"(SRC)                               \
                : "memory", "m0")
 
+__device__ __forceinline__ uint32_t all_steps_of(const TiledArgs &a) { return a.geo.k_words / 8; }
+
+__device__ __forceinline__ float cohort_kappa(const TiledArgs &a, float all_sites, float sites) {
+  const float ns = (float)a.cohort_sums[0], nm = (float)a.cohort_sums[1],
+              nh = (float)a.cohort_sums[2];
+  if (!(ns > 0.f && nh > 0.f)) return -1.f;
+  const float m = nm / (ns * all_sites), h = nh / (ns * all_sites);
+  return m * (1.f + m / (2.f * h * (1.f - m))) + 4.6f * rsqrtf(sites) + 0.003f;
+}
+
+__device__ __forceinline__ float core_mass_needed(const TiledArgs &a, float sites) {
+  if (sites <= 0.f) return 0.f;
+  const float kappa = cohort_kappa(a, 256.f * (float)all_steps_of(a), sites);
+  if (kappa < 0.f || kappa >= 0.5f) return 0.f;
+  return (1.f - 2.f * a.kin_threshold) / (1.f - 2.f * kappa);
+}
+
 __device__ __forceinline__ int filter_tile(const TiledArgs &a, const uint32_t wg, uint4 *const lds) {
   uint32_t bid = wg;
   const bool split = a.fsplit_parts != 0 && wg >= a.fsplit_first;
@@ -175,6 +192,7 @@
   const uint32_t wave = __builtin_amdgcn_readfirstlane(threadIdx.x >> 6);
   const uint32_t wy = wave >> 1, wx = wave & 1;
   uint32_t xcd_pos = 0;
+  uint32_t core = 0;
   if (!split && a.tile_done != nullptr) {
     uint32_t *verdict = reinterpret_cast<uint32_t *>(lds);
     if (threadIdx.x == 0) {
@@ -226,7 +244,25 @@
         pos += ago * 16u / ticks16;
       verdict[1 + threadIdx.x] = pos;
     }
-    __syncthreads();
+    if (a.site_ctrl != nullptr && a.check_steps != nullptr && threadIdx.x < kNumPhases) {
+      const uint32_t x = threadIdx.x + 1;
+      const float mass = __uint_as_float(a.site_ctrl[kSiteMass + threadIdx.x]);
+      const float need = core_mass_needed(a, 256.f * (float)phase_step(all_steps_of(a), x));
+      const unsigned long long ok =
+          __ballot(a.site_ctrl[kSiteOn] != 0 && need > 0.f && mass >= need);
+      if ((threadIdx.x & 63) == 0) {
+        verdict[1 + kPosSlots + 2 * (threadIdx.x >> 6)] = (uint32_t)ok;
+        verdict[2 + kPosSlots + 2 * (threadIdx.x >> 6)] = (uint32_t)(ok >> 32);
+      }
+    }
+    __syncthreads();
+    if (a.site_ctrl != nullptr && a.check_steps != nullptr) {
+#pragma unroll
+      for (uint32_t k = 4; k-- > 0;) {
+        const uint32_t w = verdict[1 + kPosSlots + k];
+        if (w != 0) core = 32 * k + (uint32_t)__builtin_ctz(w) + 1;
+      }
+    }
     const bool give_up = verdict[0] != 0;
     if (a.rotate == 1) {
 #pragma unroll
@@ -241,6 +277,9 @@
     }
   }
   xcd_pos = __builtin_amdgcn_readfirstlane(xcd_pos);
+  if (core > 62 * kPhasesPerShare) core = 0;
+  if (core != 0 && core < 32 * kPhasesPerShare) core = 32 * kPhasesPerShare;
+  core = __builtin_amdgcn_readfirstlane(core);
   const uint32_t g = lane >> 5;
   const uint32_t lr = lane & 31;
   uint32_t lane16 = lane * 16;
@@ -267,10 +306,11 @@
   const char *seg_src = g_wave;
   uint32_t seg_steps = num_steps;
   uint32_t seg_wrap = 0xFFFFFFFFu;
+  uint32_t span = kNumPhases, span_steps = all_steps;
   auto addr_of = [&](uint32_t step, uint32_t buf) {
     Addr pa;
     if (step >= seg_steps) step = seg_steps - 1;
-    const int32_t rel = (int32_t)step - (int32_t)(step >= seg_wrap ? all_steps : 0u);
+    const int32_t rel = (int32_t)step - (int32_t)(step >= seg_wrap ? span_steps : 0u);
     pa.src = seg_src + (int64_t)rel * (int64_t)kstep_bytes;
     pa.dst = l_wave + buf * (kStageU4 * 16);
     asm volatile("" : "+s"(pa.src), "+s"(pa.dst));
@@ -279,7 +319,7 @@
   auto addr_next = [&](const Addr &cur, uint32_t step, uint32_t buf) {
     Addr pa;
     const int32_t adv = (int32_t)(step < seg_steps ? 1u : 0u) -
-                        (int32_t)(step == seg_wrap ? all_steps : 0u);
+                        (int32_t)(step == seg_wrap ? span_steps : 0u);
     pa.src = cur.src + (int64_t)adv * (int64_t)kstep_bytes;
     pa.dst = l_wave + buf * (kStageU4 * 16);
     asm volatile("" : "+s"(pa.src), "+s"(pa.dst));
@@ -396,46 +436,46 @@
 
   uint32_t chk0 = 0, chk1 = 0, entry1 = 0, share1 = 0;
   uint32_t phase = 0, k0 = 0, wrap = 0, start_abs = 0;
+  uint32_t chk_phases = 0;
   if (!split && a.check_steps != nullptr && a.tile_done != nullptr) {
+    const uint32_t sw1 = a.check1 & 0xFFu;
+    if (sw1 != 1 || a.check_steps[1] == 0) core = 0;
+    if (core != 0) {
+      span = core;
+      span_steps = phase_step(all_steps, core);
+    }
     if (a.rotate != 0 && all_steps >= a.rotate_min_steps) {
       uint32_t base = 0;
       if (a.rotate == 1) {
-        const uint32_t r = xcd_pos % all_steps;
+        const uint32_t r = xcd_pos % span_steps;
         base = xcd_pos - r;
         phase = (r * kNumPhases + all_steps / 2) / all_steps;
-        if (phase >= kNumPhases) {
+        if (phase >= span) {
           phase = 0;
-          base += all_steps;
+          base += span_steps;
         }
       } else if (a.rotate == 2) {
-        phase = (bid * 37u + 11u) & (kNumPhases - 1);
+        phase = ((bid * 37u + 11u) & (kNumPhases - 1)) % span;
       } else {
-        phase = (a.rotate - 3u) & (kNumPhases - 1);
+        phase = ((a.rotate - 3u) & (kNumPhases - 1)) % span;
       }
       k0 = phase_step(all_steps, phase);
       start_abs = base + k0;
-      wrap = k0 != 0 ? all_steps - k0 : 0u;
-    }
-    float kappa = -1.f;
-    {
-      const float ns = (float)a.cohort_sums[0], nm = (float)a.cohort_sums[1],
-                  nh = (float)a.cohort_sums[2];
-      if (ns > 0.f && nh > 0.f) {
-        const float sites = 256.f * (float)all_steps;
-        const float m = nm / (ns * sites), h = nh / (ns * sites);
-        kappa = m * (1.f + m / (2.f * h * (1.f - m))) + 4.6f * rsqrtf(sites) + 0.003f;
-      }
-    }
+      wrap = k0 != 0 ? span_steps - k0 : 0u;
+    }
+    const float kappa = cohort_kappa(a, 256.f * (float)all_steps, 256.f * (float)all_steps);
     auto steps_of = [&](uint32_t share) {
       const uint32_t hi = phase + share * kPhasesPerShare;
-      return hi <= kNumPhases ? phase_step(all_steps, hi) - k0
-                              : (all_steps - k0) + phase_step(all_steps, hi - kNumPhases);
+      return hi <= span ? phase_step(all_steps, hi) - k0
+                        : (span_steps - k0) + phase_step(all_steps, hi - span);
     };
     if ((a.check0 == 2 || (a.check0 == 1 && kappa > 0.7f * a.kin_threshold)) &&
         a.check_steps[0] != 0)
       chk0 = steps_of(kCheckShares64[0]);
-    const uint32_t sw1 = a.check1 & 0xFFu;
-    if (sw1 >= 2) {
+    if (core != 0) {
+      chk_phases = core;
+      chk1 = span_steps;
+    } else if (sw1 >= 2) {
       entry1 = sw1 - 2;
     } else if (sw1 == 1 && kappa >= 0.f) {
       const float f64 = 64.f * (1.f - 2.f * a.kin_threshold) / (1.f - 2.f * kappa);
@@ -448,27 +488,30 @@
 #pragma unroll
     for (uint32_t k = 1; k < kNumCheckShares; ++k)
       if (sw1 >= 2 && k == entry1) share1 = kCheckShares64[k];
-    if (share1 != 0 && a.check_steps[entry1] != 0) chk1 = steps_of(share1);
+    if (share1 != 0 && a.check_steps[entry1] != 0) {
+      chk1 = steps_of(share1);
+      chk_phases = share1 * kPhasesPerShare;
+    }
     if (chk0 >= num_steps) chk0 = 0;
     if (chk1 >= num_steps || chk1 <= chk0) chk1 = 0;
   }
   chk0 = __builtin_amdgcn_readfirstlane(chk0);
   chk1 = __builtin_amdgcn_readfirstlane(chk1);
-  share1 = __builtin_amdgcn_readfirstlane(share1);
+  chk_phases = __builtin_amdgcn_readfirstlane(chk_phases);
+  span = __builtin_amdgcn_readfirstlane(span);
+  span_steps = __builtin_amdgcn_readfirstlane(span_steps);
   phase = __builtin_amdgcn_readfirstlane(phase);
   k0 = __builtin_amdgcn_readfirstlane(k0);
   wrap = __builtin_amdgcn_readfirstlane(wrap);
   start_abs = __builtin_amdgcn_readfirstlane(start_abs);
-  auto prefix_u_of = [&](uint32_t share, size_t idx, float total) {
-    const uint32_t hi = phase + share * kPhasesPerShare;
-    const uint32_t xb = hi > kNumPhases ? hi - kNumPhases : hi;
-    float u = hi > kNumPhases ? total : 0.f;
-    if (xb == kNumPhases)
-      u += total;
-    else if (xb != 0)
-      u += a.prefix_u[(size_t)(xb - 1) * s_stride + idx];
-    if (phase != 0) u -= a.prefix_u[(size_t)(phase - 1) * s_stride + idx];
-    return u;
+  auto cum_at = [&](uint32_t x, size_t idx, float total) {
+    return x == 0 ? 0.f : x == kNumPhases ? total : a.prefix_u[(size_t)(x - 1) * s_stride + idx];
+  };
+  auto prefix_u_of = [&](uint32_t phases, size_t idx, float total) {
+    const uint32_t hi = phase + phases;
+    float u = hi > span ? cum_at(span, idx, total) + cum_at(hi - span, idx, total)
+                        : cum_at(hi, idx, total);
+    return u - cum_at(phase, idx, total);
   };
   unsigned long long *const pos_word =
       reinterpret_cast<unsigned long long *>(a.filter_ctrl + kCtrlPos) +
@@ -510,7 +553,9 @@
     if (chk0 > seg_first) seg_end = chk0;
     seg_end = __builtin_amdgcn_readfirstlane(seg_end);
     seg_steps = seg_end - seg_first;
-    const uint32_t seg_k = seg_first >= wrap && wrap != 0 ? seg_first - wrap : k0 + seg_first;
+    const uint32_t seg_k = seg_first >= span_steps           ? seg_first
+                           : seg_first >= wrap && wrap != 0 ? seg_first - wrap
+                                                             : k0 + seg_first;
     seg_src = g_wave + (uint64_t)seg_k * kstep_bytes;
     seg_wrap = __builtin_amdgcn_readfirstlane(
         wrap > seg_first && wrap < seg_end ? wrap - seg_first : 0xFFFFFFFFu);
@@ -546,12 +591,19 @@
     if (seg_end == num_steps) break;
 
     const bool forecast = seg_end == chk0;
-    const float scale = forecast ? (float)kCheckShares64[0] * (1.f / 64.f) : 1.f;
+    float scale = forecast ? (float)kCheckShares64[0] * (1.f / 64.f) : 1.f;
+    if (forecast && core != 0) {
+      auto mass_at = [&](uint32_t x) {
+        return x == 0 ? 0.f : __uint_as_float(a.site_ctrl[kSiteMass + x - 1]);
+      };
+      const uint32_t hi = phase + kCheckShares64[0] * kPhasesPerShare;
+      scale = (hi > span ? mass_at(span) + mass_at(hi - span) : mass_at(hi)) - mass_at(phase);
+    }
     float2 *const ck_rows = reinterpret_cast<float2 *>(lds);
     float2 *const ck_cols = ck_rows + kT;
     uint32_t *const ck_words = reinterpret_cast<uint32_t *>(ck_cols + kT);
     {
-      const uint32_t share = forecast ? kCheckShares64[0] : share1;
+      const uint32_t share = forecast ? kCheckShares64[0] * kPhasesPerShare : chk_phases;
       const float thr_f = forecast ? a.kin_threshold + 3.66f * rsqrtf(256.f * (float)all_steps)
                                    : a.kin_threshold;
       const float t = 2.f - 4.f * thr_f;
@@ -614,6 +666,10 @@
   if (phase != 0 && threadIdx.x == 0)
     __hip_atomic_fetch_add(a.filter_totals + kTotalRotated, 1ull, __ATOMIC_RELAXED,
                            __HIP_MEMORY_SCOPE_AGENT);
+  if (!split && threadIdx.x == 0)
+    __hip_atomic_store(a.filter_totals + kTotalCoreShare,
+                       (unsigned long long)((core + kPhasesPerShare - 1) / kPhasesPerShare),
+                       __ATOMIC_RELAXED, __HIP_MEMORY_SCOPE_AGENT);
   if (left && !left_emit) {
     if (threadIdx.x == 0) {
       __hip_atomic_fetch_add(a.filter_ctrl + kCtrlFinished, 4u, __ATOMIC_RELAXED,
@@ -707,8 +763,8 @@
     float2 r = a.sample_stats[ir];
     float2 c = a.sample_stats[ic];
     if (left_emit) {
-      r.x = prefix_u_of(share1, ir, r.x);
-      c.x = prefix_u_of(share1, ic, c.x);
+      r.x = prefix_u_of(chk_phases, ir, r.x);
+      c.x = prefix_u_of(chk_phases, ic, c.x);
     }
     r.y = fmaf(t, r.y, 8.f);
     c.y = fmaf(t, c.y, 8.f);
diff --git a/cuking_amd/csrc/king_kernels.hip b/cuking_amd/csrc/king_kernels.hip
--- a/cuking_amd/csrc/king_kernels.hip
+++ b/cuking_amd/csrc/king_kernels.hip
@@ -680,6 +680,164 @@
 }
 
 namespace {
+
+__device__ __forceinline__ uint32_t spread16(uint32_t x) {
+  x &= 0xFFFFu;
+  x = (x | (x << 8)) & 0x00FF00FFu;
+  x = (x | (x << 4)) & 0x0F0F0F0Fu;
+  x = (x | (x << 2)) & 0x33333333u;
+  x = (x | (x << 1)) & 0x55555555u;
+  return x;
+}
+
+constexpr uint32_t kOrderedThreads = 1024;
+template <int CTRL>
+__device__ __forceinline__ int32_t dpp_add(int32_t v) {
+  return v + __builtin_amdgcn_update_dpp(0, v, CTRL, 0xF, 0xF, false);
+}
+template <int S>
+__global__ __launch_bounds__(kOrderedThreads) void prepare_t2_ordered_kernel(
+    const uint64_t *__restrict__ bits, uint32_t words_per_sample, PlaneGeometry geo,
+    uint4 *__restrict__ planes, uint32_t s_first, const uint32_t *__restrict__ perm,
+    const uint32_t *__restrict__ order, float *__restrict__ cum) {
+  extern __shared__ uint4 raw4[];
+  uint32_t *const raw = reinterpret_cast<uint32_t *>(raw4);
+  __shared__ int32_t phase_sum[S][kNumPhases];
+  __shared__ uint32_t src_of[S];
+  const uint32_t plane_words = words_per_sample / 2;
+  const uint32_t units = geo.k_words / 2, items = 4 * units;
+  const uint32_t all_steps = geo.k_words / 8;
+  const uint32_t ps0 = s_first + blockIdx.x * S;
+  for (uint32_t k = threadIdx.x; k < S * kNumPhases; k += kOrderedThreads)
+    phase_sum[k / kNumPhases][k % kNumPhases] = 0;
+  if (threadIdx.x < S) {
+    const uint32_t ps = ps0 + threadIdx.x;
+    src_of[threadIdx.x] = ps < geo.s_stride ? perm[ps] : kNoSample;
+  }
+  __syncthreads();
+  for (uint32_t w = threadIdx.x; w < units; w += kOrderedThreads) {
+    uint64_t h[S], m[S];
+#pragma unroll
+    for (int si = 0; si < S; ++si) {
+      const uint32_t src = src_of[si];
+      h[si] = m[si] = ~0ull;
+      if (src != kNoSample && w < plane_words) {
+        const uint64_t *het = bits + (uint64_t)src * words_per_sample;
+        h[si] = het[w];
+        m[si] = het[plane_words + w];
+      }
+    }
+#pragma unroll
+    for (int q = 0; q < 4; ++q)
+#pragma unroll
+      for (int si = 0; si < S; ++si)
+        raw[(4 * w + q) * S + si] = spread16((uint32_t)(h[si] >> (16 * q))) |
+                                    (spread16((uint32_t)(m[si] >> (16 * q))) << 1);
+  }
+  __syncthreads();
+  uint32_t *const t2 = reinterpret_cast<uint32_t *>(const_cast<uint4 *>(plane_t2(planes, geo)));
+#pragma unroll 1
+  for (uint32_t i0 = 0; i0 < items; i0 += kOrderedThreads) {
+    const uint32_t i = i0 + threadIdx.x;
+    const bool valid = i < items;
+    const uint32_t u = i >> 2, d = i & 3;
+    uint32_t g[S];
+#pragma unroll
+    for (int si = 0; si < S; ++si) g[si] = 0;
+    uint32_t entry[16];
+#pragma unroll
+    for (int k = 0; k < 16; ++k) entry[k] = valid ? order[(size_t)k * items + i] : 0u;
+#pragma unroll
+    for (int k = 0; k < 16; ++k) {
+      const uint32_t word = entry[k] >> 5, shift = entry[k] & 31u;
+#pragma unroll
+      for (int si = 0; si < S; ++si)
+        g[si] |= ((raw[word * S + si] >> shift) & 3u) << (k < 8 ? 4 * k + 2 : 4 * (k - 8));
+    }
+    uint32_t x = (kNumPhases * (u / 4 + 1) - 1) / all_steps;
+    if (x >= kNumPhases) x = kNumPhases - 1;
+#pragma unroll
+    for (int si = 0; si < S; ++si) {
+      const uint32_t y = ~g[si] & 0x55555555u, hom = g[si] & 0xAAAAAAAAu;
+      const bool there = valid && ps0 + si < geo.s_stride;
+      if (there)
+        t2[((uint64_t)u * geo.s_stride + ps0 + si) * 4 + d] = y | (hom & ~(g[si] << 1));
+      int32_t delta = there && u < plane_words && src_of[si] != kNoSample
+                          ? __popc(y) - __popc(hom & (g[si] << 1)) : 0;
+      delta = dpp_add<0xB1>(delta);
+      delta = dpp_add<0x4E>(delta);
+      delta = dpp_add<0x141>(delta);
+      delta = dpp_add<0x140>(delta);
+      if ((threadIdx.x & 15) == 0 && delta != 0) atomicAdd(&phase_sum[si][x], delta);
+    }
+  }
+  __syncthreads();
+  const uint32_t lane = threadIdx.x & 63, wave = threadIdx.x >> 6;
+  static_assert(kNumPhases == 128 && S <= 4, "one wavefront per sample, two phases per lane");
+  if (wave >= S || ps0 + wave >= geo.s_stride) return;
+  const int32_t p0 = phase_sum[wave][2 * lane], p1 = phase_sum[wave][2 * lane + 1];
+  int32_t run = p0 + p1;
+#pragma unroll
+  for (int off = 1; off < 64; off <<= 1) {
+    const int32_t up = __shfl_up(run, off);
+    if ((int)lane >= off) run += up;
+  }
+  const uint32_t ps = ps0 + wave;
+  cum[(size_t)(2 * lane) * geo.s_stride + ps] = (float)(run - p1);
+  if (2 * lane + 1 < kNumCum) cum[(size_t)(2 * lane + 1) * geo.s_stride + ps] = (float)run;
+}
+
+constexpr size_t kOrderedLdsBytes = 156 * 1024;
+int ordered_samples(const PlaneGeometry &geo) {
+  const size_t row = (size_t)geo.k_words * 8;
+  return 4 * row <= kOrderedLdsBytes ? 4 : 2 * row <= kOrderedLdsBytes ? 2
+                                         : row <= kOrderedLdsBytes     ? 1 : 0;
+}
+
+template <int S>
+hipError_t launch_ordered(const uint64_t *d_bit_sets, uint32_t words_per_sample,
+                          const PlaneGeometry &geo, uint4 *d_planes, const uint32_t *perm,
+                          uint32_t s_first, uint32_t s_last, hipStream_t stream) {
+  const size_t lds = (size_t)S * geo.k_words * 8;
+  static DeviceOnce attr_set;
+  if (!attr_set.done()) {
+    hipError_t e = hipFuncSetAttribute(
+        reinterpret_cast<const void *>(prepare_t2_ordered_kernel<S>),
+        hipFuncAttributeMaxDynamicSharedMemorySize, (int)kOrderedLdsBytes);
+    if (e != hipSuccess) return e;
+    attr_set.mark();
+  }
+  prepare_t2_ordered_kernel<S><<<dim3((s_last - s_first + S - 1) / S), dim3(kOrderedThreads), lds,
+                                 stream>>>(
+      d_bit_sets, words_per_sample, geo, d_planes, s_first, perm,
+      plane_site_words(d_planes, geo) + 4 * (size_t)geo.k_words * 32,
+      const_cast<float *>(plane_prefix_u(d_planes, geo)));
+  return hipGetLastError();
+}
+
+}
+
+bool site_order_fits(const PlaneGeometry &geo) { return ordered_samples(geo) != 0; }
+
+hipError_t launch_prepare_t2_ordered(const uint64_t *d_bit_sets, uint32_t words_per_sample,
+                                     const PlaneGeometry &geo, uint4 *d_planes,
+                                     const uint32_t *perm, uint32_t s_tile_begin,
+                                     uint32_t s_tile_end, hipStream_t stream) {
+  const uint32_t all = (geo.s_stride + kPrepSamples - 1) / kPrepSamples;
+  if (s_tile_end > all) s_tile_end = all;
+  if (s_tile_begin >= s_tile_end) return hipSuccess;
+  const uint32_t first = s_tile_begin * kPrepSamples;
+  uint32_t last = s_tile_end * kPrepSamples;
+  if (last > geo.s_stride) last = geo.s_stride;
+  switch (ordered_samples(geo)) {
+    case 4: return launch_ordered<4>(d_bit_sets, words_per_sample, geo, d_planes, perm, first, last, stream);
+    case 2: return launch_ordered<2>(d_bit_sets, words_per_sample, geo, d_planes, perm, first, last, stream);
+    case 1: return launch_ordered<1>(d_bit_sets, words_per_sample, geo, d_planes, perm, first, last, stream);
+  }
+  return hipErrorInvalidValue;
+}
+
+namespace {
 __global__ void mark_codes_ready_kernel(const uint32_t *gate, uint32_t *ready) {
   if ((gate[kCtrlGate] | gate[kCtrlDense]) != 0) *ready = 1;
 }
diff --git a/cuking_amd/csrc/king_sort.hip b/cuking_amd/csrc/king_sort.hip
--- a/cuking_amd/csrc/king_sort.hip
+++ b/cuking_amd/csrc/king_sort.hip
@@ -48,6 +48,134 @@
     prefix[(size_t)c * geo.s_stride + p] = tmp_prefix[(size_t)c * geo.s_stride + src];
 }
 
+
+constexpr uint32_t kKeySlice = 255;
+__global__ __launch_bounds__(256) void site_key_kernel(
+    const uint64_t *__restrict__ bits, uint32_t words_per_sample, uint32_t num_stored,
+    uint32_t stride, uint32_t *__restrict__ counts) {
+  const uint32_t plane_words = words_per_sample / 2;
+  const uint32_t w = blockIdx.x * 256 + threadIdx.x;
+  if (w >= plane_words) return;
+  const uint32_t first = blockIdx.y * kKeySlice;
+  uint64_t c[8] = {0, 0, 0, 0, 0, 0, 0, 0};
+  for (uint32_t k = 0; k < kKeySlice; ++k) {
+    const uint64_t s = (uint64_t)(first + k) * stride;
+    if (s >= num_stored) break;
+    const uint64_t *p = bits + s * words_per_sample + w;
+    uint64_t carry = p[0] & ~p[plane_words];
+#pragma unroll
+    for (int b = 0; b < 8; ++b) {
+      const uint64_t t = c[b] & carry;
+      c[b] ^= carry;
+      carry = t;
+    }
+  }
+  for (uint32_t bit = 0; bit < 64; ++bit) {
+    uint32_t n = 0;
+#pragma unroll
+    for (int b = 0; b < 8; ++b) n |= (uint32_t)((c[b] >> bit) & 1ull) << b;
+    if (n != 0) atomicAdd(counts + (size_t)w * 64 + bit, n);
+  }
+}
+
+__global__ void site_sort_keys_kernel(uint32_t sites, uint32_t stored_sites,
+                                      uint32_t *__restrict__ keys, uint32_t *__restrict__ vals) {
+  const uint32_t i = blockIdx.x * blockDim.x + threadIdx.x;
+  if (i >= sites) return;
+  keys[i] = i < stored_sites ? keys[i] + 1 : 0u;
+  vals[i] = i;
+}
+
+__global__ void site_order_kernel(uint32_t sites, const uint32_t *__restrict__ sorted,
+                                  uint32_t *__restrict__ order) {
+  const uint32_t i = blockIdx.x * blockDim.x + threadIdx.x;
+  if (i >= sites) return;
+  const uint32_t u = i >> 6, t = i & 63, d = (t & 31) >> 3, k = (t & 7) + (t >= 32 ? 8 : 0);
+  const uint32_t site = sorted[i];
+  order[(size_t)k * (sites / 16) + 4 * u + d] = ((site >> 4) << 5) | ((site & 15) << 1);
+}
+
+__global__ __launch_bounds__(1024) void site_mass_kernel(uint32_t sites,
+                                                         const uint32_t *__restrict__ keys,
+                                                         uint32_t *__restrict__ ctrl) {
+  __shared__ unsigned long long phase_mass[kNumPhases];
+  const uint32_t all_steps = sites / 256;
+  if (threadIdx.x < kNumPhases) phase_mass[threadIdx.x] = 0;
+  __syncthreads();
+  for (uint32_t i0 = 0; i0 < sites; i0 += 1024) {
+    const uint32_t i = i0 + threadIdx.x;
+    unsigned long long n = i < sites && keys[i] != 0 ? keys[i] - 1 : 0;
+#pragma unroll
+    for (int off = 32; off > 0; off >>= 1) n += __shfl_xor(n, off);
+    if ((threadIdx.x & 63) == 0 && i < sites) {
+      const uint32_t x = (kNumPhases * (i / 256 + 1) - 1) / all_steps;
+      atomicAdd(&phase_mass[x < kNumPhases ? x : kNumPhases - 1], n);
+    }
+  }
+  __syncthreads();
+  if (threadIdx.x < kNumPhases) {
+    unsigned long long before = 0, total = 0;
+    for (uint32_t x = 0; x < kNumPhases; ++x) {
+      if (x <= threadIdx.x) before += phase_mass[x];
+      total += phase_mass[x];
+    }
+    const float share = total != 0 ? (float)((double)before / (double)total)
+                                   : (float)(threadIdx.x + 1) / (float)kNumPhases;
+    ctrl[kSiteMass + threadIdx.x] = __float_as_uint(threadIdx.x + 1 == kNumPhases ? 1.f : share);
+  }
+  if (threadIdx.x == 0) ctrl[kSiteOn] = 1;
+}
+
+uint32_t site_key_stride(uint32_t num_stored) { return num_stored > 4096 ? 16 : 1; }
+int site_key_bits(uint32_t num_stored) {
+  const uint32_t sampled = (num_stored + site_key_stride(num_stored) - 1) / site_key_stride(num_stored);
+  int bits = 1;
+  while (bits < 32 && (1ull << bits) <= (unsigned long long)sampled + 1) ++bits;
+  return bits;
+}
+
+}
+
+size_t site_sort_temp_bytes_for(uint32_t sites) {
+  size_t bytes = 0;
+  uint32_t *nil = nullptr;
+  if (sites == 0) return 0;
+  (void)hipcub::DeviceRadixSort::SortPairsDescending(nullptr, bytes, nil, nil, nil, nil, (int)sites,
+                                                     0, 32);
+  return (bytes + 255) / 256 * 256;
+}
+
+hipError_t launch_site_order(const uint64_t *d_bit_sets, uint32_t words_per_sample,
+                             const PlaneGeometry &geo, uint4 *d_planes, void *sort_temp,
+                             size_t sort_temp_bytes, hipStream_t stream) {
+  const uint32_t sites = geo.k_words * 32, plane_words = words_per_sample / 2;
+  const uint32_t num_stored = geo.diag ? geo.num_rows : geo.num_rows + geo.num_cols;
+  if (sites == 0 || num_stored == 0) return hipErrorInvalidValue;
+  uint32_t *ctrl = plane_site_ctrl(d_planes, geo);
+  uint32_t *words = plane_site_words(d_planes, geo);
+  uint32_t *keys_in = words, *keys_out = words + sites, *vals_in = words + 2 * (size_t)sites,
+           *vals_out = words + 3 * (size_t)sites, *order = words + 4 * (size_t)sites;
+  hipError_t e = hipMemsetAsync(keys_in, 0, (size_t)sites * sizeof(uint32_t), stream);
+  if (e != hipSuccess) return e;
+  const uint32_t stride = site_key_stride(num_stored);
+  const uint32_t sampled = (num_stored + stride - 1) / stride;
+  site_key_kernel<<<dim3((plane_words + 255) / 256, (sampled + kKeySlice - 1) / kKeySlice),
+                    dim3(256), 0, stream>>>(d_bit_sets, words_per_sample, num_stored, stride,
+                                            keys_in);
+  if ((e = hipGetLastError()) != hipSuccess) return e;
+  const uint32_t stored_sites = plane_words * 64 < sites ? plane_words * 64 : sites;
+  site_sort_keys_kernel<<<dim3((sites + 255) / 256), dim3(256), 0, stream>>>(sites, stored_sites,
+                                                                            keys_in, vals_in);
+  if ((e = hipGetLastError()) != hipSuccess) return e;
+  size_t bytes = sort_temp_bytes;
+  e = hipcub::DeviceRadixSort::SortPairsDescending(sort_temp, bytes, keys_in, keys_out, vals_in,
+                                                   vals_out, (int)sites, 0,
+                                                   site_key_bits(num_stored), stream);
+  if (e != hipSuccess) return e;
+  site_order_kernel<<<dim3((sites + 255) / 256), dim3(256), 0, stream>>>(sites, vals_out, order);
+  if ((e = hipGetLastError()) != hipSuccess) return e;
+  site_mass_kernel<<<dim3(1), dim3(1024), 0, stream>>>(sites, keys_out, ctrl);
+  return hipGetLastError();
 }
 
 size_t sort_temp_bytes_for(uint32_t n) {
```

Measured after the change: 41.47 billion, median of 6. 11.5% higher.
